# jklebes/MetropolisEngine

Measured on AMD Instinct MI355X. Metric: MC steps/sec (chains x sweeps) at 2^20 chains, 16 params, higher is better.
Workload: dtype f64

## Files before the change

### metropolisengine_amd/csrc/me_api.hip

```cpp
#include <algorithm>
#include <cmath>
#include <cstdlib>
#include <cstring>
#include <dlfcn.h>
#include <mutex>
#include <memory>
#include <string>
#include <atomic>
#include <chrono>
#include <vector>

#include "me_engine.h"

namespace me {

static std::vector<const KernelSet *> &registry() {
  static std::vector<const KernelSet *> sets;
  return sets;
}
static std::mutex &registry_mutex() {
  static std::mutex m;
  return m;
}
void register_kernel_set(const KernelSet *set) {
  std::lock_guard<std::mutex> lock(registry_mutex());
  registry().push_back(set);
}
static bool is_user_kind(int kind) { return kind == ME_ENERGY_USER || kind == ME_ENERGY_USER_INDIRECT; }
const KernelSet *find_kernel_set(int dtype, int n_real, int n_complex, int energy_kind, const char *user_name) {
  std::lock_guard<std::mutex> lock(registry_mutex());
  for (const KernelSet *s : registry()) {
    if (s->dtype != dtype || s->n_real != n_real || s->n_complex != n_complex || !s->has_energy(energy_kind)) continue;
    if (is_user_kind(energy_kind)) {
      if (!s->user_name || !user_name || std::strcmp(s->user_name, user_name) != 0) continue;
    }
    return s;
  }
  if (n_real + 2 * n_complex > kMaxRegisterDof && !is_user_kind(energy_kind))
    for (const KernelSet *s : registry())
      if (s->dtype == dtype && s->n_real < 0 && s->has_energy(energy_kind)) return s;
  return nullptr;
}
bool has_dims(int dtype, int n_real, int n_complex) {
  if (n_real + 2 * n_complex > kMaxRegisterDof) return true;
  std::lock_guard<std::mutex> lock(registry_mutex());
  for (const KernelSet *s : registry())
    if (s->dtype == dtype && s->n_real == n_real && s->n_complex == n_complex && !s->user_name) return true;
  return false;
}

static thread_local std::string g_create_error;

static double norm_ppf(double q) {
  double x = 0.0;
  x = std::log(q / (1.0 - q)) / 1.702;
  for (int it = 0; it < 50; ++it) {
    const double cdf = 0.5 * std::erfc(-x / std::sqrt(2.0));
    const double pdf = std::exp(-0.5 * x * x) / std::sqrt(2.0 * M_PI);
    const double f = cdf - q;
    const double step = f / (pdf * (1.0 + 0.5 * x * f / pdf));
    x -= step;
    if (std::fabs(step) < 1e-16 * std::max(1.0, std::fabs(x))) break;
// ... 54 lines not shown
}

int fail(me_engine *e, int code, const std::string &msg) {
  if (e) e->err = msg;
  else g_create_error = msg;
  return code;
}

static void to_device_type(const double *src, size_t count, int dtype, std::vector<unsigned char> &out) {
  out.resize(count * (dtype == ME_F32 ? 4 : 8));
  if (dtype == ME_F32) {
    float *o = reinterpret_cast<float *>(out.data());
    for (size_t i = 0; i < count; ++i) o[i] = (float)src[i];
  } else {
    std::memcpy(out.data(), src, count * 8);
  }
}

hipError_t upload(DeviceBuffer &dst, const double *src, size_t count, int dtype) {
  std::vector<unsigned char> bytes;
  to_device_type(src, count, dtype, bytes);
  const hipError_t err = dst.resize(bytes.size());
  return err != hipSuccess ? err : hipMemcpy(dst.get(), bytes.data(), bytes.size(), hipMemcpyHostToDevice);
}

int refuse_stale_total(me_engine *e, const char *subject) {
  if (!e->stale_total) return ME_OK;
  return fail(e, ME_ERR_UNSUPPORTED, std::string(subject) + " not available with ME_FLAG_REFERENCE_ENERGY_LEDGERS: its two ledgers "
                                                            "make the energy of a chain ambiguous");
}

static int report_status(me_engine *e, unsigned int bits) {
  if (!bits) return ME_OK;
  ME_HIP(e, hipMemsetAsync(e->status.get(), 0, sizeof(unsigned int), e->stream));
  std::string msg = "numeric failure in at least one chain:";
  if (bits & ST_NONFINITE_ENERGY) msg += " non-finite energy;";
  if (bits & ST_BAD_PIVOT) msg += " non-positive Cholesky pivot (proposal covariance not positive definite);";
  if (bits & ST_BAD_WIDTH) msg += " sampling width <= 0;";
  return fail(e, ME_ERR_NUMERIC, msg);
}
int check_status(me_engine *e) {
  unsigned long long *scratch = e->host_scratch.get<unsigned long long>();
  ME_HIP(e, hipMemcpyAsync(&scratch[0], e->status.get(), sizeof(unsigned int), hipMemcpyDeviceToHost, e->stream));
  ME_HIP(e, hipStreamSynchronize(e->stream));
  return report_status(e, (unsigned int)scratch[0]);
}

}

using namespace me;

namespace {

int broadcast(me_engine *e, DeviceBuffer &dst, const std::vector<double> &row, bool tiled = false) {
  std::vector<unsigned char> bytes;
  to_device_type(row.data(), row.size(), e->dtype, bytes);
  ME_HIP(e, hipMemcpyAsync(e->row_dev.get(), bytes.data(), bytes.size(), hipMemcpyHostToDevice, e->stream));
  if (tiled) ME_HIP(e, launch_broadcast_tiled(dst.get(), e->row_dev.get(), (int)row.size(), e->n, e->dtype, e->stream));
  else ME_HIP(e, launch_broadcast_rows(dst.get(), e->row_dev.get(), (int)row.size(), e->n, e->dtype, e->stream));
  ME_HIP(e, hipStreamSynchronize(e->stream));
  return ME_OK;
}

template <typename T>
void gather_rows(const T *t, int comps, int64_t n_chains, double *dst) {
  for (int r = 0; r < comps; ++r)
    for (int64_t c = 0; c < n_chains; ++c) dst[c * comps + r] = (double)t[(size_t)r * n_chains + c];
}
template <typename T>
void scatter_rows(T *t, int comps, int64_t n_chains, const double *src) {
  for (int r = 0; r < comps; ++r)
    for (int64_t c = 0; c < n_chains; ++c) t[(size_t)r * n_chains + c] = (T)src[c * comps + r];
}
template <typename T>
void transpose_tiled(T *t, int entries, int64_t tile0, int64_t chain_begin, int64_t n_chains, double *dst, const double *src) {
  const size_t tile_values = (size_t)entries * 64;
  auto at = [&](int64_t c, int k) { return (size_t)((c >> 6) - tile0) * tile_values + (size_t)k * 64 + (size_t)(c & 63); };
  for (int64_t i = 0; i < n_chains; ++i)
    for (int k = 0; k < entries; ++k) {
      if (dst) dst[i * entries + k] = (double)t[at(chain_begin + i, k)];
      else t[at(chain_begin + i, k)] = (T)src[i * entries + k];
    }
}

int copy_tiled(me_engine *e, void *field_ptr, int entries, int64_t chain_begin, int64_t n_chains, double *dst, const double *src) {
  const int64_t tile0 = chain_begin >> 6, tile1 = (chain_begin + n_chains - 1) >> 6;
  const size_t tile_values = (size_t)entries * 64, n_values = (size_t)(tile1 - tile0 + 1) * tile_values;
  unsigned char *dev = (unsigned char *)field_ptr + (size_t)tile0 * tile_values * e->esize;
  std::vector<unsigned char> tmp(n_values * e->esize);
  const bool whole = (chain_begin & 63) == 0 && (((chain_begin + n_chains) & 63) == 0 || chain_begin + n_chains == e->n);
  if (dst || !whole) {
    ME_HIP(e, hipMemcpyAsync(tmp.data(), dev, tmp.size(), hipMemcpyDeviceToHost, e->stream));
    ME_HIP(e, hipStreamSynchronize(e->stream));
  }
  if (e->dtype == ME_F32) transpose_tiled(reinterpret_cast<float *>(tmp.data()), entries, tile0, chain_begin, n_chains, dst, src);
  else transpose_tiled(reinterpret_cast<double *>(tmp.data()), entries, tile0, chain_begin, n_chains, dst, src);
  if (src) {
    ME_HIP(e, hipMemcpyAsync(dev, tmp.data(), tmp.size(), hipMemcpyHostToDevice, e->stream));
    ME_HIP(e, hipStreamSynchronize(e->stream));
  }
  return dst ? check_status(e) : ME_OK;
}

int field_info(me_engine *e, int field, void **ptr, int *comps) {
  switch (field) {
    case ME_FIELD_PARAMS: *ptr = e->x.get(); *comps = e->d; return ME_OK;
    case ME_FIELD_ENERGY: *ptr = e->energy.get(); *comps = e->n_terms; return ME_OK;
    case ME_FIELD_WIDTH: *ptr = e->width.get(); *comps = e->width_rows; return ME_OK;
    case ME_FIELD_MEAN: *ptr = e->mean.get(); *comps = e->d; return ME_OK;
    case ME_FIELD_OBS_MEAN: *ptr = e->obs_mean.get(); *comps = e->nobs; return ME_OK;
    case ME_FIELD_COV:
      if (!e->cov)
        return fail(e, ME_ERR_UNSUPPORTED, "this engine keeps no per-chain covariance: for large parameter spaces it is "
                                           "kept on request only (me_config.flags: ME_FLAG_TRACK_COVARIANCE), and not "
                                           "at all where the field would pass 4 GiB");
      *ptr = e->cov.get(); *comps = e->p; return ME_OK;
    case ME_FIELD_ENERGY_TOTAL:
      if (!e->stale_total)
        return fail(e, ME_ERR_UNSUPPORTED, "this engine keeps one coherent energy ledger (sum ME_FIELD_ENERGY); a separate "
                                           "energy_total exists with ME_FLAG_REFERENCE_ENERGY_LEDGERS only");
      *ptr = e->energy.get<unsigned char>() + (size_t)e->n_terms * (size_t)e->n * e->esize; *comps = 1; return ME_OK;
    case ME_FIELD_FACTOR:
      if (!e->factor) return fail(e, ME_ERR_UNSUPPORTED, "this engine keeps no per-chain proposal factors (dimensions "
                                                         "without per-chain kernels, or a field beyond 4 GiB)");
      *ptr = e->factor.get(); *comps = e->p; return ME_OK;
    default: return fail(e, ME_ERR_INVALID, "unknown field id");
  }
}

int upload_shared_factor(me_engine *e, const double *packed) {
  ME_HIP(e, upload(e->shared_factor, packed, (size_t)e->p, e->dtype));
  if (e->shared_full) {
    std::vector<double> full((size_t)e->nr * e->nr, 0.0);
    for (int i = 0; i < e->nr; ++i)
      for (int j = 0; j <= i; ++j) full[(size_t)i * e->nr + j] = packed[i * (i + 1) / 2 + j];
    ME_HIP(e, upload(e->shared_full, full.data(), full.size(), e->dtype));
    if (e->shared_image) ME_HIP(e, e->ks->prepare_matrix(e->shared_full.get(), e->shared_image.get(), e->stream));
  }
  return ME_OK;
}

void fill_step_launch(me_engine *e, StepLaunch &l, int n_sweeps) {
  l.n_real = e->nr;
  l.n_complex = e->nc;
  l.x = e->x.get();
  l.energy = e->energy.get();
  l.width = e->width.get();
  l.factor = e->cov_kind == CK_PER_CHAIN ? e->factor.get() : e->shared_factor.get();
  l.factor_full = e->shared_full.get();
// ... 90 lines not shown
  if (!ks) {
    if (is_user_kind(c->energy_kind))
      return fail(nullptr, ME_ERR_UNSUPPORTED,
                  std::string("no user-energy plugin named '") + (c->user_energy_name ? c->user_energy_name : "") +
                      "' is loaded for these dimensions (build it with metropolisengine_amd.build.build_user_energy "
                      "and load it with me_load_plugin)");
    if (!has_dims(c->dtype, c->n_real, c->n_complex))
      return fail(nullptr, ME_ERR_UNSUPPORTED,
                  "no kernel set compiled for (dtype, n_real, n_complex) = (" + std::to_string(c->dtype) + ", " +
                      std::to_string(c->n_real) + ", " + std::to_string(c->n_complex) + ")");
    return fail(nullptr, ME_ERR_UNSUPPORTED, "energy kind " + std::to_string(c->energy_kind) +
                                                  " is not compiled for these dimensions");
  }
  if ((rc = check_user_reject(nullptr, c->reject_kind, ks)) != ME_OK) return rc;
  if (ks->n_real < 0) {
    if (c->cov_mode == ME_COV_POOLED && c->n_complex > 0)
      return fail(nullptr, ME_ERR_UNSUPPORTED,
                  "parameter spaces beyond " + std::to_string(kMaxRegisterDof) + " real degrees of freedom with complex "
                  "parameters run with the identity proposal shape (ME_COV_FIXED, cov_mode=\"fixed\") or per-chain shapes "
                  "(ME_COV_REFERENCE); one shared factor (ME_COV_POOLED) is there for pure real spaces");
    const bool starts_shared = !initial_shape_is_identity(c) && c->cov_mode != ME_COV_REFERENCE;
    if (starts_shared && c->n_complex > 0)
      return fail(nullptr, ME_ERR_UNSUPPORTED,
                  "parameter spaces beyond " + std::to_string(kMaxRegisterDof) + " real degrees of freedom with complex "
                  "parameters run with the identity proposal shape only: leave covariance_matrix_real / _complex unset");
    {
      const long long per_block = (long long)(c->n_real + 2 * c->n_complex) * 64 * (c->dtype == ME_F32 ? 4 : 8);
      const bool dense = c->energy_kind == ME_ENERGY_DENSE_QUAD, pooled = c->cov_mode == ME_COV_POOLED || starts_shared;
      const bool per_chain = c->cov_mode == ME_COV_REFERENCE || (c->flags & ME_FLAG_TRACK_COVARIANCE) != 0;
      if ((dense || pooled || per_chain) && per_block * (pooled ? 2 : 1) > 150 * 1024)
        return fail(nullptr, ME_ERR_UNSUPPORTED,
                    "a dense quadratic form, a shared proposal factor or per-chain shapes beyond " + std::to_string(kMaxRegisterDof) +
                        " degrees of freedom are staged in LDS: this many parameters do not fit (float64: about 290, 145 with "
                        "a shared factor or an initial covariance that ME_COV_FIXED keeps; float32 twice that)");
    }
    if (c->flags & ME_FLAG_REFERENCE_ENERGY_LEDGERS)
      return fail(nullptr, ME_ERR_UNSUPPORTED, "ME_FLAG_REFERENCE_ENERGY_LEDGERS is not available beyond " +
                                                   std::to_string(kMaxRegisterDof) + " real degrees of freedom");
    if (c->reject_kind == ME_REJECT_USER) return fail(nullptr, ME_ERR_UNSUPPORTED, "no user plugins at these dimensions");
  }
  if ((c->flags & ME_FLAG_REFERENCE_ENERGY_LEDGERS) && (c->n_real == 0 || c->n_complex == 0))
    return fail(nullptr, ME_ERR_INVALID,
                "ME_FLAG_REFERENCE_ENERGY_LEDGERS applies to mixed engines (real and complex parameters): only their "
                "step_all keeps a separate energy_total (metropolis_engine.py:241-259)");
  if (c->cov_mode == ME_COV_REFERENCE && !ks->per_chain_cov)
    return fail(nullptr, ME_ERR_UNSUPPORTED,
                "per-chain adaptive covariance is not compiled for these dimensions; use ME_COV_FIXED or ME_COV_POOLED");
  return ME_OK;
}

struct Layout {
  bool keep_per_chain;
  bool keep_cov;
  bool x_tiled;
  int width_rows;
};
int decide_layout(const me_config *c, const KernelSet *ks, Layout &l) {
  const long long esz = c->dtype == ME_F32 ? 4 : 8, limit = 1ll << 32, padded = padded_chains(c->n_chains);
  l.keep_per_chain = ks->per_chain_cov && (!ks->streams_packed || c->cov_mode == ME_COV_REFERENCE);
  if (l.keep_per_chain && !ks->streams_packed && (long long)packed_total(c->n_real, c->n_complex) * padded * esz >= limit) {
    if (c->cov_mode == ME_COV_REFERENCE)
      return fail(nullptr, ME_ERR_UNSUPPORTED,
                  "the per-chain covariance field would exceed 4 GiB on this engine; shard the chains over more "
                  "engines or use ME_COV_FIXED / ME_COV_POOLED");
    l.keep_per_chain = false;
  }
  const long long rows = std::max<long long>(c->n_real + 2 * c->n_complex, 2 * c->n_real + c->n_complex);
  if (rows * padded * esz >= limit)
    return fail(nullptr, ME_ERR_UNSUPPORTED,
                "a per-chain field would exceed 4 GiB on this engine; shard the chains over more engines");
  l.keep_cov = l.keep_per_chain ||
               ((!ks->per_chain_cov || ks->streams_packed) && ks->tracks_cov && (c->flags & ME_FLAG_TRACK_COVARIANCE));
  l.x_tiled = ks->tiled_state;
  l.width_rows = (c->n_real > 0 && c->n_complex > 0) ? 3 : 1;
  return ME_OK;
}

std::unique_ptr<me_engine> configure(const me_config *c, const KernelSet *ks, const Layout &l) {
  std::unique_ptr<me_engine> e(new me_engine);
  e->device = c->device_id;
  e->ks = ks;
  e->n_terms = ks->energy_terms(c->energy_kind);
  e->dtype = c->dtype;
  e->esize = c->dtype == ME_F32 ? 4 : 8;
  e->n = c->n_chains;
  e->nr = c->n_real;
  e->nc = c->n_complex;
  e->d = e->nr + 2 * e->nc;
  e->p = packed_total(e->nr, e->nc);
  e->nobs = n_observables(e->nr, e->nc);
  e->chain_offset = c->chain_offset;
  e->seed = c->seed;
  e->temp = c->temp;
  e->target_acceptance = c->target_acceptance;
  e->energy_kind = c->energy_kind;
  e->reject_kind = c->reject_kind;
  e->reject_bound = c->reject_bound;
  e->cov_mode = c->cov_mode;
  e->coef.assign(c->energy_coeffs, c->energy_coeffs + c->n_energy_coeffs);
  e->alpha = -norm_ppf(c->target_acceptance / 2.0);
  e->m = e->nr + e->nc;
  e->ratio = (1.0 - 1.0 / e->m) * std::sqrt(2.0 * M_PI) * std::exp(e->alpha * e->alpha / 2.0) / 2.0 * e->alpha +
             1.0 / (e->m * c->target_acceptance * (1.0 - c->target_acceptance));
  if (const char *g = std::getenv("ME_GRID_BLOCKS")) e->grid_blocks = std::atoi(g);
  e->x_tiled = l.x_tiled;
  e->stale_total = (c->flags & ME_FLAG_REFERENCE_ENERGY_LEDGERS) != 0;
  e->width_rows = l.width_rows;
  e->n_slots = (e->n + 31) / 32 + 8;
  return e;
}

int allocate(me_engine *e, const Layout &l) {
  const KernelSet *ks = e->ks;
  ME_HIP(e, hipSetDevice(e->device));
  ME_HIP(e, e->stream.create());
  const size_t n = (size_t)e->n, tiles = (size_t)padded_chains(e->n), es = e->esize;
  ME_HIP(e, e->x.resize((e->x_tiled ? tiles : n) * e->d * es));
  ME_HIP(e, e->energy.resize(n * (e->n_terms + (e->stale_total ? 1 : 0)) * es));
  ME_HIP(e, e->width.resize(n * e->width_rows * es));
  ME_HIP(e, e->mean.resize(n * e->d * es));
  ME_HIP(e, e->obs_mean.resize(n * e->nobs * es));
  if (l.keep_cov) ME_HIP(e, e->cov.resize(tiles * e->p * es));
  if (l.keep_per_chain) ME_HIP(e, e->factor.resize(tiles * e->p * es));
  ME_HIP(e, e->shared_factor.resize((size_t)e->p * es));
  if (e->nc == 0) ME_HIP(e, e->shared_full.resize((size_t)e->nr * e->nr * es));
  if (e->shared_full && ks->prepare_matrix) ME_HIP(e, e->shared_image.resize(ks->matrix_image_bytes));
  ME_HIP(e, e->row_dev.resize((size_t)std::max(std::max(e->d, e->p), e->nobs) * es));
  ME_HIP(e, e->accept_slots.resize((size_t)e->n_slots * sizeof(unsigned long long)));
  ME_HIP(e, e->accept_total.resize(sizeof(unsigned long long)));
  ME_HIP(e, e->status.resize(sizeof(unsigned int)));
  const size_t moments_bytes = sizeof(double) * (size_t)moments_size(e->nr, e->nc);
  ME_HIP(e, e->pool.dev.resize(moments_bytes));
  ME_HIP(e, e->host_scratch.allocate(64));
  e->host_scratch.get<unsigned long long>()[0] = e->host_scratch.get<unsigned long long>()[1] = 0;
  ME_HIP(e, e->pool.host.allocate(moments_bytes));
  if (pool_reduce_supported(e->nr, e->nc, e->dtype))
    ME_HIP(e, e->pool.partials.resize(sizeof(double) * (size_t)pool_reduce_blocks(e->n, e->nr, e->nc) *
                                      (size_t)(1 + e->d + e->nr + e->nc + e->d * (e->d + 1) / 2)));
  ME_HIP(e, hipMemsetAsync(e->accept_slots.get(), 0, e->accept_slots.bytes(), e->stream));
  ME_HIP(e, hipMemsetAsync(e->status.get(), 0, sizeof(unsigned int), e->stream));
  return ME_OK;
}

int upload_coefficients(me_engine *e) {
  const std::vector<double> &coef = e->coef;
  const bool runtime_dims = e->ks->n_real < 0;
  std::vector<double> form;
  if (runtime_dims && e->energy_kind == ME_ENERGY_DIAG_QUAD) {
    if ((int)coef.size() != e->nr + e->nc) return fail(e, ME_ERR_INVALID, "wrong number of energy coefficients for this energy kind");
    form.assign(coef.begin(), coef.end());
    form.insert(form.end(), coef.begin() + e->nr, coef.end());
  } else if (runtime_dims && e->energy_kind == ME_ENERGY_DENSE_QUAD) {
    if ((int)coef.size() != e->d * e->d) return fail(e, ME_ERR_INVALID, "wrong number of energy coefficients for this energy kind");
    form.reserve((size_t)e->d * (e->d + 1) / 2);
    for (int i = 0; i < e->d; ++i)
      for (int j = 0; j <= i; ++j)
        form.push_back(i == j ? coef[(size_t)i * e->d + i] : coef[(size_t)i * e->d + j] + coef[(size_t)j * e->d + i]);
  } else if (e->energy_kind == ME_ENERGY_DENSE_QUAD || (is_user_kind(e->energy_kind) && !coef.empty())) {
    form = coef;
  } else {
    return ME_OK;
  }
  ME_HIP(e, upload(e->coef_dev, form.data(), form.size(), e->dtype));
  if (!runtime_dims && e->energy_kind == ME_ENERGY_DENSE_QUAD && e->ks->prepare_matrix) {
    ME_HIP(e, e->energy_image.resize(e->ks->matrix_image_bytes));
    ME_HIP(e, e->ks->prepare_matrix(e->coef_dev.get(), e->energy_image.get(), e->stream));
  }
  return ME_OK;
}

int initial_state(me_engine *e, const me_config *c) {
  std::vector<double> init(c->initial_params, c->initial_params + e->d);
  std::vector<double> obs(e->nobs);
  for (int i = 0; i < e->nr; ++i) {
    obs[i] = std::fabs(init[i]);
    obs[e->nr + e->nc + i] = init[i] * init[i];
  }
  for (int j = 0; j < e->nc; ++j) obs[e->nr + j] = std::hypot(init[e->nr + j], init[e->nr + e->nc + j]);
  const int pr = packed_real(e->nr);
  std::vector<double> c0(e->p, 0.0);
  bool identity = true;
  for (int i = 0; i < e->nr; ++i)
    for (int j = 0; j <= i; ++j) {
      const double v = c->covariance_real ? c->covariance_real[i * e->nr + j] : (i == j ? 1.0 : 0.0);
      c0[i * (i + 1) / 2 + j] = v;
      identity = identity && v == (i == j ? 1.0 : 0.0);
    }
  for (int i = 0; i < e->nc; ++i) {
    for (int j = 0; j < i; ++j) {
      const double re = c->covariance_complex ? c->covariance_complex[2 * (i * e->nc + j)] : 0.0;
      const double im = c->covariance_complex ? c->covariance_complex[2 * (i * e->nc + j) + 1] : 0.0;
      c0[pr + i * i + 2 * j] = re;
      c0[pr + i * i + 2 * j + 1] = im;
      identity = identity && re == 0.0 && im == 0.0;
    }
    const double dg = c->covariance_complex ? c->covariance_complex[2 * (i * e->nc + i)] : 1.0;
    c0[pr + i * i + 2 * i] = dg;
    identity = identity && dg == 1.0;
  }
  std::vector<double> f0 = c0;
  for (int i = 0; i < e->nc; ++i)
    for (int j = 0; j < i; ++j) f0[pr + i * i + 2 * j + 1] = -f0[pr + i * i + 2 * j + 1];
  if (!host_factor(f0, e->nr, e->nc))
    return fail(e, ME_ERR_INVALID, "initial covariance matrix is not positive definite (metropolis_engine.py:270)");
  int rc = ME_OK;
  std::vector<double> width_row((size_t)e->width_rows, c->sampling_width);
  if ((rc = broadcast(e, e->x, init, e->x_tiled)) || (rc = broadcast(e, e->mean, init)) || (rc = broadcast(e, e->obs_mean, obs)) ||
      (rc = broadcast(e, e->width, width_row)) || (e->cov && (rc = broadcast(e, e->cov, c0, true))) ||
      (e->factor && (rc = broadcast(e, e->factor, f0, true))) || (rc = upload_shared_factor(e, f0.data())))
    return rc;
  e->cov_kind = identity ? CK_IDENTITY : (e->ks->n_real < 0 && e->factor) ? CK_PER_CHAIN : CK_SHARED;
  return ME_OK;
}

int initial_energy(me_engine *e) {
  const int rc = me_recompute_energy(e);
  if (rc != ME_OK) return rc;
  const hipError_t herr = hipStreamSynchronize(e->stream);
  if (herr != hipSuccess) return fail(e, ME_ERR_HIP, std::string("initial energy evaluation: ") + hipGetErrorString(herr));
  return ME_OK;
}

}

int me_create(const me_config *c, me_engine **out) {
  if (!c || !out) return fail(nullptr, ME_ERR_INVALID, "null config or output pointer");
  *out = nullptr;
  const KernelSet *ks = nullptr;
  Layout layout;
  int rc;
  if ((rc = validate_config(c, &ks)) || (rc = decide_layout(c, ks, layout))) return rc;
  int n_dev = 0;
  if (hipGetDeviceCount(&n_dev) != hipSuccess || n_dev <= 0)
    return fail(nullptr, ME_ERR_HIP, "no HIP device available (this library has no CPU fallback)");
  if (c->device_id < 0 || c->device_id >= n_dev) return fail(nullptr, ME_ERR_INVALID, "device_id out of range");

  std::unique_ptr<me_engine> e = configure(c, ks, layout);
  if ((rc = allocate(e.get(), layout)) || (rc = upload_coefficients(e.get())) || (rc = initial_state(e.get(), c)) ||
      (rc = initial_energy(e.get())))
    return fail(nullptr, rc, e->err);
  *out = e.release();
  return ME_OK;
}

int me_set_reject_condition(me_engine *e, int32_t reject_kind, double reject_bound) {
  if (!e) return ME_ERR_INVALID;
  int rc;
  if ((rc = check_reject_kind(e, reject_kind, e->energy_kind, e->nr)) || (rc = check_user_reject(e, reject_kind, e->ks))) return rc;
  e->reject_kind = reject_kind;
  e->reject_bound = reject_bound;
  return ME_OK;
}

int me_set_energy(me_engine *e, int32_t energy_kind, const double *coeffs, int32_t n_coeffs, const char *user_name) {
  if (!e) return ME_ERR_INVALID;
  if (n_coeffs < 0 || (n_coeffs > 0 && !coeffs)) return fail(e, ME_ERR_INVALID, "energy coefficients missing");
  if (e->ks->n_real < 0) return fail(e, ME_ERR_UNSUPPORTED, "me_set_energy: not available on the runtime-dimension kernel set");
  if (energy_kind == ME_ENERGY_DENSE_QUAD)
    return fail(e, ME_ERR_UNSUPPORTED, "me_set_energy: the dense quadratic form keeps device images of its matrix; create a new engine");
  const KernelSet *ks = find_kernel_set(e->dtype, e->nr, e->nc, energy_kind, user_name);
  if (!ks || ks->n_real < 0)
    return fail(e, ME_ERR_UNSUPPORTED, is_user_kind(energy_kind)
                    ? std::string("no user-energy plugin named '") + (user_name ? user_name : "") + "' is loaded for these dimensions"
                    : "energy kind " + std::to_string(energy_kind) + " is not compiled for these dimensions");
  if (ks->tiled_state != e->ks->tiled_state || ks->per_chain_cov != e->ks->per_chain_cov || ks->streams_packed != e->ks->streams_packed ||
      ks->tracks_cov != e->ks->tracks_cov)
    return fail(e, ME_ERR_UNSUPPORTED, "me_set_energy: the plugin was built with other per-chain covariance options than this engine's kernel set");
  if (e->reject_kind == ME_REJECT_USER && !ks->has_user_reject)
    return fail(e, ME_ERR_UNSUPPORTED, "me_set_energy: the engine's wall is the plugin's me_user_reject, which the new energy does not define");
  const int n_terms = ks->energy_terms(energy_kind);
  ME_HIP(e, hipSetDevice(e->device));
  ME_HIP(e, hipStreamSynchronize(e->stream));
  DeviceBuffer ledger, coef_dev;
  if (n_terms != e->n_terms)
    ME_HIP(e, ledger.resize((size_t)e->n * (size_t)(n_terms + (e->stale_total ? 1 : 0)) * e->esize));
  if (is_user_kind(energy_kind) && n_coeffs > 0) ME_HIP(e, upload(coef_dev, coeffs, (size_t)n_coeffs, e->dtype));
  if (n_terms != e->n_terms) {
    e->energy = std::move(ledger);
    e->n_terms = n_terms;
    if (e->trace.chains > 0) e->trace.restart();
  }
  e->coef.assign(coeffs, coeffs + n_coeffs);
  e->coef_dev = std::move(coef_dev);
  e->ks = ks;
  e->energy_kind = energy_kind;
  const int rc = me_recompute_energy(e);
  if (rc != ME_OK) return rc;
  ME_HIP(e, hipStreamSynchronize(e->stream));
  return check_status(e);
}

int me_load_plugin(const char *path) {
  if (!path) return fail(nullptr, ME_ERR_INVALID, "null plugin path");
  void *handle = dlopen(path, RTLD_NOW | RTLD_GLOBAL);
  if (!handle) return fail(nullptr, ME_ERR_INVALID, std::string("dlopen failed: ") + dlerror());
  return ME_OK;
}

int me_destroy(me_engine *e) {
  if (!e) return ME_ERR_INVALID;
  (void)hipSetDevice(e->device);
  if (e->stream) (void)hipStreamSynchronize(e->stream);
  if (e->pool.copy_stream) (void)hipStreamSynchronize(e->pool.copy_stream);
  delete e;
  return ME_OK;
}

int me_recompute_energy(me_engine *e) {
  if (!e) return ME_ERR_INVALID;
  ME_HIP(e, hipSetDevice(e->device));
  EnergyLaunch l;
  l.n_real = e->nr;
  l.n_complex = e->nc;
  l.total_row = e->stale_total ? e->n_terms : -1;
  l.x = e->x.get();
  l.energy = e->energy.get();
  l.coef_device = e->coef_dev.get();
  l.coef_host = e->coef.data();
// ... 88 lines not shown
      for (size_t j = 0; j < nz; ++j) zn[(s * nz + j) * n + c] = normals[(s * n + c) * nz + j];
      for (size_t j = 0; j < nu; ++j) un[(s * nu + j) * n + c] = uniforms[(s * n + c) * nu + j];
    }
  DeviceBuffer zd, ud;
  ME_HIP(e, zd.resize(zn.size() * sizeof(double)));
  if (ud.resize(un.size() * sizeof(double)) != hipSuccess) return fail(e, ME_ERR_HIP, "hipMalloc of the injected uniforms failed");
  if (hipMemcpy(zd.get(), zn.data(), zd.bytes(), hipMemcpyHostToDevice) != hipSuccess ||
      hipMemcpy(ud.get(), un.data(), ud.bytes(), hipMemcpyHostToDevice) != hipSuccess)
    return fail(e, ME_ERR_HIP, "upload of the injected streams failed");
  int rc = launch_step_kind(e, kind, n_sweeps, zd.get(), ud.get());
  if (rc == ME_OK && hipStreamSynchronize(e->stream) != hipSuccess) rc = fail(e, ME_ERR_HIP, "injected step failed");
  return rc;
}

namespace {
void fill_measure_launch(me_engine *e, MeasureLaunch &l, unsigned long long count) {
  l.n_real = e->nr;
  l.n_complex = e->nc;
  l.x = e->x.get();
  l.width = e->width.get();
  l.mean = e->mean.get();
  l.cov = e->cov.get();
  l.obs_mean = e->obs_mean.get();
  l.factor = e->factor.get();
  l.status = e->status.get<unsigned int>();
  l.n = e->n;
  l.measure_count = count;
  l.update_cov = (count > 50 && e->cov) ? 1 : 0;
  l.split_widths = (e->width_rows == 3 && !e->widths_synced) ? 1 : 0;
  l.write_factor = (l.update_cov && e->cov_mode == ME_COV_REFERENCE) ? 1 : 0;
  l.grid_blocks = e->grid_blocks;
}

int commit_measure(me_engine *e, const MeasureLaunch &l) {
  e->measure_count = l.measure_count;
  if (l.write_factor) e->cov_kind = CK_PER_CHAIN;
  if (e->trace.chains > 0) {
    const long long cols = e->d + e->n_terms + e->width_rows;
    if (e->trace.rows == e->trace.capacity) {
      const long long cap = e->trace.capacity ? 2 * e->trace.capacity : 1024;
      DeviceBuffer bigger;
      ME_HIP(e, bigger.resize(sizeof(double) * (size_t)(cap * cols * e->trace.chains)));
      if (e->trace.dev) {
        ME_HIP(e, hipMemcpyAsync(bigger.get(), e->trace.dev.get(), sizeof(double) * (size_t)(e->trace.rows * cols * e->trace.chains),
                                 hipMemcpyDeviceToDevice, e->stream));
        ME_HIP(e, hipStreamSynchronize(e->stream));
      }
      e->trace.dev = std::move(bigger);
      e->trace.capacity = cap;
    }
    const int rows_valid = (e->width_rows == 3 && e->widths_synced) ? 1 : e->width_rows;
    double *row = e->trace.dev.get<double>() + e->trace.rows * cols * e->trace.chains;
    ME_HIP(e, launch_trace(e->x.get(), e->energy.get(), e->width.get(), e->n, e->d, e->n_terms, rows_valid, e->dtype, e->trace.chains,
                           e->trace.stride, row, e->stream, e->x_tiled));
    if (rows_valid != e->width_rows) {
      double *widths = row + (size_t)(e->d + e->n_terms) * e->trace.chains;
      for (int r = 1; r < 3; ++r)
        ME_HIP(e, hipMemcpyAsync(widths + (size_t)r * e->trace.chains, widths, sizeof(double) * (size_t)e->trace.chains,
                                 hipMemcpyDeviceToDevice, e->stream));
    }
    e->trace.rows += 1;
  }
  return ME_OK;
}
}

int me_measure(me_engine *e) {
  if (!e) return ME_ERR_INVALID;
  ME_HIP(e, hipSetDevice(e->device));
  MeasureLaunch l;
  fill_measure_launch(e, l, e->measure_count + 1);
  ME_HIP(e, e->ks->measure(l, e->stream));
  return commit_measure(e, l);
}

int me_cycle(me_engine *e, int32_t n_sweeps) {
  if (!e) return ME_ERR_INVALID;
  if (n_sweeps <= 0) return fail(e, ME_ERR_INVALID, "n_sweeps must be positive");
  ME_HIP(e, hipSetDevice(e->device));
  if (e->ks->cycle) {
    StepLaunch sl;
    fill_step_launch(e, sl, n_sweeps);
    MeasureLaunch ml;
    fill_measure_launch(e, ml, e->measure_count + 1);
    ml.split_widths = 0;
    const hipError_t err = e->ks->cycle(sl, ml, e->stream);
    if (err == hipSuccess) {
      count_steps(e, n_sweeps);
      e->fused_cycles += 1;
      return commit_measure(e, ml);
    }
    if (err != hipErrorNotSupported) ME_HIP(e, err);
    (void)hipGetLastError();
  }
  const int rc = me_step(e, n_sweeps);
  return rc != ME_OK ? rc : me_measure(e);
}

int me_cycle_stats(me_engine *e, uint64_t *fused_cycles) {
  if (!e || !fused_cycles) return ME_ERR_INVALID;
  *fused_cycles = e->fused_cycles;
  return ME_OK;
}

int me_trace_enable(me_engine *e, int64_t n_traced, int64_t stride) {
  if (!e) return ME_ERR_INVALID;
  if (n_traced < 0 || stride < 1 || (n_traced > 0 && (n_traced - 1) * stride >= e->n))
    return fail(e, ME_ERR_INVALID, "traced chains out of range");
  ME_HIP(e, hipSetDevice(e->device));
  ME_HIP(e, hipStreamSynchronize(e->stream));
  e->trace.restart();
  e->trace.chains = n_traced;
  e->trace.stride = stride;
  return ME_OK;
}

int me_trace_shape(me_engine *e, int64_t *rows, int64_t *cols, int64_t *n_traced) {
  if (!e) return ME_ERR_INVALID;
  if (rows) *rows = e->trace.rows;
  if (cols) *cols = e->d + e->n_terms + e->width_rows;
  if (n_traced) *n_traced = e->trace.chains;
  return ME_OK;
}

int me_trace_get(me_engine *e, double *dst, int64_t n_doubles) {
  if (!e || !dst) return ME_ERR_INVALID;
  const long long want = e->trace.rows * (e->d + e->n_terms + e->width_rows) * e->trace.chains;
  if (n_doubles != want) return fail(e, ME_ERR_INVALID, "wrong trace buffer length");
  if (want == 0) return ME_OK;
  ME_HIP(e, hipSetDevice(e->device));
  ME_HIP(e, hipStreamSynchronize(e->stream));
  ME_HIP(e, hipMemcpy(dst, e->trace.dev.get(), sizeof(double) * (size_t)want, hipMemcpyDeviceToHost));
  return ME_OK;
}

int me_field_components(me_engine *e, int32_t field, int32_t *n_components) {
  if (!e || !n_components) return ME_ERR_INVALID;
  void *ptr;
  int comps;
  int rc = field_info(e, field, &ptr, &comps);
  if (rc == ME_OK) *n_components = comps;
  return rc;
}

int me_energy_terms(me_engine *e, int32_t *n_terms) {
  if (!e || !n_terms) return ME_ERR_INVALID;
  *n_terms = e->n_terms;
  return ME_OK;
}

int me_get(me_engine *e, int32_t field, int64_t chain_begin, int64_t n_chains, double *dst) {
  if (!e || !dst) return ME_ERR_INVALID;
  if (chain_begin < 0 || n_chains < 0 || chain_begin + n_chains > e->n) return fail(e, ME_ERR_INVALID, "chain range out of bounds");
  ME_HIP(e, hipSetDevice(e->device));
  void *ptr;
  int comps;
  int rc = field_info(e, field, &ptr, &comps);
  if (rc != ME_OK) return rc;
  if (n_chains == 0) return ME_OK;
  if (field == ME_FIELD_COV || field == ME_FIELD_FACTOR || (field == ME_FIELD_PARAMS && e->x_tiled))
    return copy_tiled(e, ptr, comps, chain_begin, n_chains, dst, nullptr);
  std::vector<unsigned char> tmp((size_t)comps * n_chains * e->esize);
  for (int r = 0; r < comps; ++r)
    ME_HIP(e, hipMemcpyAsync(tmp.data() + (size_t)r * n_chains * e->esize,
                             (const unsigned char *)ptr + ((size_t)r * e->n + chain_begin) * e->esize,
                             (size_t)n_chains * e->esize, hipMemcpyDeviceToHost, e->stream));
  ME_HIP(e, hipStreamSynchronize(e->stream));
  if (e->dtype == ME_F32) gather_rows(reinterpret_cast<const float *>(tmp.data()), comps, n_chains, dst);
  else gather_rows(reinterpret_cast<const double *>(tmp.data()), comps, n_chains, dst);
  if (field == ME_FIELD_WIDTH && e->width_rows == 3 && e->widths_synced)
    for (int64_t c = 0; c < n_chains; ++c) dst[c * 3 + 1] = dst[c * 3 + 2] = dst[c * 3];
  return check_status(e);
}

int me_set(me_engine *e, int32_t field, int64_t chain_begin, int64_t n_chains, const double *src) {
  if (!e || !src) return ME_ERR_INVALID;
  if (chain_begin < 0 || n_chains < 0 || chain_begin + n_chains > e->n) return fail(e, ME_ERR_INVALID, "chain range out of bounds");
  ME_HIP(e, hipSetDevice(e->device));
  void *ptr;
  int comps;
  int rc = field_info(e, field, &ptr, &comps);
  if (rc != ME_OK) return rc;
  if (field == ME_FIELD_WIDTH && e->width_rows == 3 && (chain_begin != 0 || n_chains != e->n))
    return fail(e, ME_ERR_INVALID, "widths of a mixed engine must be set for all chains at once");
  if (n_chains == 0) return ME_OK;
  if (field == ME_FIELD_COV || field == ME_FIELD_FACTOR || (field == ME_FIELD_PARAMS && e->x_tiled)) {
    rc = copy_tiled(e, ptr, comps, chain_begin, n_chains, nullptr, src);
    if (rc != ME_OK) return rc;
    if (field == ME_FIELD_FACTOR) e->cov_kind = CK_PER_CHAIN;
    return ME_OK;
  }
  std::vector<unsigned char> tmp((size_t)comps * n_chains * e->esize);
  if (e->dtype == ME_F32) scatter_rows(reinterpret_cast<float *>(tmp.data()), comps, n_chains, src);
  else scatter_rows(reinterpret_cast<double *>(tmp.data()), comps, n_chains, src);
  for (int r = 0; r < comps; ++r)
    ME_HIP(e, hipMemcpyAsync((unsigned char *)ptr + ((size_t)r * e->n + chain_begin) * e->esize,
                             tmp.data() + (size_t)r * n_chains * e->esize, (size_t)n_chains * e->esize,
                             hipMemcpyHostToDevice, e->stream));
  ME_HIP(e, hipStreamSynchronize(e->stream));
  if (field == ME_FIELD_FACTOR) e->cov_kind = CK_PER_CHAIN;
  if (field == ME_FIELD_WIDTH && e->width_rows == 3) e->widths_synced = false;
  return ME_OK;
}

int me_constants(me_engine *e, double *alpha, int32_t *m, double *ratio) {
  if (!e) return ME_ERR_INVALID;
  if (alpha) *alpha = e->alpha;
  if (m) *m = e->m;
  if (ratio) *ratio = e->ratio;
  return ME_OK;
}

int me_counters(me_engine *e, uint64_t *step_index, uint64_t *measure_step_counter) {
  if (!e) return ME_ERR_INVALID;
  if (step_index) *step_index = e->step_index;
  if (measure_step_counter) *measure_step_counter = e->measure_count;
  return ME_OK;
}

int me_set_counters(me_engine *e, uint64_t step_index, uint64_t measure_step_counter) {
  if (!e) return ME_ERR_INVALID;
  if (measure_step_counter < 1) return fail(e, ME_ERR_INVALID, "measure_step_counter starts at 1");
  e->step_index = step_index;
  e->measure_count = measure_step_counter;
  return ME_OK;
}

int me_accept_stats(me_engine *e, uint64_t *accepted, uint64_t *proposed) {
  if (!e) return ME_ERR_INVALID;
  ME_HIP(e, hipSetDevice(e->device));
  unsigned long long *scratch = e->host_scratch.get<unsigned long long>();
  ME_HIP(e, launch_sum_slots(e->accept_slots.get<unsigned long long>(), e->n_slots, e->accept_total.get<unsigned long long>(), e->stream));
  ME_HIP(e, hipMemcpyAsync(&scratch[1], e->accept_total.get(), sizeof(unsigned long long), hipMemcpyDeviceToHost, e->stream));
  ME_HIP(e, hipMemcpyAsync(&scratch[0], e->status.get(), sizeof(unsigned int), hipMemcpyDeviceToHost, e->stream));
  ME_HIP(e, hipStreamSynchronize(e->stream));
  if (accepted) *accepted = scratch[1];
  if (proposed) *proposed = e->proposed;
  return report_status(e, (unsigned int)scratch[0]);
}

int me_set_accept_stats(me_engine *e, uint64_t accepted, uint64_t proposed) {
  if (!e) return ME_ERR_INVALID;
  if (accepted > proposed) return fail(e, ME_ERR_INVALID, "accepted exceeds proposed");
  ME_HIP(e, hipSetDevice(e->device));
  const unsigned long long total = accepted;
  ME_HIP(e, hipMemsetAsync(e->accept_slots.get(), 0, e->accept_slots.bytes(), e->stream));
  ME_HIP(e, hipMemcpyAsync(e->accept_slots.get(), &total, sizeof(total), hipMemcpyHostToDevice, e->stream));
  ME_HIP(e, hipStreamSynchronize(e->stream));
  e->proposed = proposed;
  return ME_OK;
}

int me_pooled_moments_size(me_engine *e, int64_t *n_doubles) {
  if (!e || !n_doubles) return ME_ERR_INVALID;
  *n_doubles = moments_size(e->nr, e->nc);
  return ME_OK;
}

namespace {
hipError_t wait_polling(hipEvent_t ev) {
  const auto t0 = std::chrono::steady_clock::now();
  for (;;) {
    const hipError_t rc = hipEventQuery(ev);
    if (rc != hipErrorNotReady) return rc;
    if (std::chrono::steady_clock::now() - t0 > std::chrono::milliseconds(2)) return hipEventSynchronize(ev);
  }
}
hipError_t wait_polling(hipStream_t stream) {
  const auto t0 = std::chrono::steady_clock::now();
  for (;;) {
    const hipError_t rc = hipStreamQuery(stream);
    if (rc != hipErrorNotReady) return rc;
    if (std::chrono::steady_clock::now() - t0 > std::chrono::milliseconds(2)) return hipStreamSynchronize(stream);
  }
}

int check_pooled(me_engine *e, int64_t n_doubles) {
  if (n_doubles != moments_size(e->nr, e->nc)) return fail(e, ME_ERR_INVALID, "wrong pooled-moment buffer length");
  if (e->pool.pending) return fail(e, ME_ERR_STATE, "a pooled-moment reduction is in flight (me_pooled_moments_end first)");
  if (!e->pool.partials) return fail(e, ME_ERR_UNSUPPORTED, "pooled moments: dimension too large for the reduction kernel");
  ME_HIP(e, hipSetDevice(e->device));
  return ME_OK;
}
int enqueue_pool_reduce(me_engine *e, const void *x, long long n_chains, long long n_slots, double proposed, double *device_out) {
  hipError_t err = launch_pool_reduce(x, n_chains, e->nr, e->nc, e->dtype, e->accept_slots.get<unsigned long long>(), n_slots, proposed,
                                      e->pool.partials.get<double>(), device_out, e->stream, e->ks->pool_stage1, e->x_tiled);
  if (err == hipErrorInvalidValue) return fail(e, ME_ERR_UNSUPPORTED, "pooled moments: dimension too large for the reduction kernel");
  ME_HIP(e, err);
  return ME_OK;
}
int enqueue_pooled_moments(me_engine *e, double *device_out, int64_t n_doubles) {
  const int rc = check_pooled(e, n_doubles);
  return rc != ME_OK ? rc : enqueue_pool_reduce(e, e->x.get(), e->n, e->n_slots, (double)e->proposed, device_out);
}
int fetch_pooled_moments(me_engine *e, double *host_out, int64_t n_doubles) {
  const size_t bytes = sizeof(double) * (size_t)n_doubles;
  ME_HIP(e, hipMemcpyAsync(e->pool.host.get<double>(), e->pool.dev.get(), bytes, hipMemcpyDeviceToHost, e->stream));
  ME_HIP(e, wait_polling(e->stream));
  std::memcpy(host_out, e->pool.host.get<double>(), bytes);
  return ME_OK;
}
}

int me_pooled_moments_device(me_engine *e, void *device_out, int64_t n_doubles) {
  if (!e || !device_out) return ME_ERR_INVALID;
  int rc = enqueue_pooled_moments(e, (double *)device_out, n_doubles);
  if (rc != ME_OK) return rc;
  ME_HIP(e, wait_polling(e->stream));
  return ME_OK;
}

int me_pooled_moments(me_engine *e, double *host_out, int64_t n_doubles) {
  if (!e || !host_out) return ME_ERR_INVALID;
  const int rc = enqueue_pooled_moments(e, e->pool.dev.get<double>(), n_doubles);
  return rc != ME_OK ? rc : fetch_pooled_moments(e, host_out, n_doubles);
}

int me_pooled_moments_range(me_engine *e, int64_t chain_begin, int64_t n_chains, double *host_out, int64_t n_doubles) {
  if (!e || !host_out) return ME_ERR_INVALID;
  if (chain_begin < 0 || n_chains <= 0 || chain_begin + n_chains > e->n || chain_begin % 64 != 0 || n_chains % 64 != 0)
    return fail(e, ME_ERR_INVALID, "the chain range must be whole 64-chain tiles inside the engine");
  int rc = check_pooled(e, n_doubles);
  if (rc != ME_OK) return rc;
  const unsigned char *x = e->x.get<unsigned char>();
  if (e->x_tiled) {
    x += (size_t)chain_begin * e->d * e->esize;
  } else {
    const size_t row = (size_t)n_chains * e->esize;
    if (row * e->d > e->pool.range_x.bytes()) {
      ME_HIP(e, hipStreamSynchronize(e->stream));
      ME_HIP(e, e->pool.range_x.reserve(row * e->d));
    }
    ME_HIP(e, hipMemcpy2DAsync(e->pool.range_x.get(), row, x + (size_t)chain_begin * e->esize, (size_t)e->n * e->esize, row, (size_t)e->d,
                               hipMemcpyDeviceToDevice, e->stream));
    x = e->pool.range_x.get<unsigned char>();
  }
  if ((rc = enqueue_pool_reduce(e, x, n_chains, 0, 0.0, e->pool.dev.get<double>())) != ME_OK) return rc;
  return fetch_pooled_moments(e, host_out, n_doubles);
}

namespace {
int begin_pooled(me_engine *e, bool allreduce) {
  if (e->pool.pending) return fail(e, ME_ERR_STATE, "a pooled-moment reduction is already in flight: call me_pooled_moments_end first");
  if (allreduce && !e->comm)
    return fail(e, ME_ERR_STATE, "this engine has no communicator: call me_comm_init_rank first (single-GPU engines use me_pooled_moments)");
  ME_HIP(e, hipSetDevice(e->device));
  if (!e->pool.copy_stream) {
    ME_HIP(e, e->pool.copy_stream.create());
    ME_HIP(e, e->pool.reduced.create(hipEventDisableTiming));
    ME_HIP(e, e->pool.copied.create(hipEventDisableTiming));
  }
  const int64_t n_doubles = moments_size(e->nr, e->nc);
  int rc = enqueue_pooled_moments(e, e->pool.dev.get<double>(), n_doubles);
  if (rc != ME_OK) return rc;
  ME_HIP(e, hipEventRecord(e->pool.reduced, e->stream));
  ME_HIP(e, hipStreamWaitEvent(e->pool.copy_stream, e->pool.reduced, 0));
  if (allreduce) {
    const ncclResult_t nrc = e->rccl->all_reduce(e->pool.dev.get<double>(), e->pool.dev.get<double>(), (size_t)n_doubles, ncclDouble, ncclSum, e->comm, e->pool.copy_stream);
    if (nrc != ncclSuccess) return fail(e, ME_ERR_HIP, std::string("ncclAllReduce: ") + e->rccl->error_string(nrc));
  }
  ME_HIP(e, hipMemcpyAsync(e->pool.host.get<double>(), e->pool.dev.get<double>(), sizeof(double) * (size_t)n_doubles, hipMemcpyDeviceToHost, e->pool.copy_stream));
  ME_HIP(e, hipEventRecord(e->pool.copied, e->pool.copy_stream));
  e->pool.pending = true;
  return ME_OK;
}
}

int me_pooled_moments_begin(me_engine *e) {
  if (!e) return ME_ERR_INVALID;
  return begin_pooled(e, false);
}

int me_pooled_moments_allreduce_begin(me_engine *e) {
  if (!e) return ME_ERR_INVALID;
  return begin_pooled(e, true);
}

int me_pooled_moments_allreduce(me_engine *e, double *host_out, int64_t n_doubles) {
// ... 148 lines not shown
```

### metropolisengine_amd/csrc/me_device.h

```cpp
#pragma once

#include <type_traits>
#include <utility>

#include <hip/hip_runtime.h>
#include <stdint.h>

#include "me_internal.h"
#include "me_math64.h"

namespace me {

struct U4 {
  uint32_t x, y, z, w;
};

__device__ __forceinline__ uint32_t xor3(uint32_t a, uint32_t b, uint32_t c) {
  return __builtin_amdgcn_bitop3_b32(a, b, c, 0x96);
}
__device__ __forceinline__ U4 philox4x32_10(U4 c, uint32_t k0, uint32_t k1) {
#pragma unroll
  for (int r = 0; r < 10; ++r) {
    const uint64_t p0 = (uint64_t)0xD2511F53u * c.x;
    const uint64_t p1 = (uint64_t)0xCD9E8D57u * c.z;
// ... 148 lines not shown
  static constexpr unsigned int kEntryBytes = 64u * (unsigned int)sizeof(R);
  template <int AUX>
  __device__ __forceinline__ R load_aux(int k, unsigned int tile_off) const {
    if constexpr (sizeof(R) == 4) {
      return __builtin_bit_cast(R, __builtin_amdgcn_raw_buffer_load_b32(rsrc, tile_off, (unsigned int)k * kEntryBytes, AUX));
    } else {
      const auto v = __builtin_amdgcn_raw_buffer_load_b64(rsrc, tile_off, (unsigned int)k * kEntryBytes, AUX);
      return __builtin_bit_cast(R, v);
    }
  }
  template <int AUX>
  __device__ __forceinline__ void store_aux(int k, unsigned int tile_off, R value) const {
    if constexpr (sizeof(R) == 4) {
      __builtin_amdgcn_raw_buffer_store_b32(__builtin_bit_cast(unsigned int, value), rsrc, tile_off, (unsigned int)k * kEntryBytes, AUX);
    } else {
      using v2 = decltype(__builtin_amdgcn_raw_buffer_load_b64(rsrc, 0u, 0u, 0));
      __builtin_amdgcn_raw_buffer_store_b64(__builtin_bit_cast(v2, value), rsrc, tile_off, (unsigned int)k * kEntryBytes, AUX);
    }
  }
  __device__ __forceinline__ R load(int k, unsigned int tile_off) const { return load_aux<0>(k, tile_off); }
  __device__ __forceinline__ R load_nt(int k, unsigned int tile_off) const { return load_aux<ME_NT_AUX>(k, tile_off); }
  __device__ __forceinline__ void store(int k, unsigned int tile_off, R value) const { store_aux<0>(k, tile_off, value); }
  __device__ __forceinline__ void store_nt(int k, unsigned int tile_off, R value) const { store_aux<ME_NT_AUX>(k, tile_off, value); }
};

template <bool NT, class F>
__device__ __forceinline__ auto packed_load(const F &f, int row, unsigned int chain_off) {
  if constexpr (NT) return f.load_nt(row, chain_off);
  else return f.load(row, chain_off);
}
template <bool NT, class F, typename R>
__device__ __forceinline__ void packed_store(const F &f, int row, unsigned int chain_off, R value) {
  if constexpr (NT) f.store_nt(row, chain_off, value);
  else f.store(row, chain_off, value);
}

template <typename R, bool NTS>
struct StateField : Field<R> {
  using Field<R>::Field;
  __device__ __forceinline__ R load(int row, unsigned int chain_off) const {
    if constexpr (NTS) return Field<R>::load_nt(row, chain_off);
    else return Field<R>::load(row, chain_off);
  }
  __device__ __forceinline__ void store(int row, unsigned int chain_off, R value) const {
    if constexpr (NTS) Field<R>::store_nt(row, chain_off, value);
    else Field<R>::store(row, chain_off, value);
  }
};

#ifndef ME_TILED_STATE_DOF
#define ME_TILED_STATE_DOF 16
#endif
constexpr int kTiledStateDof = ME_TILED_STATE_DOF;
template <typename R, int D, bool NTS = false>
struct XField {
  static constexpr bool kTiled = D >= kTiledStateDof;
  std::conditional_t<kTiled, TiledField<R>, StateField<R, NTS>> f;
  __device__ __forceinline__ XField(const R *base, long long n) : f(base, n, D) {}
  static __device__ __forceinline__ unsigned int offset(long long c) {
    if constexpr (kTiled) return tiled_offset<R>(c, D);
    else return (unsigned int)c * (unsigned int)sizeof(R);
  }
  __device__ __forceinline__ R load(int row, unsigned int off) const {
    if constexpr (kTiled && NTS) return f.load_nt(row, off);
    else return f.load(row, off);
  }
  __device__ __forceinline__ void store(int row, unsigned int off, R value) const {
    if constexpr (kTiled && NTS) f.store_nt(row, off, value);
    else f.store(row, off, value);
  }
};
template <typename R, int D>
__device__ __forceinline__ long long state_index(long long c, int row, long long n) {
  if constexpr (D >= kTiledStateDof) return ((c >> 6) * (long long)D + row) * 64 + (c & 63);
  else return (long long)row * n + c;
}

constexpr int kMaxPackedInRegisters = 160;
#ifndef ME_STREAM_F64_ENTRIES
#define ME_STREAM_F64_ENTRIES 96
#endif
constexpr int kStreamF64Entries = ME_STREAM_F64_ENTRIES;

template <typename R, int NR, int NC>
struct EnergyIso {
  static constexpr int D = NR + 2 * NC;
  R a;
  __device__ __forceinline__ R operator()(const R (&x)[D]) const {
    R s0 = 0, s1 = 0;
#pragma unroll
    for (int d = 0; d + 1 < D; d += 2) {
      s0 += x[d] * x[d];
      s1 += x[d + 1] * x[d + 1];
    }
    if constexpr (D % 2 == 1) s0 += x[D - 1] * x[D - 1];
    return a * (s0 + s1);
  }
};

template <typename R, int NR, int NC>
struct EnergyDiag {
  static constexpr int D = NR + 2 * NC;
  R w[D];
  __device__ __forceinline__ R operator()(const R (&x)[D]) const {
    R s0 = 0, s1 = 0;
#pragma unroll
    for (int d = 0; d + 1 < D; d += 2) {
      s0 += w[d] * x[d] * x[d];
      s1 += w[d + 1] * x[d + 1] * x[d + 1];
    }
    if constexpr (D % 2 == 1) s0 += w[D - 1] * x[D - 1] * x[D - 1];
    return s0 + s1;
  }
};

template <typename R, int NR, int NC>
struct EnergyDense {
  static constexpr int D = NR + 2 * NC;
  static constexpr int PT = D * (D + 1) / 2;
  const R *a;
  static __device__ __forceinline__ R *folded() {
    __shared__ R t[PT];
    return t;
  }
  __device__ __forceinline__ void prepare() const {
    R *t = folded();
    constexpr int kBatch = 8;
    for (int k0 = threadIdx.x; k0 < PT; k0 += kBatch * (int)blockDim.x) {
      R lo[kBatch], hi[kBatch];
// ... 256 lines not shown
  constexpr bool MOVE_REAL = NR > 0 && GROUP != GROUP_COMPLEX;
  constexpr bool MOVE_COMPLEX = NC > 0 && GROUP != GROUP_REAL;
#pragma unroll
  for (int d = 0; d < D; ++d) xp[d] = x[d];
  if constexpr (CK == CK_IDENTITY) {
    if constexpr (MOVE_REAL) {
#pragma unroll
      for (int i = 0; i < NR; ++i) xp[i] = x[i] + w_r * g[i];
    }
    if constexpr (MOVE_COMPLEX) {
#pragma unroll
      for (int j = 0; j < NC; ++j) {
        xp[NR + j] = x[NR + j] + w_c * (g[NR + j] * R(0.70710678118654752440));
        xp[NR + NC + j] = x[NR + NC + j] + w_c * (g[NR + NC + j] * R(0.70710678118654752440));
      }
    }
  } else {
    if constexpr (MOVE_REAL) {
#pragma unroll
      for (int i = 0; i < NR; ++i) {
        R acc = 0;
#pragma unroll
        for (int j = 0; j <= i; ++j) acc += fac(tri(i, j)) * g[j];
        xp[i] = x[i] + w_r * acc;
      }
    }
    if constexpr (MOVE_COMPLEX) {
#pragma unroll
      for (int i = 0; i < NC; ++i) {
        R are = 0, aim = 0;
#pragma unroll
        for (int j = 0; j < i; ++j) {
          const R lre = fac(cre(PR, i, j));
          const R lim = fac(cim(PR, i, j));
          const R wre = g[NR + j] * R(0.70710678118654752440), wim = g[NR + NC + j] * R(0.70710678118654752440);
          are += lre * wre - lim * wim;
          aim += lre * wim + lim * wre;
        }
        const R ld = fac(cdiag(PR, i));
        are += ld * (g[NR + i] * R(0.70710678118654752440));
        aim += ld * (g[NR + NC + i] * R(0.70710678118654752440));
        xp[NR + i] = x[NR + i] + w_c * are;
        xp[NR + NC + i] = x[NR + NC + i] + w_c * aim;
      }
    }
  }

}

template <typename R, int NR, int NC, class Energy, int CK, int GROUP, bool LADDER, class Ledger>
__device__ __forceinline__ void decide_step(const StepArgs<R> &a, long long c, const Energy &en, bool stale_total, R u,
                                            const R (&g)[2 * ((NR + 2 * NC + 1) / 2)], R (&x)[NR + 2 * NC], const R (&xp)[NR + 2 * NC],
                                            Ledger &ledger, R &total_q5, R &w, R &w_r, R &w_c, unsigned int &wave_accepted,
                                            bool &bad_energy) {
  [[maybe_unused]] constexpr int D = NR + 2 * NC;
  constexpr bool MOVE_REAL = NR > 0 && GROUP != GROUP_COMPLEX;
  constexpr bool MOVE_COMPLEX = NC > 0 && GROUP != GROUP_REAL;
  using N_ = Num<R>;
  bool rejected = false;
  if (a.reject_kind == ME_REJECT_ABS_REAL0_GE) rejected = !(N_::abs_(xp[0]) < a.reject_bound);
  else if (a.reject_kind == ME_REJECT_USER) rejected = energy_reject(en, xp, 0);
  R terms_new[Ledger::T];
  const R e_new = ledger.propose(en, xp, terms_new);
  const R diff = e_new - (stale_total ? total_q5 : ledger.partial());
  bool accept = diff <= R(0);
  if constexpr (LADDER) accept = accept || uphill_at<true>(a, c, u, diff);
  else if (a.temp > R(0)) accept = accept || N_::uphill(u, diff, a.inv_temp, a.inv_temp_log2e);
  accept = accept && !rejected;
  bad_energy |= (!rejected && !N_::finite(e_new));
  if constexpr (CK == CK_IDENTITY) {
    const R wa_r = accept ? w_r : R(0), wa_c = accept ? w_c : R(0);
    if constexpr (MOVE_REAL) {
#pragma unroll
      for (int i = 0; i < NR; ++i) x[i] = x[i] + wa_r * g[i];
    }
    if constexpr (MOVE_COMPLEX) {
#pragma unroll
      for (int j = 0; j < NC; ++j) {
        x[NR + j] = x[NR + j] + wa_c * (g[NR + j] * R(0.70710678118654752440));
        x[NR + NC + j] = x[NR + NC + j] + wa_c * (g[NR + NC + j] * R(0.70710678118654752440));
      }
    }
  } else {
#pragma unroll
    for (int d = 0; d < D; ++d) x[d] = accept ? xp[d] : x[d];
  }
  if (stale_total) total_q5 = accept ? e_new : total_q5;
  else ledger.commit(accept, terms_new);
  w = N_::adapt(w, accept, a.ratio, a.p, a.damping, a.up, a.down);
  if constexpr (GROUP == GROUP_ALL) w_r = w_c = w;
  else if constexpr (GROUP == GROUP_REAL) w_r = w;
  else w_c = w;
  wave_accepted += (unsigned int)__popcll(__ballot(accept));
}

template <typename R, int NR, int NC, class Energy, int CK, bool INJECT, int GROUP, bool LADDER, class Ledger, class Fac>
__device__ __forceinline__ void run_sweeps(const StepArgs<R> &a, const Energy &en, long long c, unsigned long long gid,
                                           bool stale_total, R (&x)[NR + 2 * NC], Ledger &ledger, R &total_q5, R &w, R &w_r,
                                           R &w_c, Fac &&fac, unsigned int &wave_accepted, bool &bad_energy) {
  constexpr int D = NR + 2 * NC;
  constexpr int NW = 2 * ((D + 1) / 2);
  for (int s = 0; s < a.n_sweeps; ++s) {
    R g[NW], u, xp[D];
    draw_step<R, NR, NC, INJECT>(a, c, gid, s, g, u);
    propose_registers<R, NR, NC, CK, GROUP>(x, g, w_r, w_c, fac, xp);
    decide_step<R, NR, NC, Energy, CK, GROUP, LADDER>(a, c, en, stale_total, u, g, x, xp, ledger, total_q5, w, w_r, w_c, wave_accepted, bad_energy);
  }
}

#ifndef ME_STEP_WAVES_PER_EU
#define ME_STEP_WAVES_PER_EU 0
#endif
#if ME_STEP_WAVES_PER_EU > 0
#define ME_STEP_BOUNDS __launch_bounds__(kFusedStepThreads, ME_STEP_WAVES_PER_EU)
#else
#define ME_STEP_BOUNDS __launch_bounds__(kFusedStepThreads)
#endif

#ifndef ME_STEP_PRIO_SHIFT
#define ME_STEP_PRIO_SHIFT 8
#endif
__device__ __forceinline__ void stagger_priority() {
#if ME_STEP_PRIO_SHIFT >= 0
  switch ((blockIdx.x >> ME_STEP_PRIO_SHIFT) & 3u) {
    case 0: __builtin_amdgcn_s_setprio(3); break;
    case 1: __builtin_amdgcn_s_setprio(2); break;
    case 2: __builtin_amdgcn_s_setprio(1); break;
    default: break;
  }
#endif
}

template <typename R, int NR, int NC, class Energy, int CK, bool INJECT = false, int GROUP = GROUP_ALL, bool NTS = false,
          bool LADDER = false>
__global__ void ME_STEP_BOUNDS k_step(StepArgs<R> a, Energy en) {
  constexpr int D = NR + 2 * NC;
  constexpr bool MIXED = NR > 0 && NC > 0;
  static_assert(GROUP == GROUP_ALL || MIXED, "group-wise kernels exist for mixed engines only");
  using N_ = Num<R>;

  stagger_priority();
  if constexpr (!INJECT) N_::prepare();
  energy_prepare(en, 0);
  unsigned int wave_accepted = 0;
  bool bad_energy = false, bad_width = false;
  const long long stride = (long long)gridDim.x * blockDim.x;
  using Ledger = EnergyLedger<R, Energy, GROUP>;
  const XField<R, D, NTS> fx(a.x, a.n);
  const StateField<R, NTS> fe(a.energy, a.n, Ledger::T + (MIXED ? 1 : 0)), fw(a.width, a.n, MIXED ? 3 : 1);
  const bool stale_total = MIXED && GROUP == GROUP_ALL && a.stale_total != 0;
  constexpr bool PER_CHAIN = CK == CK_PER_CHAIN || CK == CK_PER_CHAIN_NT;
  constexpr int PF = PER_CHAIN ? NR * (NR + 1) / 2 + NC * NC : 0;
  constexpr bool STREAM_FACTOR = PER_CHAIN && (PF > kMaxPackedInRegisters ||
                                               (!INJECT && sizeof(R) == 8 && NC == 0 && PF > kStreamF64Entries));
  const TiledField<R> ffac(a.factor, a.n, STREAM_FACTOR ? 0 : PF);
  for (long long c = (long long)blockIdx.x * blockDim.x + threadIdx.x; c < a.n; c += stride) {
    const unsigned int coff = (unsigned int)c * (unsigned int)sizeof(R);
    const unsigned int xoff = fx.offset(c);
    R x[D];
#pragma unroll
    for (int d = 0; d < D; ++d) x[d] = fx.load(d, xoff);
    Ledger ledger;
    R total_q5 = R(0);
    if (stale_total) total_q5 = fe.load(Ledger::T, coff);
    else ledger.load(fe, coff);
    R w = fw.load(MIXED ? GROUP : 0, coff);
    R w_r = w, w_c = w;
    if constexpr (MIXED && GROUP == GROUP_ALL) {
      if (a.split_widths) {
        w_r = fw.load(GROUP_REAL, coff);
        w_c = fw.load(GROUP_COMPLEX, coff);
      }
    }
    const unsigned long long gid = a.chain_offset + (unsigned long long)c;
    [[maybe_unused]] const unsigned int toff = tiled_offset<R>(c, PF);
    auto fac = [&](int k) -> R {
      if constexpr (CK == CK_PER_CHAIN_NT) return ffac.load_nt(k, toff);
      else if constexpr (CK == CK_PER_CHAIN) return ffac.load(k, toff);
      else return a.factor[k];
    };

    if constexpr (STREAM_FACTOR) {
      constexpr int NW = 2 * ((D + 1) / 2);
      for (int s = 0; s < a.n_sweeps; ++s) {
        static_assert(!INJECT, "the streamed-factor form has no replay hook");
        constexpr int NBLK = (NW + 1 + 3) / 4;
        const unsigned long long step = a.step_index + (unsigned long long)s;
        R g[NW];
        R u_accept;
        {
          uint32_t words[4 * NBLK];
#pragma unroll
          for (int b = 0; b < NBLK; ++b) {
            U4 ctr;
            ctr.x = (uint32_t)gid;
            ctr.y = (uint32_t)(gid >> 32);
            ctr.z = (uint32_t)step;
            ctr.w = ((uint32_t)(step >> 32) << 16) | (uint32_t)b;
            const U4 o = philox4x32_10(ctr, a.seed_lo, a.seed_hi);
            words[4 * b + 0] = o.x;
            words[4 * b + 1] = o.y;
            words[4 * b + 2] = o.z;
            words[4 * b + 3] = o.w;
          }
#pragma unroll
          for (int q = 0; q < NW / 2; ++q) N_::normal_pair(words[2 * q], words[2 * q + 1], g[2 * q], g[2 * q + 1]);
          u_accept = N_::unit(words[NW]);
        }
        R xp[D];
#pragma unroll
        for (int d = 0; d < D; ++d) xp[d] = x[d];
        asm volatile("" ::: "memory");
        constexpr int CH = (int)(ME_STREAM_CHUNK_BYTES / sizeof(R));
        const R *tile_base = a.factor + (c >> 6) * (long long)PF * 64;
// ... 24 lines not shown
            __builtin_amdgcn_sched_barrier(0);
          }
          return f[(k / CH) & 1][k % CH];
        };
        static_for<NR>([&](auto row_index) {
          constexpr int i = decltype(row_index)::value;
          R acc = 0;
          static_for<i + 1>([&](auto col_index) {
            constexpr int j = decltype(col_index)::value, k = tri(i, j);
            const R l = use(std::integral_constant<int, k>{});
            acc = j == 0 ? l * g[0] : acc + l * g[j];
          });
          if constexpr (GROUP != GROUP_COMPLEX) xp[i] = x[i] + w_r * acc;
        });
        static_for<NC>([&](auto row_index) {
          constexpr int i = decltype(row_index)::value;
          R are = 0, aim = 0;
          static_for<i>([&](auto col_index) {
            constexpr int j = decltype(col_index)::value;
            const R lre = use(std::integral_constant<int, cre(NR * (NR + 1) / 2, i, j)>{});
            const R lim = use(std::integral_constant<int, cim(NR * (NR + 1) / 2, i, j)>{});
            const R wre = g[NR + j] * R(0.70710678118654752440), wim = g[NR + NC + j] * R(0.70710678118654752440);
            are += lre * wre - lim * wim;
            aim += lre * wim + lim * wre;
          });
          const R ld = use(std::integral_constant<int, cdiag(NR * (NR + 1) / 2, i)>{});
          are += ld * (g[NR + i] * R(0.70710678118654752440));
          aim += ld * (g[NR + NC + i] * R(0.70710678118654752440));
          if constexpr (GROUP != GROUP_REAL) {
            xp[NR + i] = x[NR + i] + w_c * are;
            xp[NR + NC + i] = x[NR + NC + i] + w_c * aim;
          }
        });
        bool rejected = false;
        if (a.reject_kind == ME_REJECT_ABS_REAL0_GE) rejected = !(N_::abs_(xp[0]) < a.reject_bound);
        else if (a.reject_kind == ME_REJECT_USER) rejected = energy_reject(en, xp, 0);
        R terms_new[Ledger::T];
        const R e_new = ledger.propose(en, xp, terms_new);
        const R diff = e_new - (stale_total ? total_q5 : ledger.partial());
        bool accept = diff <= R(0);
        if constexpr (LADDER) accept = accept || uphill_at<true>(a, c, u_accept, diff);
        else if (a.temp > R(0)) accept = accept || N_::uphill(u_accept, diff, a.inv_temp, a.inv_temp_log2e);
        accept = accept && !rejected;
        bad_energy |= (!rejected && !N_::finite(e_new));
#pragma unroll
        for (int d = 0; d < D; ++d) x[d] = accept ? xp[d] : x[d];
        if (stale_total) total_q5 = accept ? e_new : total_q5;
        else ledger.commit(accept, terms_new);
        w = N_::adapt(w, accept, a.ratio, a.p, a.damping, a.up, a.down);
        if constexpr (GROUP == GROUP_ALL) w_r = w_c = w;
        else if constexpr (GROUP == GROUP_REAL) w_r = w;
        else w_c = w;
        wave_accepted += (unsigned int)__popcll(__ballot(accept));
      }
    } else {
      run_sweeps<R, NR, NC, Energy, CK, INJECT, GROUP, LADDER>(a, en, c, gid, stale_total, x, ledger, total_q5, w, w_r, w_c, fac, wave_accepted, bad_energy);
    }
    bad_width |= !(w > R(0));
#pragma unroll
    for (int d = 0; d < D; ++d) fx.store(d, xoff, x[d]);
    if (stale_total) fe.store(Ledger::T, coff, total_q5);
    else ledger.store(fe, coff);
    fw.store(MIXED ? GROUP : 0, coff, w);
  }
  if ((threadIdx.x & 63) == 0 && wave_accepted) {
    unsigned long long *slot = a.accept_slots + (size_t)blockIdx.x * (blockDim.x >> 6) + (threadIdx.x >> 6);
    *slot += (unsigned long long)wave_accepted;
  }
  const unsigned int bits = (bad_energy ? ST_NONFINITE_ENERGY : 0u) | (bad_width ? ST_BAD_WIDTH : 0u);
  if (bits) atomicOr(a.status, bits);
}

template <typename R, int NR, int NC, class Energy>
__global__ void __launch_bounds__(kStepThreads) k_init_energy(const R *xs, R *energy, long long n, unsigned int *status,
                                                                Energy en, int total_row) {
  constexpr int D = NR + 2 * NC;
  energy_prepare(en, 0);
  const long long stride = (long long)gridDim.x * kStepThreads;
  for (long long c = (long long)blockIdx.x * kStepThreads + threadIdx.x; c < n; c += stride) {
    R x[D];
#pragma unroll
    for (int d = 0; d < D; ++d) x[d] = xs[state_index<R, D>(c, d, n)];
    constexpr int T = term_count<Energy>::value;
    bool finite = true;
    R total = R(0);
#pragma unroll
    for (int t = 0; t < T; ++t) {
      R e;
      if constexpr (T == 1) e = en(x);
      else e = en.term(t, x);
      energy[(long long)t * n + c] = e;
      total = t == 0 ? e : total + e;
      finite = finite && Num<R>::finite(e);
    }
    if (total_row >= 0) energy[(long long)total_row * n + c] = total;
    if (!finite) atomicOr(status, (unsigned int)ST_NONFINITE_ENERGY);
  }
}

template <typename R>
struct MeasureArgs {
  const R *x, *width;
  R *mean, *cov, *obs_mean, *factor;
  unsigned int *status;
  long long n;
  R keep;
  R inv_i;
  R cov_keep;
  int update_cov, write_factor, split_widths;
};

template <typename R, int NR, int NC>
__device__ __forceinline__ void cholesky_packed(R (&m)[NR * (NR + 1) / 2 + NC * NC], bool &bad_pivot) {
  constexpr int PR = NR * (NR + 1) / 2;
  using N_ = Num<R>;
#pragma unroll
    for (int j = 0; j < NR; ++j) {
      R s = m[tri(j, j)];
#pragma unroll
      for (int k = 0; k < j; ++k) s = fma_(-m[tri(j, k)], m[tri(j, k)], s);
      if (!(s > R(0))) { bad_pivot = true; s = R(1e-30); }
      const R dg = N_::sqrt_(s);
      const R inv = R(1) / dg;
      m[tri(j, j)] = dg;
#pragma unroll
      for (int i = j + 1; i < NR; ++i) {
        R t = m[tri(i, j)];
#pragma unroll
        for (int k = 0; k < j; ++k) t = fma_(-m[tri(i, k)], m[tri(j, k)], t);
        m[tri(i, j)] = t * inv;
      }
    }
#pragma unroll
    for (int j = 0; j < NC; ++j) {
      R s = m[cdiag(PR, j)];
// ... 149 lines not shown
        }
      } else {
      R m[P];
#pragma unroll
      for (int k = 0; k < P; ++k) m[k] = src.cov(k);
#pragma unroll
      for (int i = 0; i < NR; ++i)
#pragma unroll
        for (int j = 0; j <= i; ++j) {
          const int k = tri(i, j);
          R v = fma_(delta[i] * delta[j], a.inv_i, m[k] * a.cov_keep);
          if (i == j) v = fma_(w2_real, a.inv_i, v);
          packed_store<NT>(fcov, k, toff, v);
          m[k] = v;
        }
#pragma unroll
      for (int i = 0; i < NC; ++i) {
        const R ai = delta[NR + i], bi = delta[NR + NC + i];
#pragma unroll
        for (int j = 0; j < i; ++j) {
          const R aj = delta[NR + j], bj = delta[NR + NC + j];
          const int kr = cre(PR, i, j), ki = cim(PR, i, j);
          const R vr = fma_(fma_(ai, aj, bi * bj), a.inv_i, m[kr] * a.cov_keep);
          const R vi = fma_(fma_(bi, aj, -(ai * bj)), a.inv_i, m[ki] * a.cov_keep);
          packed_store<NT>(fcov, kr, toff, vr);
          packed_store<NT>(fcov, ki, toff, vi);
          m[kr] = vr;
          m[ki] = -vi;
        }
        const int kd = cdiag(PR, i);
        const R vd = fma_(w2_cplx, a.inv_i, fma_(fma_(ai, ai, bi * bi), a.inv_i, m[kd] * a.cov_keep));
        packed_store<NT>(fcov, kd, toff, vd);
        m[kd] = vd;
      }
      if constexpr (FUSED) {
        if (a.write_factor) {
          cholesky_packed<R, NR, NC>(m, bad_pivot);
#pragma unroll
          for (int k = 0; k < P; ++k) packed_store<NT>(ffac, k, toff, m[k]);
        }
      }
      }
    }
  }
}

template <typename R, int NR, int NC, bool PER_CHAIN_COV, bool FUSED, bool NT, bool NTM>
__global__ void __launch_bounds__(kStepThreads, ME_MEASURE_WAVES) k_measure(MeasureArgs<R> a) {
  constexpr int D = NR + 2 * NC;
  constexpr int P = NR * (NR + 1) / 2 + NC * NC;
  constexpr int NOBS = 2 * NR + NC;
  bool bad_pivot = false;
  const long long stride = (long long)gridDim.x * kStepThreads;
  const XField<R, D> fx(a.x, a.n);
  const Field<R> fw(a.width, a.n, (NR > 0 && NC > 0) ? 3 : 1), fmean(a.mean, a.n, D), fobs(a.obs_mean, a.n, NOBS);
  constexpr bool STREAM = PER_CHAIN_COV && P > kMaxPackedInRegisters;
  const TiledField<R> fcov(a.cov, a.n, (PER_CHAIN_COV && !STREAM) ? P : 0);
  const TiledField<R> ffac(a.factor, a.n, (PER_CHAIN_COV && FUSED) ? P : 0);
  __shared__ R s_delta[STREAM ? D : 1][kStepThreads];
  for (long long c = (long long)blockIdx.x * kStepThreads + threadIdx.x; c < a.n; c += stride) {
    const unsigned int coff = (unsigned int)c * (unsigned int)sizeof(R);
    const unsigned int xoff = fx.offset(c);
    R x[D];
#pragma unroll
    for (int d = 0; d < D; ++d) x[d] = fx.load(d, xoff);
    const MeasureFromMemory<R, NT, NTM> src{fmean, fobs, fcov, coff, tiled_offset<R>(c, P)};
    measure_chain<R, NR, NC, PER_CHAIN_COV, FUSED, NT, NTM>(a, c, x, src, fmean, fobs, fcov, ffac, s_delta, [&](R &w_real, R &w_cplx) {
      constexpr bool MIXED = NR > 0 && NC > 0;
      w_real = fw.load((MIXED && a.split_widths) ? 1 : 0, coff);
      w_cplx = fw.load((MIXED && a.split_widths) ? 2 : 0, coff);
    }, bad_pivot);
  }
  if (bad_pivot) atomicOr(a.status, (unsigned int)ST_BAD_PIVOT);
}

#ifndef ME_CYCLE_PREFETCH
#define ME_CYCLE_PREFETCH 0
#endif
constexpr int cycle_prefetch_level(int, int, int, int) { return ME_CYCLE_PREFETCH; }

template <typename R, int NR, int NC, class Energy, int CK, bool NT, bool NTM, bool LADDER = false>
__global__ void ME_STEP_BOUNDS k_cycle(StepArgs<R> a, MeasureArgs<R> ma, Energy en) {
  constexpr int D = NR + 2 * NC;
  constexpr int P = NR * (NR + 1) / 2 + NC * NC;
  constexpr int NOBS = 2 * NR + NC;
  constexpr bool MIXED = NR > 0 && NC > 0;
  static_assert(P <= kMaxPackedInRegisters, "k_cycle keeps the packed matrix in registers");
  static_assert(CK == CK_IDENTITY || CK == CK_SHARED || CK == CK_PER_CHAIN, "NT selects the non-temporal factor read");
  constexpr int CKX = CK == CK_PER_CHAIN ? (NT ? CK_PER_CHAIN_NT : CK_PER_CHAIN) : CK;
  using N_ = Num<R>;
  N_::prepare();
  energy_prepare(en, 0);
  unsigned int wave_accepted = 0;
  bool bad_energy = false, bad_width = false, bad_pivot = false;
  const long long stride = (long long)gridDim.x * blockDim.x;
  using Ledger = EnergyLedger<R, Energy, GROUP_ALL>;
  const XField<R, D> fx(a.x, a.n);
  const Field<R> fe(a.energy, a.n, Ledger::T + (MIXED ? 1 : 0)), fw(a.width, a.n, MIXED ? 3 : 1);
  const Field<R> fmean(ma.mean, a.n, D), fobs(ma.obs_mean, a.n, NOBS);
  const TiledField<R> fcov(ma.cov, a.n, P), ffac(ma.factor, a.n, P);
  const bool stale_total = MIXED && a.stale_total != 0;
  for (long long c = (long long)blockIdx.x * blockDim.x + threadIdx.x; c < a.n; c += stride) {
    const unsigned int coff = (unsigned int)c * (unsigned int)sizeof(R);
    const unsigned int xoff = fx.offset(c);
    R x[D];
#pragma unroll
    for (int d = 0; d < D; ++d) x[d] = fx.load(d, xoff);
    Ledger ledger;
    R total_q5 = R(0);
    if (stale_total) total_q5 = fe.load(Ledger::T, coff);
    else ledger.load(fe, coff);
    R w = fw.load(0, coff);
    R w_r = w, w_c = w;
    if constexpr (MIXED) {
      if (a.split_widths) {
        w_r = fw.load(GROUP_REAL, coff);
        w_c = fw.load(GROUP_COMPLEX, coff);
      }
    }
    const unsigned long long gid = a.chain_offset + (unsigned long long)c;
    [[maybe_unused]] const unsigned int toff = tiled_offset<R>(c, P);
    auto fac = [&](int k) -> R {
      if constexpr (CK == CK_PER_CHAIN) return packed_load<NT>(ffac, k, toff);
      else return a.factor[k];
    };
    constexpr int kPrefetch = cycle_prefetch_level(D, NOBS, P, (int)sizeof(R));
    MeasurePreloaded<R, D, NOBS, P, kPrefetch, NT> pre{{}, {}, {}, fcov, toff};
    if constexpr (kPrefetch >= 1) {
#pragma unroll
      for (int d = 0; d < D; ++d) pre.mu[d] = packed_load<NTM>(fmean, d, coff);
#pragma unroll
      for (int k = 0; k < NOBS; ++k) pre.ob[k] = packed_load<NTM>(fobs, k, coff);
    }
    if constexpr (kPrefetch >= 2) {
      if (ma.update_cov) {
#pragma unroll
        for (int k = 0; k < P; ++k) pre.cv[k] = packed_load<NT>(fcov, k, toff);
      }
    }
    run_sweeps<R, NR, NC, Energy, CKX, false, GROUP_ALL, LADDER>(a, en, c, gid, stale_total, x, ledger, total_q5, w, w_r, w_c, fac,
                                                         wave_accepted, bad_energy);
    bad_width |= !(w > R(0));
#pragma unroll
    for (int d = 0; d < D; ++d) fx.store(d, xoff, x[d]);
    if (stale_total) fe.store(Ledger::T, coff, total_q5);
    else ledger.store(fe, coff);
    fw.store(0, coff, w);
    if constexpr (kPrefetch >= 1) {
      measure_chain<R, NR, NC, true, true, NT, NTM>(ma, c, x, pre, fmean, fobs, fcov, ffac, nullptr,
                                                    [&](R &w_real, R &w_cplx) { w_real = w_cplx = w; }, bad_pivot);
    } else {
      const MeasureFromMemory<R, NT, NTM> src{fmean, fobs, fcov, coff, toff};
      measure_chain<R, NR, NC, true, true, NT, NTM>(ma, c, x, src, fmean, fobs, fcov, ffac, nullptr,
                                                    [&](R &w_real, R &w_cplx) { w_real = w_cplx = w; }, bad_pivot);
    }
  }
  if ((threadIdx.x & 63) == 0 && wave_accepted) {
    unsigned long long *slot = a.accept_slots + (size_t)blockIdx.x * (blockDim.x >> 6) + (threadIdx.x >> 6);
    *slot += (unsigned long long)wave_accepted;
  }
  const unsigned int bits = (bad_energy ? ST_NONFINITE_ENERGY : 0u) | (bad_width ? ST_BAD_WIDTH : 0u) | (bad_pivot ? ST_BAD_PIVOT : 0u);
  if (bits) atomicOr(a.status, bits);
}

template <typename R, int NR, int NC, bool NT>
__global__ void __launch_bounds__(kStepThreads) k_factor(const R *cov, R *factor, unsigned int *status, long long n) {
  constexpr int PR = NR * (NR + 1) / 2;
  constexpr int P = PR + NC * NC;
  bool bad_pivot = false;
  const long long stride = (long long)gridDim.x * kStepThreads;
  const TiledField<R> fcov(cov, n, P), ffac(factor, n, P);
  for (long long c = (long long)blockIdx.x * kStepThreads + threadIdx.x; c < n; c += stride) {
    const unsigned int toff = tiled_offset<R>(c, P);
    R m[P];
#pragma unroll
    for (int k = 0; k < P; ++k) m[k] = packed_load<NT>(fcov, k, toff);
#pragma unroll
    for (int i = 0; i < NC; ++i)
#pragma unroll
      for (int j = 0; j < i; ++j) m[cim(PR, i, j)] = -m[cim(PR, i, j)];
    cholesky_packed<R, NR, NC>(m, bad_pivot);
#pragma unroll
    for (int k = 0; k < P; ++k) packed_store<NT>(ffac, k, toff, m[k]);
  }
  if (bad_pivot) atomicOr(status, (unsigned int)ST_BAD_PIVOT);
}

template <typename R, int NR, bool NT>
__global__ void __launch_bounds__(kStepThreads) k_factor_stream(const R *cov, R *factor, unsigned int *status, long long n) {
  constexpr int P = NR * (NR + 1) / 2;
  constexpr int ROWS = sizeof(R) == 4 ? 4 : 2;
  using N_ = Num<R>;
  __shared__ R rows[ROWS][NR][kStepThreads];
  bool bad_pivot = false;
// ... 178 lines not shown
```

### metropolisengine_amd/csrc/me_engine.h

```cpp
#pragma once

#include <string>
#include <utility>
#include <vector>

#include "me_comm.h"
#include "me_internal.h"

#pragma GCC visibility push(hidden)

namespace me {


class DeviceBuffer {
 public:
  DeviceBuffer() = default;
  DeviceBuffer(DeviceBuffer &&o) noexcept : ptr_(std::exchange(o.ptr_, nullptr)), bytes_(std::exchange(o.bytes_, 0)) {}
  DeviceBuffer &operator=(DeviceBuffer &&o) noexcept {
    if (this != &o) {
      reset();
      ptr_ = std::exchange(o.ptr_, nullptr);
      bytes_ = std::exchange(o.bytes_, 0);
    }
    return *this;
// ... 66 lines not shown

 private:
  hipStream_t stream_ = nullptr;
  bool owned_ = false;
};

class Event {
 public:
  Event() = default;
  Event(const Event &) = delete;
  Event &operator=(const Event &) = delete;
  ~Event() { reset(); }
  void reset() {
    if (event_) (void)hipEventDestroy(event_);
    event_ = nullptr;
  }
  hipError_t create(unsigned flags = hipEventDefault) {
    reset();
    return hipEventCreateWithFlags(&event_, flags);
  }
  operator hipEvent_t() const { return event_; }

 private:
  hipEvent_t event_ = nullptr;
};

}

struct me_engine {
  int device = 0;
  me::Stream stream;
  const me::KernelSet *ks = nullptr;
  int dtype = ME_F32;
  size_t esize = 4;
  long long n = 0;
  int nr = 0, nc = 0, d = 0, p = 0, nobs = 0;
  unsigned long long chain_offset = 0, seed = 0;
  double temp = 0, target_acceptance = 0.3, alpha = 0, ratio = 0, reject_bound = 0;
  int m = 0, energy_kind = 0, reject_kind = 0, cov_mode = 0;
  bool stale_total = false;
  me::Event time_start, time_stop;
  std::vector<double> shared_host;
  int cov_kind = me::CK_IDENTITY;
  int grid_blocks = 0;
  int n_terms = 1;
  std::vector<double> coef;
  unsigned long long step_index = 0, measure_count = 1;
  unsigned long long fused_cycles = 0;
  me::DeviceBuffer x, energy, width, mean, cov, obs_mean;
  me::DeviceBuffer factor, shared_factor, shared_full, shared_image, energy_image, coef_dev, row_dev;
  me::DeviceBuffer accept_slots, accept_total;
  long long n_slots = 0;
  unsigned long long proposed = 0;
  bool x_tiled = false;
  int width_rows = 1;
  bool widths_synced = true;
  me::DeviceBuffer status;
  me::PinnedBuffer host_scratch;
  struct Pool {
    me::DeviceBuffer dev, partials;
    me::PinnedBuffer host;
    me::DeviceBuffer range_x;
    me::Stream copy_stream;
    me::Event reduced, copied;
    bool pending = false;
  } pool;
  const me::RcclApi *rccl = nullptr;
  ncclComm_t comm = nullptr;
  int comm_rank = 0, comm_world = 1;
  struct Trace {
    me::DeviceBuffer dev;
    long long chains = 0, stride = 1, rows = 0, capacity = 0;
    void restart() {
      dev.reset();
      rows = capacity = 0;
    }
  } trace;
  struct Ladder {
    int n_rungs = 0;
    std::vector<double> temps;
    me::DeviceBuffer table;
    me::DeviceBuffer pair_counts;
    unsigned long long round = 0;
  } ladder;
  struct Population {
    me::DeviceBuffer fam, fam_out;
    me::DeviceBuffer x, energy;
    me::DeviceBuffer anc;
    me::DeviceBuffer scratch;
    me::DeviceBuffer records;
    unsigned long long stages = 0, capacity = 0;
    std::vector<double> temps;
  } population;
  struct Samples {
    me::DeviceBuffer data;
    long long capacity = 0, rows = 0;
  } samples;
  std::string err;

  ~me_engine() {
    (void)hipSetDevice(device);
    if (comm && rccl) (void)rccl->comm_destroy(comm);
  }
};

namespace me {

// ... 21 lines not shown
```

### metropolisengine_amd/csrc/me_generic.hip

```cpp
#include "me_internal.h"
#include "me_per_device.h"

namespace me {
namespace {

template <typename R>
__global__ void __launch_bounds__(kBlockThreads) k_broadcast_rows(R *dst, const R *row_values, int rows, long long n) {
  const long long stride = (long long)gridDim.x * kBlockThreads;
  for (long long c = (long long)blockIdx.x * kBlockThreads + threadIdx.x; c < n; c += stride)
    for (int r = 0; r < rows; ++r) dst[(long long)r * n + c] = row_values[r];
}

template <typename R>
__global__ void __launch_bounds__(kBlockThreads) k_broadcast_tiled(R *dst, const R *entry_values, int entries, long long n_padded) {
  const long long total = n_padded * entries, stride = (long long)gridDim.x * kBlockThreads;
  for (long long i = (long long)blockIdx.x * kBlockThreads + threadIdx.x; i < total; i += stride)
    dst[i] = entry_values[(i >> 6) % entries];
}

__device__ __forceinline__ void pair_of(int p, int &i, int &j) {
  i = (int)((sqrtf(8.0f * (float)p + 1.0f) - 1.0f) * 0.5f);
  while (i * (i + 1) / 2 > p) --i;
  while ((i + 1) * (i + 2) / 2 <= p) ++i;
  j = p - i * (i + 1) / 2;
}

constexpr int kMaxEntries = 12;

template <typename R, int TILE>
__global__ void __launch_bounds__(kBlockThreads) k_pool_reduce(const R *x, long long n, int nr, int nc, int entry_base, int tiled, double *partials) {
  extern __shared__ __attribute__((aligned(16))) unsigned char smem_raw[];
  R *tile = reinterpret_cast<R *>(smem_raw);
  constexpr int kTilePitch = TILE + 1;
  const int d = nr + 2 * nc;
  const int n_aug = d + nr + nc;
  const int n_pair = d * (d + 1) / 2;
  const int n_entries = 1 + n_aug + n_pair;
  const int tid = threadIdx.x;
  auto at = [&](int r, long long c) -> long long { return tiled ? ((c >> 6) * (long long)d + r) * 64 + (c & 63) : (long long)r * n + c; };

  int row_i[kMaxEntries], row_j[kMaxEntries];
  bool active[kMaxEntries];
  double acc[kMaxEntries];
#pragma unroll
  for (int k = 0; k < kMaxEntries; ++k) {
    const int e = entry_base + tid + k * kBlockThreads;
    acc[k] = 0.0;
    row_i[k] = row_j[k] = -1;
    active[k] = e < n_entries;
    if (!active[k] || e == 0) continue;
    if (e <= n_aug) {
      row_i[k] = e - 1;
    } else {
      pair_of(e - 1 - n_aug, row_i[k], row_j[k]);
    }
  }

  const long long n_tiles = (n + TILE - 1) / TILE;
  for (long long t = blockIdx.x; t < n_tiles; t += gridDim.x) {
    const long long base = t * TILE;
    const int valid = (int)((n - base) < TILE ? (n - base) : TILE);
    for (int r = tid / TILE; r < n_aug; r += kBlockThreads / TILE) {
      const int col = tid % TILE;
      R v = 0;
      if (col < valid) {
        const long long c = base + col;
        if (r < d) v = x[at(r, c)];
        else if (r < d + nr) {
          const R xv = x[at(r - d, c)];
          v = xv < 0 ? -xv : xv;
        } else {
          const int j = r - d - nr;
          const R re = x[at(nr + j, c)], im = x[at(nr + nc + j, c)];
          v = (R)sqrt((double)re * re + (double)im * im);
        }
      }
      tile[r * kTilePitch + col] = v;
    }
    __syncthreads();
#pragma unroll
    for (int k = 0; k < kMaxEntries; ++k) {
      if (!active[k]) continue;
      if (row_i[k] < 0) {
        acc[k] += (double)valid;
      } else if (row_j[k] < 0) {
        const R *ri = tile + row_i[k] * kTilePitch;
        R s = 0;
        for (int col = 0; col < TILE; ++col) s += ri[col];
        acc[k] += (double)s;
      } else {
        const R *ri = tile + row_i[k] * kTilePitch;
        const R *rj = tile + row_j[k] * kTilePitch;
// ... 52 lines not shown
    for (int b = slice; b < n_blocks; b += kFinishSlices) s += partials[(long long)b * n_entries + e];
  }
  part[slice][lane] = s;
  __syncthreads();
  if (slice != 0) return;
  s = 0.0;
#pragma unroll
  for (int w = 0; w < kFinishSlices; ++w) s += part[w][lane];
  if (e == 0) {
    out[0] = s;
  } else if (e <= n_aug) {
    const int r = e - 1;
    out[r < d ? 1 + r : 1 + d + n_pair + (r - d)] = s;
  } else if (e < n_entries) {
    const int p = e - 1 - n_aug;
    int i, j;
    pair_of(p, i, j);
    out[1 + d + p] = s;
    if (i == j && i < nr) out[1 + d + n_pair + nr + nc + i] = s;
  }
}

}

hipError_t launch_broadcast_rows(void *dst, const void *row_values, int rows, long long n, int dtype,
                                 hipStream_t stream) {
  long long blocks = (n + kBlockThreads - 1) / kBlockThreads;
  if (blocks > 4096) blocks = 4096;
  if (blocks < 1) blocks = 1;
  if (dtype == ME_F32)
    hipLaunchKernelGGL(k_broadcast_rows<float>, dim3((unsigned)blocks), dim3(kBlockThreads), 0, stream, (float *)dst,
                       (const float *)row_values, rows, n);
  else
    hipLaunchKernelGGL(k_broadcast_rows<double>, dim3((unsigned)blocks), dim3(kBlockThreads), 0, stream, (double *)dst,
                       (const double *)row_values, rows, n);
  return hipGetLastError();
}

hipError_t launch_broadcast_tiled(void *dst, const void *entry_values, int entries, long long n, int dtype,
                                  hipStream_t stream) {
  const long long n_padded = (n + 63) / 64 * 64;
  long long blocks = (n_padded * entries + kBlockThreads - 1) / kBlockThreads;
  if (blocks > 8192) blocks = 8192;
  if (blocks < 1) blocks = 1;
  if (dtype == ME_F32)
    hipLaunchKernelGGL(k_broadcast_tiled<float>, dim3((unsigned)blocks), dim3(kBlockThreads), 0, stream, (float *)dst,
                       (const float *)entry_values, entries, n_padded);
  else
    hipLaunchKernelGGL(k_broadcast_tiled<double>, dim3((unsigned)blocks), dim3(kBlockThreads), 0, stream, (double *)dst,
                       (const double *)entry_values, entries, n_padded);
  return hipGetLastError();
}

constexpr int kSumThreads = 1024;
__global__ void __launch_bounds__(kSumThreads) k_sum_slots(const unsigned long long *slots, long long n_slots,
                                                           unsigned long long *total) {
  __shared__ unsigned long long part[kSumThreads / 64];
  unsigned long long s = 0;
  long long i = threadIdx.x;
  for (; i + 7 * kSumThreads < n_slots; i += 8 * kSumThreads) {
    unsigned long long v[8];
#pragma unroll
    for (int u = 0; u < 8; ++u) v[u] = slots[i + u * kSumThreads];
#pragma unroll
    for (int u = 0; u < 8; ++u) s += v[u];
  }
  for (; i < n_slots; i += kSumThreads) s += slots[i];
#pragma unroll
  for (int w = 32; w > 0; w >>= 1) s += __shfl_xor(s, w, 64);
  if ((threadIdx.x & 63) == 0) part[threadIdx.x >> 6] = s;
  __syncthreads();
  if (threadIdx.x == 0) {
    unsigned long long t = 0;
#pragma unroll
    for (int w = 0; w < kSumThreads / 64; ++w) t += part[w];
    total[0] = t;
  }
}

template <typename R>
__global__ void __launch_bounds__(kBlockThreads) k_trace(const R *x, const R *energy, const R *width, long long n, int d,
                                                         int n_terms, int width_rows, long long n_traced, long long stride,
                                                         int tiled, double *out) {
  const long long t = (long long)blockIdx.x * kBlockThreads + threadIdx.x;
  if (t >= n_traced) return;
  const long long c = t * stride;
  for (int k = 0; k < d; ++k)
    out[(long long)k * n_traced + t] = (double)x[tiled ? ((c >> 6) * (long long)d + k) * 64 + (c & 63) : (long long)k * n + c];
  for (int k = 0; k < n_terms; ++k) out[(long long)(d + k) * n_traced + t] = (double)energy[(long long)k * n + c];
  for (int r = 0; r < width_rows; ++r)
    out[(long long)(d + n_terms + r) * n_traced + t] = (double)width[(long long)r * n + c];
}

hipError_t launch_trace(const void *x, const void *energy, const void *width, long long n, int d, int n_terms,
                        int width_rows, int dtype, long long n_traced, long long stride, double *out, hipStream_t stream,
                        bool tiled_state) {
  const dim3 grid((unsigned)((n_traced + kBlockThreads - 1) / kBlockThreads)), block(kBlockThreads);
  if (dtype == ME_F32)
    hipLaunchKernelGGL(k_trace<float>, grid, block, 0, stream, (const float *)x, (const float *)energy, (const float *)width,
                       n, d, n_terms, width_rows, n_traced, stride, tiled_state ? 1 : 0, out);
  else
    hipLaunchKernelGGL(k_trace<double>, grid, block, 0, stream, (const double *)x, (const double *)energy,
                       (const double *)width, n, d, n_terms, width_rows, n_traced, stride, tiled_state ? 1 : 0, out);
  return hipGetLastError();
}

hipError_t launch_sum_slots(const unsigned long long *slots, long long n_slots, unsigned long long *total,
                            hipStream_t stream) {
  hipLaunchKernelGGL(k_sum_slots, dim3(1), dim3(kSumThreads), 0, stream, slots, n_slots, total);
  return hipGetLastError();
}

constexpr size_t kPoolLdsLimit = 160 * 1024;
int pool_tile_chains(int nr, int nc, int dtype) {
  const int n_aug = nr + 2 * nc + nr + nc;
  const size_t elem = dtype == ME_F32 ? sizeof(float) : sizeof(double);
  for (int tile : {64, 32, 16})
    if ((size_t)n_aug * (size_t)(tile + 1) * elem <= kPoolLdsLimit) return tile;
  return 0;
}

bool pool_reduce_supported(int nr, int nc, int dtype) { return pool_tile_chains(nr, nc, dtype) != 0; }

int pool_reduce_blocks(long long n, int nr, int nc) {
  const int d = nr + 2 * nc;
  const long long n_entries = 1 + d + nr + nc + (long long)d * (d + 1) / 2;
  long long cap = (32ll << 20) / (8 * n_entries);
  if (cap > 1024) cap = 1024;
  if (cap < 64) cap = 64;
  if (d + nr + nc <= 32) cap = 256;
  const long long tiles = (n + 63) / 64;
  return (int)(tiles < cap ? (tiles < 1 ? 1 : tiles) : cap);
}

namespace {
template <typename R, int TILE>
hipError_t launch_pool_stage1(const void *x, long long n, int nr, int nc, int n_entries, int blocks, double *partials, hipStream_t stream, bool tiled) {
  const size_t lds = (size_t)(nr + 2 * nc + nr + nc) * (size_t)(TILE + 1) * sizeof(R);
  if (lds > 64 * 1024) {
    static PerDevice<hipError_t> attr;
    int device = 0;
    if (hipError_t rc = hipGetDevice(&device); rc != hipSuccess) return rc;
    const hipError_t rc = attr.get(device, [] {
      return hipFuncSetAttribute((const void *)k_pool_reduce<R, TILE>, hipFuncAttributeMaxDynamicSharedMemorySize, (int)kPoolLdsLimit);
    });
    if (rc != hipSuccess) return rc;
  }
  for (int base = 0; base < n_entries; base += kMaxEntries * kBlockThreads)
    hipLaunchKernelGGL((k_pool_reduce<R, TILE>), dim3((unsigned)blocks), dim3(kBlockThreads), lds, stream, (const R *)x, n, nr, nc, base,
                       tiled ? 1 : 0, partials);
  return hipGetLastError();
}
template <typename R>
hipError_t launch_pool_stage1_tile(int tile, const void *x, long long n, int nr, int nc, int n_entries, int blocks, double *partials, hipStream_t stream, bool tiled) {
  switch (tile) {
    case 64: return launch_pool_stage1<R, 64>(x, n, nr, nc, n_entries, blocks, partials, stream, tiled);
    case 32: return launch_pool_stage1<R, 32>(x, n, nr, nc, n_entries, blocks, partials, stream, tiled);
    case 16: return launch_pool_stage1<R, 16>(x, n, nr, nc, n_entries, blocks, partials, stream, tiled);
    default: return hipErrorInvalidValue;
  }
}
}

hipError_t launch_pool_reduce(const void *x, long long n, int nr, int nc, int dtype, const unsigned long long *slots,
                              long long n_slots, double proposed, double *partials, double *out_device,
                              hipStream_t stream,
                              hipError_t (*stage1)(const void *, long long, double *, int, hipStream_t), bool tiled_state) {
  const int d = nr + 2 * nc;
  const int n_aug = d + nr + nc;
  const int n_entries = 1 + n_aug + d * (d + 1) / 2;
  const int tile = pool_tile_chains(nr, nc, dtype);
  if (!stage1 && tile == 0) return hipErrorInvalidValue;
  const int blocks = pool_reduce_blocks(n, nr, nc);
  hipError_t err;
  if (stage1) err = stage1(x, n, partials, blocks, stream);
  else if (dtype == ME_F32) err = launch_pool_stage1_tile<float>(tile, x, n, nr, nc, n_entries, blocks, partials, stream, tiled_state);
  else err = launch_pool_stage1_tile<double>(tile, x, n, nr, nc, n_entries, blocks, partials, stream, tiled_state);
  if (err != hipSuccess) return err;
  hipLaunchKernelGGL(k_pool_finish, dim3((unsigned)((n_entries + 63) / 64 + 1)), dim3(kFinishThreads), 0, stream,
                     (const double *)partials, blocks, nr, nc, slots, n_slots, proposed, out_device);
  return hipGetLastError();
}

}
```

### metropolisengine_amd/csrc/me_internal.h

```cpp
#pragma once

#include <hip/hip_runtime.h>
#include <stdint.h>

#include "../../include/metropolis_engine.h"

namespace me {

enum CovKind { CK_IDENTITY = 0, CK_SHARED = 1, CK_PER_CHAIN = 2, CK_PER_CHAIN_NT = 3 };

enum StepGroup { GROUP_ALL = 0, GROUP_REAL = 1, GROUP_COMPLEX = 2 };

enum StatusBits : uint32_t {
  ST_NONFINITE_ENERGY = 1u,
  ST_BAD_PIVOT = 2u,
  ST_BAD_WIDTH = 4u
};

long long cache_budget_bytes();
void set_cache_budget_bytes(long long bytes);

constexpr int kBlockThreads = 256;
#ifndef ME_STEP_THREADS
#define ME_STEP_THREADS 64
#endif
constexpr int kStepThreads = ME_STEP_THREADS;
constexpr int kFusedStepThreads = 256;
constexpr int kFusedSweepsThreshold = 4;

struct StepLaunch {
  int n_real, n_complex;
  void *x, *energy, *width;
  const void *factor;
  const void *factor_full;
  const void *factor_image;
  const void *energy_image;
  const void *coef_device;
  const double *coef_host;
  int n_coef;
  const void *inj_normals;
  const void *inj_uniforms;
  unsigned long long *accept_slots;
  unsigned int *status;
  long long n;
  unsigned long long chain_offset, step_index, seed;
  int n_sweeps, energy_kind, cov_kind, reject_kind, grid_blocks;
  int group;
  int split_widths;
  int stale_total;
  const void *cov;
  double reject_bound, temp, ratio, target_acceptance, damping;
  const void *ladder;
  int tiles_per_rung;
};

struct MeasureLaunch {
  int n_real, n_complex;
  void *x, *width, *mean, *cov, *obs_mean, *factor;
  unsigned int *status;
  long long n;
  unsigned long long measure_count;
  int update_cov;
  int split_widths;
  int write_factor;
  int grid_blocks;
};

struct EnergyLaunch {
  int n_real, n_complex;
  int total_row;
  void *x, *energy;
  const void *coef_device;
  const double *coef_host;
  int n_coef;
  unsigned int *status;
  long long n;
  int energy_kind, grid_blocks;
};

constexpr int kMaxRegisterDof = 96;

struct KernelSet {
  const char *user_name;
  int dtype, n_real, n_complex;
  bool per_chain_cov;
  bool tracks_cov;
  bool (*has_energy)(int energy_kind);
  int (*energy_terms)(int energy_kind);
  hipError_t (*step)(const StepLaunch &, hipStream_t);
  hipError_t (*magphase)(const StepLaunch &, hipStream_t);
  hipError_t (*measure)(const MeasureLaunch &, hipStream_t);
  hipError_t (*init_energy)(const EnergyLaunch &, hipStream_t);
  size_t matrix_image_bytes;
  hipError_t (*prepare_matrix)(const void *matrix, void *image, hipStream_t);
  hipError_t (*pool_stage1)(const void *x, long long n, double *partials, int n_rows, hipStream_t);
  bool has_user_reject;
  bool streams_packed;
  hipError_t (*cycle)(const StepLaunch &, const MeasureLaunch &, hipStream_t);
  bool tiled_state;
};

void register_kernel_set(const KernelSet *set);
const KernelSet *find_kernel_set(int dtype, int n_real, int n_complex, int energy_kind, const char *user_name);
bool has_dims(int dtype, int n_real, int n_complex);

hipError_t launch_broadcast_rows(void *dst, const void *row_values, int rows, long long n, int dtype,
                                 hipStream_t stream);
hipError_t launch_broadcast_tiled(void *dst, const void *entry_values, int entries, long long n, int dtype,
                                  hipStream_t stream);
hipError_t launch_pool_reduce(const void *x, long long n, int n_real, int n_complex, int dtype,
                              const unsigned long long *slots, long long n_slots, double proposed, double *partials,
                              double *out_device, hipStream_t stream,
                              hipError_t (*stage1)(const void *, long long, double *, int, hipStream_t) = nullptr,
                              bool tiled_state = false);
int pool_reduce_blocks(long long n, int n_real, int n_complex);
bool pool_reduce_supported(int n_real, int n_complex, int dtype);
hipError_t launch_trace(const void *x, const void *energy, const void *width, long long n, int d, int n_terms,
                        int width_rows, int dtype, long long n_traced, long long stride, double *out, hipStream_t stream,
                        bool tiled_state = false);
hipError_t launch_sum_slots(const unsigned long long *slots, long long n_slots, unsigned long long *total,
                            hipStream_t stream);

inline int grid_for(long long n, int requested, int threads = kStepThreads) {
  long long blocks = (n + threads - 1) / threads;
  if (requested > 0 && blocks > requested) blocks = requested;
  if (blocks < 1) blocks = 1;
  return (int)blocks;
}

__host__ __device__ inline int packed_real(int nr) { return nr * (nr + 1) / 2; }
__host__ __device__ inline int packed_total(int nr, int nc) { return nr * (nr + 1) / 2 + nc * nc; }
__host__ __device__ inline int n_observables(int nr, int nc) { return 2 * nr + nc; }
__host__ __device__ inline long long moments_size(int nr, int nc) {
  const int d = nr + 2 * nc;
  return 1 + d + (long long)d * (d + 1) / 2 + n_observables(nr, nc) + 2;
}

}
```

### metropolisengine_amd/csrc/me_kernels.hip

```cpp
#include <type_traits>

#include "me_device.h"
#include "me_dense_mfma.h"
#include "me_dense_bf16x3.h"
#include "me_dense_f64.h"
#include "me_factor_tile.h"
#include "me_per_device.h"
#include "me_pool_gram.h"
#include "me_magphase.h"

#ifdef ME_USER_SOURCE
#include ME_USER_SOURCE
#endif

#ifndef ME_NR
#error "compile with -DME_NR=<n_real> -DME_NC=<n_complex>"
#endif
#ifndef ME_DENSE
#define ME_DENSE 0
#endif
#ifndef ME_PER_CHAIN
#define ME_PER_CHAIN 1
#endif
#ifndef ME_TRACK_COV
// ... 73 lines not shown
  if (kind == ME_ENERGY_USER) return 1;
#endif
  return kind == ME_ENERGY_USER_INDIRECT ? 1 : 0;
#endif
  switch (kind) {
    case ME_ENERGY_ISO_QUAD:
    case ME_ENERGY_DIAG_QUAD: return 1;
    case ME_ENERGY_DENSE_QUAD: return ME_DENSE != 0 ? 1 : 0;
    case ME_ENERGY_LANDAU_TOY: return kLandau ? 1 : 0;
    case ME_ENERGY_LANDAU_TERMS: return kLandau ? 2 : 0;
    case ME_ENERGY_CYLINDER: return kCylinder ? 1 : 0;
    default: return 0;
  }
}
bool has_energy(int kind) { return energy_terms(kind) > 0; }

template <typename R>
StepArgs<R> typed(const StepLaunch &l) {
  StepArgs<R> a;
  a.x = (R *)l.x;
  a.energy = (R *)l.energy;
  a.width = (R *)l.width;
  a.factor = (const R *)l.factor;
  a.inj_normals = (const R *)l.inj_normals;
  a.inj_uniforms = (const R *)l.inj_uniforms;
  a.accept_slots = l.accept_slots;
  a.status = l.status;
  a.n = l.n;
  a.chain_offset = l.chain_offset;
  a.step_index = l.step_index;
  a.seed_lo = (uint32_t)l.seed;
  a.seed_hi = (uint32_t)(l.seed >> 32);
  a.n_sweeps = l.n_sweeps;
  a.reject_kind = l.reject_kind;
  a.split_widths = l.split_widths;
  a.stale_total = l.stale_total;
  a.reject_bound = (R)l.reject_bound;
  a.temp = (R)l.temp;
  a.inv_temp = l.temp > 0 ? (R)(1.0 / l.temp) : (R)0;
  a.inv_temp_log2e = l.temp > 0 ? (R)(1.4426950408889634 / l.temp) : (R)0;
  a.ratio = (R)l.ratio;
  a.p = (R)l.target_acceptance;
  a.damping = (R)l.damping;
  a.up = (R)(l.ratio * (1.0 - l.target_acceptance) / l.damping);
  a.down = (R)(-l.ratio * l.target_acceptance / l.damping);
  a.ladder = (const R *)l.ladder;
  a.tiles_per_rung = l.tiles_per_rung;
  return a;
}

template <typename R, class Energy, bool INJECT, int GROUP, bool LADDER>
hipError_t launch_step_cov(const StepLaunch &l, const StepArgs<R> &a, const Energy &en, dim3 grid, dim3 block,
                           hipStream_t stream) {
  switch (l.cov_kind) {
    case CK_IDENTITY: {
      constexpr long long state_bytes = (long long)sizeof(R) * (D + 2);
      if constexpr (!INJECT && GROUP == GROUP_ALL && !LADDER) {
        if (state_bytes * l.n > 2 * cache_budget_bytes()) {
          hipLaunchKernelGGL((k_step<R, NR, NC, Energy, CK_IDENTITY, INJECT, GROUP, true>), grid, block, 0, stream, a, en);
          break;
        }
      }
      hipLaunchKernelGGL((k_step<R, NR, NC, Energy, CK_IDENTITY, INJECT, GROUP, false, LADDER>), grid, block, 0, stream, a, en);
      break;
    }
    case CK_SHARED: hipLaunchKernelGGL((k_step<R, NR, NC, Energy, CK_SHARED, INJECT, GROUP, false, LADDER>), grid, block, 0, stream, a, en); break;
#if ME_PER_CHAIN == 2
    case CK_PER_CHAIN: {
      if constexpr (INJECT) return hipErrorInvalidValue;
      else hipLaunchKernelGGL((k_step<R, NR, NC, Energy, CK_PER_CHAIN_NT, INJECT, GROUP, false, LADDER>), grid, block, 0, stream, a, en);
      break;
    }
#elif ME_PER_CHAIN
    case CK_PER_CHAIN: {
      constexpr long long per_chain_bytes = (long long)sizeof(R) * (D + 2 + NR * (NR + 1) / 2 + NC * NC);
      if constexpr (!INJECT) {
        if (per_chain_bytes * l.n > cache_budget_bytes()) {
          hipLaunchKernelGGL((k_step<R, NR, NC, Energy, CK_PER_CHAIN_NT, INJECT, GROUP, false, LADDER>), grid, block, 0, stream, a, en);
          break;
        }
      }
      hipLaunchKernelGGL((k_step<R, NR, NC, Energy, CK_PER_CHAIN, INJECT, GROUP, false, LADDER>), grid, block, 0, stream, a, en);
      break;
    }
#endif
    default: return hipErrorInvalidValue;
  }
  return hipGetLastError();
}

template <typename R, class Energy, bool INJECT, bool LADDER = false>
hipError_t launch_step_group(const StepLaunch &l, const StepArgs<R> &a, const Energy &en, dim3 grid, dim3 block,
                             hipStream_t stream) {
  if (l.group == GROUP_ALL) return launch_step_cov<R, Energy, INJECT, GROUP_ALL, LADDER>(l, a, en, grid, block, stream);
  if constexpr (NR > 0 && NC > 0) {
    if (l.group == GROUP_REAL) return launch_step_cov<R, Energy, INJECT, GROUP_REAL, LADDER>(l, a, en, grid, block, stream);
    if (l.group == GROUP_COMPLEX) return launch_step_cov<R, Energy, INJECT, GROUP_COMPLEX, LADDER>(l, a, en, grid, block, stream);
  }
  return hipErrorInvalidValue;
}

template <typename R, class Energy>
hipError_t step_with(const StepLaunch &l, const Energy &en, hipStream_t stream) {
  const StepArgs<R> a = typed<R>(l);
  const bool per_chain = l.cov_kind == CK_PER_CHAIN;
  const int threads = (l.n_sweeps >= kFusedSweepsThreshold || (ME_PER_CHAIN == 2 && per_chain)) ? kFusedStepThreads : kStepThreads;
  const dim3 grid(grid_for(l.n, l.grid_blocks, threads)), block(threads);
  if (l.ladder) {
    if (l.inj_normals) return hipErrorNotSupported;
#if ME_DENSE && !defined(ME_USER_SOURCE)
    if constexpr (NR == 64 && NC == 0 && std::is_same<Energy, EnergyDense<R, 64, 0>>::value) return hipErrorNotSupported;
    else
#endif
      return launch_step_group<R, Energy, false, true>(l, a, en, grid, block, stream);
  }
  if (l.inj_normals) {
    if constexpr (std::is_same<R, double>::value) return launch_step_group<R, Energy, true>(l, a, en, grid, block, stream);
    else return hipErrorNotSupported;
  }
#if ME_DENSE && !defined(ME_USER_SOURCE)
  if constexpr (std::is_same<R, float>::value && NR == 64 && NC == 0 &&
                std::is_same<Energy, EnergyDense<float, 64, 0>>::value) {
    if (per_chain) return launch_step_group<R, Energy, false>(l, a, en, grid, block, stream);
    if (dense64_exact_fp32_mfma()) {
      if (l.cov_kind == CK_IDENTITY)
        return launch_step_dense64_mfma<CK_IDENTITY>(a, en.a, nullptr, l.grid_blocks, stream);
      if (l.cov_kind == CK_SHARED && l.factor_full)
        return launch_step_dense64_mfma<CK_SHARED>(a, en.a, (const float *)l.factor_full, l.grid_blocks, stream);
      return hipErrorInvalidValue;
    }
    if (!l.energy_image) return hipErrorInvalidValue;
    if (l.cov_kind == CK_IDENTITY)
      return launch_step_dense64_bf16x3<CK_IDENTITY>(a, (const unsigned int *)l.energy_image, nullptr, l.grid_blocks, stream);
    if (l.cov_kind == CK_SHARED && l.factor_image)
      return launch_step_dense64_bf16x3<CK_SHARED>(a, (const unsigned int *)l.energy_image,
// ... 234 lines not shown
  return hipGetLastError();
}

#ifdef ME_USER_SOURCE
#define ME_SET_NAME ME_USER_NAME
#else
#define ME_SET_NAME nullptr
#endif
constexpr auto pool_stage1_f32() -> hipError_t (*)(const void *, long long, double *, int, hipStream_t) {
  if constexpr (NR == 64 && NC == 0) return launch_pool_gram64;
  else if constexpr (D + NR + NC <= 32) return launch_pool_gram32<NR, NC>;
  else return nullptr;
}
constexpr auto pool_stage1_f64() -> hipError_t (*)(const void *, long long, double *, int, hipStream_t) {
  if constexpr (NR == 64 && NC == 0) return launch_pool_gram64_f64;
  else if constexpr (D + NR + NC <= 32) return launch_pool_gram32_f64<NR, NC>;
  else return nullptr;
}
#if ME_DENSE && !defined(ME_USER_SOURCE)
hipError_t prepare_matrix_f32(const void *factor_full, void *image, hipStream_t stream) {
  if constexpr (NR == 64 && NC == 0) {
    hipLaunchKernelGGL(k_dense64_bf16_fragments<0>, dim3(1), dim3(256), 0, stream, (const float *)factor_full,
                       (unsigned int *)image);
    return hipGetLastError();
  }
  return hipSuccess;
}
[[maybe_unused]] constexpr size_t kMatrixImageBytes = (NR == 64 && NC == 0) ? sizeof(unsigned int) * kBf16FragWords : 0;
#define ME_PREPARE_MATRIX_F32 kMatrixImageBytes, (kMatrixImageBytes ? prepare_matrix_f32 : nullptr), pool_stage1_f32()
hipError_t prepare_matrix_f64(const void *matrix, void *image, hipStream_t stream) {
  if constexpr (NR == 64 && NC == 0) {
    hipLaunchKernelGGL(k_dense64_f64_fragments<0>, dim3(1), dim3(256), 0, stream, (const double *)matrix, (double *)image);
    return hipGetLastError();
  }
  return hipSuccess;
}
[[maybe_unused]] constexpr size_t kMatrixImageBytesF64 = (NR == 64 && NC == 0) ? sizeof(double) * kDense64F64ImageDoubles : 0;
#define ME_PREPARE_MATRIX_F64 kMatrixImageBytesF64, (kMatrixImageBytesF64 ? prepare_matrix_f64 : nullptr), pool_stage1_f64()
#else
#define ME_PREPARE_MATRIX_F32 0, nullptr, pool_stage1_f32()
#define ME_PREPARE_MATRIX_F64 0, nullptr, pool_stage1_f64()
#endif
#ifdef ME_USER_HAS_REJECT
constexpr bool kHasUserReject = true;
#else
constexpr bool kHasUserReject = false;
#endif
#ifndef ME_ONLY_DTYPE
#define ME_ONLY_DTYPE 0
#endif
#if ME_ONLY_DTYPE != 64
const KernelSet kSetF32 = {ME_SET_NAME, ME_F32, NR, NC, ME_PER_CHAIN != 0, (ME_PER_CHAIN != 0 || ME_TRACK_COV != 0), has_energy, energy_terms, step<float>,
                           (NC > 0 && ME_PER_CHAIN == 1) ? magphase<float> : nullptr, measure<float>, init_energy<float>,
                           ME_PREPARE_MATRIX_F32, kHasUserReject, ME_PER_CHAIN == 2, cycle<float>, D >= kTiledStateDof};
#endif
#if ME_ONLY_DTYPE != 32
const KernelSet kSetF64 = {ME_SET_NAME, ME_F64, NR, NC, ME_PER_CHAIN != 0, (ME_PER_CHAIN != 0 || ME_TRACK_COV != 0), has_energy, energy_terms, step<double>,
                           (NC > 0 && ME_PER_CHAIN == 1) ? magphase<double> : nullptr, measure<double>, init_energy<double>,
                           ME_PREPARE_MATRIX_F64, kHasUserReject, ME_PER_CHAIN == 2, cycle<double>, D >= kTiledStateDof};
#endif

struct Registrar {
  Registrar() {
#if ME_ONLY_DTYPE != 64
    register_kernel_set(&kSetF32);
#endif
#if ME_ONLY_DTYPE != 32
    register_kernel_set(&kSetF64);
#endif
  }
} registrar;

}
}
```

### metropolisengine_amd/csrc/me_pool_gram.h

```cpp
#pragma once

#include "me_dense_mfma.h"
#include "me_dense_f64.h"
#include "me_per_device.h"

namespace me {

constexpr int kGramWaves = 2;
constexpr int kGramPitch = 65;

template <int UNUSED = 0>
__global__ void __launch_bounds__(64 * kGramWaves) k_pool_gram64(const float *__restrict__ x, long long n,
                                                                 double *__restrict__ partials, int n_rows) {
  constexpr int D = 64;
  constexpr int n_aug = 2 * D;
  constexpr int n_entries = 1 + n_aug + D * (D + 1) / 2;
  __shared__ float slab[kGramWaves][D * kGramPitch];
  const int lane = threadIdx.x & 63, wave = threadIdx.x >> 6;
  const int row_id = blockIdx.x * kGramWaves + wave;
  if (row_id >= n_rows) return;
  float *tile = slab[wave];
  const int r31 = lane & 31, h = lane >> 5;

  double g[3][16];
// ... 253 lines not shown
      if (v - 1024 < n_aug) out[1 + (v - 1024)] = s;
    } else {
      const int r = v >> 6, l = v & 63;
      const int i = acc_row(r) + 4 * (l >> 5), j = l & 31;
      if (i < D && j <= i) out[1 + n_aug + i * (i + 1) / 2 + j] = s;
    }
  }
}

template <int NR, int NC>
inline hipError_t launch_pool_gram32(const void *x, long long n, double *partials, int n_rows, hipStream_t stream) {
  constexpr size_t lds = (size_t)kSmallWavesF32 * kSmallSlabBytesF32;
  static PerDevice<int> raised;
  int device = 0;
  hipError_t err = hipGetDevice(&device);
  if (err != hipSuccess) return err;
  if (raised.get(device, [&]() -> int {
        return hipFuncSetAttribute((const void *)k_pool_gram32<NR, NC>, hipFuncAttributeMaxDynamicSharedMemorySize, (int)lds) == hipSuccess ? 1 : -1;
      }) < 0)
    return hipErrorInvalidValue;
  hipLaunchKernelGGL((k_pool_gram32<NR, NC>), dim3((unsigned)n_rows), dim3(64 * kSmallWavesF32), lds, stream, (const float *)x, n, partials, n_rows);
  return hipGetLastError();
}

template <int NR, int NC>
__global__ void __launch_bounds__(64 * kSmallWavesF64) k_pool_gram32_f64(const double *__restrict__ x, long long n,
                                                                         double *__restrict__ partials, int n_rows) {
  constexpr int D = NR + 2 * NC;
  constexpr int n_aug = D + NR + NC;
  static_assert(n_aug <= 32, "two 16-row MFMA blocks");
  static_assert(897 * 8 <= kSmallSlabBytesF64, "slab holds the sums");
  constexpr int n_entries = 1 + n_aug + D * (D + 1) / 2;
  extern __shared__ __attribute__((aligned(16))) unsigned char small_lds[];
  const int lane = threadIdx.x & 63, wave = threadIdx.x >> 6;
  double *tile = reinterpret_cast<double *>(small_lds + (size_t)wave * kSmallSlabBytesF64);
  const int j = lane & 15, h = lane >> 4;
#pragma unroll
  for (int r = n_aug; r < 32; ++r) tile[r * kSmallPitchF64 + lane] = 0.0;

  f64x4 acc[3];
#pragma unroll
  for (int b = 0; b < 3; ++b) acc[b] = f64x4{0.0, 0.0, 0.0, 0.0};
  double sum_row[2] = {0.0, 0.0}, count = 0.0;

  const long long n_tiles = (n + 63) / 64;
  const long long first = (long long)blockIdx.x * kSmallWavesF64 + wave, step = (long long)n_rows * kSmallWavesF64;
  double next[D];
  auto request = [&](long long t) {
    const long long c = t * 64 + lane;
    const bool live = t < n_tiles && c < n;
    const long long cc = live ? c : 0;
#pragma unroll
    for (int d = 0; d < D; ++d) {
      const double v = x[state_index<double, D>(cc, d, n)];
      next[d] = live ? v : 0.0;
    }
  };
  request(first);
  for (long long t = first; t < n_tiles; t += step) {
#pragma unroll
    for (int d = 0; d < D; ++d) tile[d * kSmallPitchF64 + lane] = next[d];
#pragma unroll
    for (int i = 0; i < NR; ++i) tile[(D + i) * kSmallPitchF64 + lane] = __builtin_fabs(next[i]);
#pragma unroll
    for (int k = 0; k < NC; ++k)
      tile[(D + NR + k) * kSmallPitchF64 + lane] = sqrt(next[NR + k] * next[NR + k] + next[NR + NC + k] * next[NR + NC + k]);
    request(t + step);
    count += (double)(n - t * 64 < 64 ? n - t * 64 : 64);
    __builtin_amdgcn_wave_barrier();
#pragma unroll 4
    for (int s = 0; s < 16; ++s) {
      double f[2];
#pragma unroll
      for (int b = 0; b < 2; ++b) {
        f[b] = tile[(16 * b + j) * kSmallPitchF64 + 4 * s + h];
        sum_row[b] += f[b];
      }
      acc[0] = __builtin_amdgcn_mfma_f64_16x16x4f64(f[0], f[0], acc[0], 0, 0, 0);
      acc[1] = __builtin_amdgcn_mfma_f64_16x16x4f64(f[1], f[0], acc[1], 0, 0, 0);
      acc[2] = __builtin_amdgcn_mfma_f64_16x16x4f64(f[1], f[1], acc[2], 0, 0, 0);
    }
    __builtin_amdgcn_wave_barrier();
  }
#pragma unroll
  for (int b = 0; b < 2; ++b) {
    sum_row[b] += __shfl_xor(sum_row[b], 16);
    sum_row[b] += __shfl_xor(sum_row[b], 32);
  }
  double *red = reinterpret_cast<double *>(small_lds + (size_t)wave * kSmallSlabBytesF64);
#pragma unroll
  for (int b = 0; b < 3; ++b)
#pragma unroll
    for (int r = 0; r < 4; ++r) red[64 * (4 * b + r) + lane] = acc[b][r];
  red[768 + lane] = sum_row[0];
  red[832 + lane] = sum_row[1];
  if (lane == 0) red[896] = count;
  __syncthreads();
  double *out = partials + (long long)blockIdx.x * n_entries;
  for (int v = threadIdx.x; v < 897; v += 64 * kSmallWavesF64) {
    double s = 0.0;
#pragma unroll
    for (int w = 0; w < kSmallWavesF64; ++w) s += reinterpret_cast<const double *>(small_lds + (size_t)w * kSmallSlabBytesF64)[v];
    if (v == 896) {
      out[0] = s;
    } else if (v >= 768) {
      const int b = (v - 768) >> 6, l = (v - 768) & 63;
      if (l < 16 && 16 * b + l < n_aug) out[1 + 16 * b + l] = s;
// ... 26 lines not shown
```

### metropolisengine_amd/csrc/me_population.hip

```cpp
#include <algorithm>
#include <cmath>
#include <vector>

#include "me_device.h"
#include "me_engine.h"

namespace me {
namespace {

constexpr int kPopThreads = 256;
constexpr int kPopWaves = kPopThreads / 64;
constexpr int kPopItems = 8;
constexpr int kPopChunk = kPopThreads * kPopItems;
constexpr int kFinalThreads = 256;
constexpr long long kSerialSlots = 8;

struct PopParams {
  double M, W, u;
  long long hi;
  long long n_finite;
};

template <typename R>
__device__ __forceinline__ double chain_log_weight(const Field<R> &fe, long long c, long long n, int n_terms, double neg_dbeta,
// ... 204 lines not shown
      if (c < n) ancestors[c] = (unsigned int)c;
    }
    return;
  }
  const Field<R> fe(energy, n, n_terms);
  const double m = partials[4 * (size_t)blockIdx.x], f = factors[blockIdx.x], o = offsets[blockIdx.x];
  const double N = (double)n;
  double l[kPopItems];
  bool ok[kPopItems];
#pragma unroll
  for (int r = 0; r < kPopItems; ++r) l[r] = chain_log_weight(fe, base + r * kPopThreads + threadIdx.x, n, n_terms, neg_dbeta, ok[r]);
  double carry = 0.0, prev;
#pragma unroll
  for (int r = 0; r < kPopItems; ++r) {
    const double v = ok[r] ? exp(l[r] - m) : 0.0;
    const double q = round_running_sum(v, carry, prev, wave_tot, wave_last);
    const long long c = base + r * kPopThreads + threadIdx.x;
    long long lo = 0, up = 0;
    if (q > prev) {
      lo = slot_bound(o + f * prev, N, p.W, p.u, p.hi);
      up = slot_bound(o + f * q, N, p.W, p.u, p.hi);
    }
    const bool long_run = up - lo > kSerialSlots;
    if (!long_run)
      for (long long j = lo; j < up; ++j) ancestors[j] = (unsigned int)c;
    unsigned long long runs = __ballot(long_run);
    while (runs) {
      const int src = __ffsll((long long)runs) - 1;
      runs &= runs - 1;
      const long long run_lo = __shfl(lo, src), run_up = __shfl(up, src);
      const unsigned int run_c = (unsigned int)__shfl(c, src);
      for (long long j = run_lo + (threadIdx.x & 63); j < run_up; j += 64) ancestors[j] = run_c;
    }
  }
}

template <class F>
__device__ __forceinline__ void copy_rows(const F &src, const F &dst, unsigned int src_off, unsigned int dst_off, int rows) {
  constexpr int B = 8;
  for (int r0 = 0; r0 < rows; r0 += B) {
    decltype(src.load(0, 0u)) v[B];
#pragma unroll
    for (int k = 0; k < B; ++k)
      if (r0 + k < rows) v[k] = src.load(r0 + k, src_off);
#pragma unroll
    for (int k = 0; k < B; ++k)
      if (r0 + k < rows) dst.store(r0 + k, dst_off, v[k]);
  }
}

template <typename R>
__global__ void __launch_bounds__(kPopThreads) k_pop_gather(const R *x, const R *energy, const long long *fam, R *x_out,
                                                           R *energy_out, long long *fam_out, long long n, int d, int n_terms,
                                                           int tiled, const unsigned int *ancestors, const PopParams *params) {
  const long long j = (long long)blockIdx.x * kPopThreads + threadIdx.x;
  if (j >= n) return;
  const long long hi = params->hi;
  const long long a = (long long)ancestors[j < hi ? j : hi - 1];
  const unsigned int a_off = (unsigned int)a * (unsigned int)sizeof(R), j_off = (unsigned int)j * (unsigned int)sizeof(R);
  if (tiled) copy_rows(TiledField<R>(x, n, d), TiledField<R>(x_out, n, d), tiled_offset<R>(a, d), tiled_offset<R>(j, d), d);
  else copy_rows(Field<R>(x, n, d), Field<R>(x_out, n, d), a_off, j_off, d);
  copy_rows(Field<R>(energy, n, n_terms), Field<R>(energy_out, n, n_terms), a_off, j_off, n_terms);
  fam_out[j] = fam[a];
}

__global__ void __launch_bounds__(kPopThreads) k_pop_init_families(long long *fam, long long n, unsigned long long chain_offset) {
  const long long j = (long long)blockIdx.x * kPopThreads + threadIdx.x;
  if (j < n) fam[j] = (long long)(chain_offset + (unsigned long long)j);
}

template <typename R>
hipError_t launch(me_engine *e, double neg_dbeta) {
  me_engine::Population &pop = e->population;
  const long long n = e->n;
  hipStream_t stream = e->stream;
  const int n_blocks = (int)((n + kPopChunk - 1) / kPopChunk);
  const unsigned slot_blocks = (unsigned)((n + kPopThreads - 1) / kPopThreads);
  double *partials = pop.scratch.get<double>(), *factors = partials + 4 * (size_t)n_blocks, *offsets = factors + n_blocks;
  PopParams *params = (PopParams *)(offsets + n_blocks + 1);
  double *record = pop.records.get<double>() + 3 * (size_t)pop.stages;
  hipLaunchKernelGGL(k_pop_weights<R>, dim3(n_blocks), dim3(kPopThreads), 0, stream, e->energy.get<const R>(), n, e->n_terms,
                     neg_dbeta, partials);
  hipLaunchKernelGGL(k_pop_finalize, dim3(1), dim3(kFinalThreads), 0, stream, (const double *)partials, n_blocks, n,
                     e->chain_offset, pop.stages, (uint32_t)e->seed, (uint32_t)(e->seed >> 32), factors, offsets, params, record);
  hipLaunchKernelGGL(k_pop_scan_ancestors<R>, dim3(n_blocks), dim3(kPopThreads), 0, stream, e->energy.get<const R>(), n,
                     e->n_terms, neg_dbeta, (const double *)partials, (const double *)factors, (const double *)offsets,
                     (const PopParams *)params, pop.anc.get<unsigned int>());
  hipLaunchKernelGGL(k_pop_gather<R>, dim3(slot_blocks), dim3(kPopThreads), 0, stream, e->x.get<const R>(), e->energy.get<const R>(),
                     pop.fam.get<const long long>(), pop.x.get<R>(), pop.energy.get<R>(), pop.fam_out.get<long long>(), n, e->d,
                     e->n_terms, e->x_tiled ? 1 : 0, pop.anc.get<const unsigned int>(), (const PopParams *)params);
  return hipGetLastError();
}

size_t population_scratch_doubles(long long n) {
  const long long n_blocks = (n + kPopChunk - 1) / kPopChunk;
  return (size_t)(4 * n_blocks + n_blocks + n_blocks + 1) + (sizeof(PopParams) + sizeof(double) - 1) / sizeof(double);
}

int ensure_families(me_engine *e) {
  me_engine::Population &pop = e->population;
  if (pop.fam) return ME_OK;
  ME_HIP(e, pop.fam.resize((size_t)e->n * sizeof(long long)));
  hipLaunchKernelGGL(k_pop_init_families, dim3((unsigned)((e->n + kPopThreads - 1) / kPopThreads)), dim3(kPopThreads), 0, e->stream,
                     pop.fam.get<long long>(), e->n, e->chain_offset);
  ME_HIP(e, hipGetLastError());
  return ME_OK;
}
int ensure_population_scratch(me_engine *e) {
  me_engine::Population &pop = e->population;
  const size_t energy_bytes = (size_t)e->n * (size_t)e->n_terms * e->esize;
  if (pop.energy.bytes() < energy_bytes) {
    if (pop.energy) ME_HIP(e, hipStreamSynchronize(e->stream));
    ME_HIP(e, pop.energy.reserve(energy_bytes));
  }
  if (!pop.x) {
    ME_HIP(e, pop.x.resize(e->x.bytes()));
    ME_HIP(e, hipMemcpyAsync(pop.x.get(), e->x.get(), pop.x.bytes(), hipMemcpyDeviceToDevice, e->stream));
  }
  ME_HIP(e, pop.fam_out.resize((size_t)e->n * sizeof(long long)));
  ME_HIP(e, pop.anc.resize((size_t)e->n * sizeof(unsigned int)));
  ME_HIP(e, pop.scratch.resize(population_scratch_doubles(e->n) * sizeof(double)));
  return ME_OK;
}
int ensure_records(me_engine *e, unsigned long long stages) {
  me_engine::Population &pop = e->population;
  if (stages <= pop.capacity) return ME_OK;
  unsigned long long cap = std::max<unsigned long long>(256, pop.capacity);
  while (cap < stages) cap *= 2;
  DeviceBuffer grown;
  ME_HIP(e, grown.resize((size_t)cap * 3 * sizeof(double)));
  if (pop.records) {
    ME_HIP(e, hipMemcpyAsync(grown.get(), pop.records.get(), (size_t)pop.stages * 3 * sizeof(double), hipMemcpyDeviceToDevice, e->stream));
    ME_HIP(e, hipStreamSynchronize(e->stream));
  }
  pop.records = std::move(grown);
  pop.capacity = cap;
  return ME_OK;
}
int check_family_range(me_engine *e, int64_t chain_begin, int64_t n) {
  if (chain_begin < 0 || n < 0 || chain_begin + n > e->n) return fail(e, ME_ERR_INVALID, "family range outside the engine's chains");
  return ME_OK;
}

// ... 109 lines not shown
```

### metropolisengine_amd/csrc/me_replica.hip

```cpp
#include <algorithm>
#include <cmath>
#include <string>
#include <vector>

#include "me_device.h"
#include "me_engine.h"

namespace me {
namespace {

constexpr int kSwapThreads = 256;
constexpr int kSwapBlocks = 2048;

template <typename R>
struct SwapArgs {
  R *x, *energy;
  const R *ladder;
  unsigned long long *pair_counts;
  long long n, rung_chains;
  unsigned long long chain_offset, round;
  uint32_t seed_lo, seed_hi;
  int d, n_terms, first_rung, tiled;
};

template <class F>
__device__ __forceinline__ void swap_rows(const F &f, unsigned int off_a, unsigned int off_b, int rows) {
  constexpr int B = 8;
  for (int r0 = 0; r0 < rows; r0 += B) {
    decltype(f.load(0, 0u)) va[B], vb[B];
#pragma unroll
    for (int u = 0; u < B; ++u)
      if (r0 + u < rows) {
        va[u] = f.load(r0 + u, off_a);
        vb[u] = f.load(r0 + u, off_b);
      }
#pragma unroll
    for (int u = 0; u < B; ++u)
      if (r0 + u < rows) {
        f.store(r0 + u, off_a, vb[u]);
        f.store(r0 + u, off_b, va[u]);
      }
  }
}

template <typename R>
__device__ __forceinline__ bool swap_pair(const SwapArgs<R> &s, const Field<R> &fe, int k, long long j, R dbeta, R dbeta_log2e) {
  using N_ = Num<R>;
  const long long a = (long long)k * s.rung_chains + j, b = a + s.rung_chains;
  const unsigned int ea_off = (unsigned int)a * (unsigned int)sizeof(R), eb_off = (unsigned int)b * (unsigned int)sizeof(R);
  const R ea = chain_energy(fe, ea_off, s.n_terms), eb = chain_energy(fe, eb_off, s.n_terms);
  const unsigned long long gid = s.chain_offset + (unsigned long long)a;
  U4 ctr;
  ctr.x = (uint32_t)gid;
  ctr.y = (uint32_t)(gid >> 32);
  ctr.z = (uint32_t)s.round;
  ctr.w = ((uint32_t)(s.round >> 32) << 16) | 0xffffu;
  const R u = N_::unit(philox4x32_10(ctr, s.seed_lo, s.seed_hi).x);
  const R delta = dbeta * (ea - eb);
  const bool accept = N_::finite(ea) && N_::finite(eb) && (delta >= R(0) || N_::uphill(u, eb - ea, dbeta, dbeta_log2e));
  if (accept) {
    if (s.tiled) swap_rows(TiledField<R>(s.x, s.n, s.d), tiled_offset<R>(a, s.d), tiled_offset<R>(b, s.d), s.d);
    else swap_rows(Field<R>(s.x, s.n, s.d), ea_off, eb_off, s.d);
    swap_rows(fe, ea_off, eb_off, s.n_terms);
  }
  return accept;
}

template <typename R>
__global__ void __launch_bounds__(kSwapThreads) k_replica_swap(SwapArgs<R> s) {
  const int k = s.first_rung + 2 * (int)blockIdx.y;
  const Field<R> fe(s.energy, s.n, s.n_terms);
  const R dbeta = s.ladder[2 * k] - s.ladder[2 * k + 2], dbeta_log2e = s.ladder[2 * k + 1] - s.ladder[2 * k + 3];
  unsigned int attempted = 0, accepted = 0;
  for (long long j = (long long)blockIdx.x * kSwapThreads + threadIdx.x; j < s.rung_chains; j += (long long)gridDim.x * kSwapThreads) {
    const bool acc = swap_pair(s, fe, k, j, dbeta, dbeta_log2e);
    attempted += (unsigned int)__popcll(__ballot(true));
    accepted += (unsigned int)__popcll(__ballot(acc));
  }
  __shared__ unsigned int wave_counts[kSwapThreads / 64][2];
  if ((threadIdx.x & 63) == 0) {
    wave_counts[threadIdx.x >> 6][0] = attempted;
    wave_counts[threadIdx.x >> 6][1] = accepted;
  }
  __syncthreads();
  if (threadIdx.x < 2) {
    unsigned long long total = 0;
#pragma unroll
    for (int w = 0; w < kSwapThreads / 64; ++w) total += wave_counts[w][threadIdx.x];
    if (total) atomicAdd(&s.pair_counts[2 * k + threadIdx.x], total);
  }
}

template <typename R>
hipError_t launch(void *x, void *energy, long long n, int d, int n_terms, bool tiled_state, const void *ladder, int n_rungs,
                  unsigned long long round, unsigned long long chain_offset, unsigned long long seed,
                  unsigned long long *pair_counts, hipStream_t stream) {
  SwapArgs<R> s;
  s.x = (R *)x;
  s.energy = (R *)energy;
  s.ladder = (const R *)ladder;
  s.pair_counts = pair_counts;
  s.n = n;
  s.rung_chains = n / n_rungs;
  s.first_rung = (int)(round & 1ull);
  const int n_pairs = (n_rungs - s.first_rung) / 2;
  s.chain_offset = chain_offset;
  s.round = round;
  s.seed_lo = (uint32_t)seed;
  s.seed_hi = (uint32_t)(seed >> 32);
  s.d = d;
  s.n_terms = n_terms;
  s.tiled = tiled_state ? 1 : 0;
  if (n_pairs == 0) return hipSuccess;
  const long long per_pair = std::min<long long>((s.rung_chains + kSwapThreads - 1) / kSwapThreads, std::max(kSwapBlocks / n_pairs, 1));
  hipLaunchKernelGGL(k_replica_swap<R>, dim3((unsigned)per_pair, (unsigned)n_pairs), dim3(kSwapThreads), 0, stream, s);
  return hipGetLastError();
}

int check_ladder_capable(me_engine *e) {
  if (e->ks->n_real < 0)
    return fail(e, ME_ERR_UNSUPPORTED, "temperature ladders are not available on the runtime-dimension kernel set (beyond " +
                                           std::to_string(kMaxRegisterDof) + " real degrees of freedom)");
  if (e->energy_kind == ME_ENERGY_DENSE_QUAD && e->nr == 64 && e->nc == 0)
    return fail(e, ME_ERR_UNSUPPORTED, "temperature ladders are not available on the matrix-core kernels of the dense 64-parameter form");
  return refuse_stale_total(e, "temperature ladders are");
}
int free_ladder(me_engine *e) {
  ME_HIP(e, hipStreamSynchronize(e->stream));
  e->ladder = me_engine::Ladder();
  e->samples.rows = 0;
  return ME_OK;
}
}
}

using namespace me;

extern "C" {

int me_set_temperature_ladder(me_engine *e, const double *temps, int32_t n_rungs) {
  if (!e) return ME_ERR_INVALID;
  if (n_rungs < 0 || (n_rungs > 0 && !temps)) return fail(e, ME_ERR_INVALID, "n_rungs must be >= 0 and temps given");
  ME_HIP(e, hipSetDevice(e->device));
  if (n_rungs == 0) return free_ladder(e);
  int rc = check_ladder_capable(e);
  if (rc != ME_OK) return rc;
  for (int k = 0; k < n_rungs; ++k) {
    if (!(std::isfinite(temps[k]) && temps[k] > 0))
      return fail(e, ME_ERR_INVALID, "ladder temperatures must be finite and > 0");
    if (k > 0 && !(temps[k] > temps[k - 1]))
      return fail(e, ME_ERR_INVALID, "ladder temperatures must be strictly increasing");
  }
  if (e->n % (64ll * n_rungs) != 0)
    return fail(e, ME_ERR_INVALID, "n_chains must be a multiple of 64 * n_rungs: every rung is a run of whole 64-chain tiles");
  std::vector<double> table(2 * (size_t)n_rungs);
  for (int k = 0; k < n_rungs; ++k) {
    table[2 * k] = 1.0 / temps[k];
    table[2 * k + 1] = 1.4426950408889634 / temps[k];
  }
  if ((rc = free_ladder(e)) != ME_OK) return rc;
  ME_HIP(e, upload(e->ladder.table, table.data(), table.size(), e->dtype));
  ME_HIP(e, e->ladder.pair_counts.resize(2 * (size_t)std::max(n_rungs - 1, 1) * sizeof(unsigned long long)));
  ME_HIP(e, hipMemset(e->ladder.pair_counts.get(), 0, e->ladder.pair_counts.bytes()));
  e->ladder.temps.assign(temps, temps + n_rungs);
  e->ladder.n_rungs = n_rungs;
  return ME_OK;
}

int me_temperature_ladder(me_engine *e, double *temps, int32_t capacity, int32_t *n_rungs) {
  if (!e || !n_rungs) return ME_ERR_INVALID;
  *n_rungs = e->ladder.n_rungs;
  if (e->ladder.n_rungs == 0 || !temps) return ME_OK;
  if (capacity < e->ladder.n_rungs) return fail(e, ME_ERR_INVALID, "temps must hold n_rungs doubles");
  std::copy(e->ladder.temps.begin(), e->ladder.temps.end(), temps);
  return ME_OK;
}

int me_replica_exchange(me_engine *e, int32_t n_rounds) {
  if (!e) return ME_ERR_INVALID;
  if (n_rounds < 0) return fail(e, ME_ERR_INVALID, "n_rounds must be >= 0");
  if (e->ladder.n_rungs == 0) return fail(e, ME_ERR_STATE, "no temperature ladder: call me_set_temperature_ladder first");
  ME_HIP(e, hipSetDevice(e->device));
  const auto swap = e->dtype == ME_F32 ? launch<float> : launch<double>;
  for (int i = 0; i < n_rounds; ++i) {
    ME_HIP(e, swap(e->x.get(), e->energy.get(), e->n, e->d, e->n_terms, e->x_tiled, e->ladder.table.get(), e->ladder.n_rungs, e->ladder.round,
                   e->chain_offset, e->seed, e->ladder.pair_counts.get<unsigned long long>(), e->stream));
    e->ladder.round += 1;
  }
  return ME_OK;
}

int me_replica_stats(me_engine *e, uint64_t *round, uint64_t *attempted, uint64_t *accepted, int32_t n_pairs) {
  if (!e) return ME_ERR_INVALID;
  if (e->ladder.n_rungs == 0) return fail(e, ME_ERR_STATE, "no temperature ladder");
  if (n_pairs != e->ladder.n_rungs - 1) return fail(e, ME_ERR_INVALID, "n_pairs must be n_rungs - 1");
  if (round) *round = e->ladder.round;
  if (n_pairs == 0) return ME_OK;
  ME_HIP(e, hipSetDevice(e->device));
  std::vector<unsigned long long> counts(2 * (size_t)n_pairs);
  ME_HIP(e, hipMemcpyAsync(counts.data(), e->ladder.pair_counts.get(), counts.size() * sizeof(unsigned long long), hipMemcpyDeviceToHost,
                           e->stream));
  ME_HIP(e, hipStreamSynchronize(e->stream));
  for (int k = 0; k < n_pairs; ++k) {
    if (attempted) attempted[k] = counts[2 * k];
    if (accepted) accepted[k] = counts[2 * k + 1];
  }
  return ME_OK;
}

int me_set_replica_stats(me_engine *e, uint64_t round, const uint64_t *attempted, const uint64_t *accepted, int32_t n_pairs) {
  if (!e) return ME_ERR_INVALID;
  if (e->ladder.n_rungs == 0) return fail(e, ME_ERR_STATE, "no temperature ladder");
  if (n_pairs != e->ladder.n_rungs - 1) return fail(e, ME_ERR_INVALID, "n_pairs must be n_rungs - 1");
  if (n_pairs > 0 && (!attempted || !accepted)) return fail(e, ME_ERR_INVALID, "attempted / accepted missing");
  std::vector<unsigned long long> counts(2 * (size_t)n_pairs);
  for (int k = 0; k < n_pairs; ++k) {
    if (accepted[k] > attempted[k]) return fail(e, ME_ERR_INVALID, "accepted swaps exceed attempted ones");
    counts[2 * k] = attempted[k];
    counts[2 * k + 1] = accepted[k];
  }
  ME_HIP(e, hipSetDevice(e->device));
  if (n_pairs > 0) {
    ME_HIP(e, hipMemcpyAsync(e->ladder.pair_counts.get(), counts.data(), counts.size() * sizeof(unsigned long long), hipMemcpyHostToDevice,
                             e->stream));
    ME_HIP(e, hipStreamSynchronize(e->stream));
  }
  e->ladder.round = round;
  return ME_OK;
}

}
```

Measured before the change: 18.98 billion.

## Store f64 16-parameter state chain-major with LDS-staged 128-byte line loads

Adds a chain-major state layout for f64 engines with 16 real parameters, enabled by default. Each chain's parameters then occupy one contiguous 128-byte line. A per-wave LDS staging path loads these lines with 128-bit buffer loads and transposes them into registers through a swizzled slab. On store, only the lines of chains whose proposal was accepted are written back. The aim is fully coalesced wide transfers and no write traffic for rejected chains, at the cost of LDS use, wave barriers and new host, replica and population paths for the layout.

```diff
diff --git a/metropolisengine_amd/csrc/me_api.hip b/metropolisengine_amd/csrc/me_api.hip
--- a/metropolisengine_amd/csrc/me_api.hip
+++ b/metropolisengine_amd/csrc/me_api.hip
@@ -8,6 +8,7 @@
 #include <string>
 #include <atomic>
 #include <chrono>
+#include <type_traits>
 #include <vector>
 
 #include "me_engine.h"
@@ -168,11 +169,12 @@
 
 namespace {
 
-int broadcast(me_engine *e, DeviceBuffer &dst, const std::vector<double> &row, bool tiled = false) {
+int broadcast(me_engine *e, DeviceBuffer &dst, const std::vector<double> &row, int layout = STATE_COMPONENT) {
   std::vector<unsigned char> bytes;
   to_device_type(row.data(), row.size(), e->dtype, bytes);
   ME_HIP(e, hipMemcpyAsync(e->row_dev.get(), bytes.data(), bytes.size(), hipMemcpyHostToDevice, e->stream));
-  if (tiled) ME_HIP(e, launch_broadcast_tiled(dst.get(), e->row_dev.get(), (int)row.size(), e->n, e->dtype, e->stream));
+  if (layout == STATE_CHAIN) ME_HIP(e, launch_broadcast_chains(dst.get(), e->row_dev.get(), (int)row.size(), e->n, e->dtype, e->stream));
+  else if (layout == STATE_TILED) ME_HIP(e, launch_broadcast_tiled(dst.get(), e->row_dev.get(), (int)row.size(), e->n, e->dtype, e->stream));
   else ME_HIP(e, launch_broadcast_rows(dst.get(), e->row_dev.get(), (int)row.size(), e->n, e->dtype, e->stream));
   ME_HIP(e, hipStreamSynchronize(e->stream));
   return ME_OK;
@@ -211,6 +213,30 @@
   }
   if (e->dtype == ME_F32) transpose_tiled(reinterpret_cast<float *>(tmp.data()), entries, tile0, chain_begin, n_chains, dst, src);
   else transpose_tiled(reinterpret_cast<double *>(tmp.data()), entries, tile0, chain_begin, n_chains, dst, src);
+  if (src) {
+    ME_HIP(e, hipMemcpyAsync(dev, tmp.data(), tmp.size(), hipMemcpyHostToDevice, e->stream));
+    ME_HIP(e, hipStreamSynchronize(e->stream));
+  }
+  return dst ? check_status(e) : ME_OK;
+}
+
+int copy_chains(me_engine *e, void *field_ptr, int rows, int64_t chain_begin, int64_t n_chains, double *dst, const double *src) {
+  const size_t n_values = (size_t)n_chains * rows;
+  unsigned char *dev = (unsigned char *)field_ptr + (size_t)chain_begin * rows * e->esize;
+  std::vector<unsigned char> tmp(n_values * e->esize);
+  auto convert = [&](auto *t) {
+    using T = std::remove_pointer_t<decltype(t)>;
+    for (size_t i = 0; i < n_values; ++i) {
+      if (dst) dst[i] = (double)t[i];
+      else t[i] = (T)src[i];
+    }
+  };
+  if (dst) {
+    ME_HIP(e, hipMemcpyAsync(tmp.data(), dev, tmp.size(), hipMemcpyDeviceToHost, e->stream));
+    ME_HIP(e, hipStreamSynchronize(e->stream));
+  }
+  if (e->dtype == ME_F32) convert(reinterpret_cast<float *>(tmp.data()));
+  else convert(reinterpret_cast<double *>(tmp.data()));
   if (src) {
     ME_HIP(e, hipMemcpyAsync(dev, tmp.data(), tmp.size(), hipMemcpyHostToDevice, e->stream));
     ME_HIP(e, hipStreamSynchronize(e->stream));
@@ -407,7 +433,7 @@
 struct Layout {
   bool keep_per_chain;
   bool keep_cov;
-  bool x_tiled;
+  int x_layout;
   int width_rows;
 };
 int decide_layout(const me_config *c, const KernelSet *ks, Layout &l) {
@@ -426,7 +452,7 @@
                 "a per-chain field would exceed 4 GiB on this engine; shard the chains over more engines");
   l.keep_cov = l.keep_per_chain ||
                ((!ks->per_chain_cov || ks->streams_packed) && ks->tracks_cov && (c->flags & ME_FLAG_TRACK_COVARIANCE));
-  l.x_tiled = ks->tiled_state;
+  l.x_layout = ks->state_layout;
   l.width_rows = (c->n_real > 0 && c->n_complex > 0) ? 3 : 1;
   return ME_OK;
 }
@@ -458,7 +484,7 @@
   e->ratio = (1.0 - 1.0 / e->m) * std::sqrt(2.0 * M_PI) * std::exp(e->alpha * e->alpha / 2.0) / 2.0 * e->alpha +
              1.0 / (e->m * c->target_acceptance * (1.0 - c->target_acceptance));
   if (const char *g = std::getenv("ME_GRID_BLOCKS")) e->grid_blocks = std::atoi(g);
-  e->x_tiled = l.x_tiled;
+  e->x_layout = l.x_layout;
   e->stale_total = (c->flags & ME_FLAG_REFERENCE_ENERGY_LEDGERS) != 0;
   e->width_rows = l.width_rows;
   e->n_slots = (e->n + 31) / 32 + 8;
@@ -470,7 +496,7 @@
   ME_HIP(e, hipSetDevice(e->device));
   ME_HIP(e, e->stream.create());
   const size_t n = (size_t)e->n, tiles = (size_t)padded_chains(e->n), es = e->esize;
-  ME_HIP(e, e->x.resize((e->x_tiled ? tiles : n) * e->d * es));
+  ME_HIP(e, e->x.resize((e->x_layout == STATE_TILED ? tiles : n) * e->d * es));
   ME_HIP(e, e->energy.resize(n * (e->n_terms + (e->stale_total ? 1 : 0)) * es));
   ME_HIP(e, e->width.resize(n * e->width_rows * es));
   ME_HIP(e, e->mean.resize(n * e->d * es));
@@ -560,7 +586,7 @@
     return fail(e, ME_ERR_INVALID, "initial covariance matrix is not positive definite (metropolis_engine.py:270)");
   int rc = ME_OK;
   std::vector<double> width_row((size_t)e->width_rows, c->sampling_width);
-  if ((rc = broadcast(e, e->x, init, e->x_tiled)) || (rc = broadcast(e, e->mean, init)) || (rc = broadcast(e, e->obs_mean, obs)) ||
+  if ((rc = broadcast(e, e->x, init, e->x_layout)) || (rc = broadcast(e, e->mean, init)) || (rc = broadcast(e, e->obs_mean, obs)) ||
       (rc = broadcast(e, e->width, width_row)) || (e->cov && (rc = broadcast(e, e->cov, c0, true))) ||
       (e->factor && (rc = broadcast(e, e->factor, f0, true))) || (rc = upload_shared_factor(e, f0.data())))
     return rc;
@@ -618,7 +644,7 @@
     return fail(e, ME_ERR_UNSUPPORTED, is_user_kind(energy_kind)
                     ? std::string("no user-energy plugin named '") + (user_name ? user_name : "") + "' is loaded for these dimensions"
                     : "energy kind " + std::to_string(energy_kind) + " is not compiled for these dimensions");
-  if (ks->tiled_state != e->ks->tiled_state || ks->per_chain_cov != e->ks->per_chain_cov || ks->streams_packed != e->ks->streams_packed ||
+  if (ks->state_layout != e->ks->state_layout || ks->per_chain_cov != e->ks->per_chain_cov || ks->streams_packed != e->ks->streams_packed ||
       ks->tracks_cov != e->ks->tracks_cov)
     return fail(e, ME_ERR_UNSUPPORTED, "me_set_energy: the plugin was built with other per-chain covariance options than this engine's kernel set");
   if (e->reject_kind == ME_REJECT_USER && !ks->has_user_reject)
@@ -813,7 +839,7 @@
     const int rows_valid = (e->width_rows == 3 && e->widths_synced) ? 1 : e->width_rows;
     double *row = e->trace.dev.get<double>() + e->trace.rows * cols * e->trace.chains;
     ME_HIP(e, launch_trace(e->x.get(), e->energy.get(), e->width.get(), e->n, e->d, e->n_terms, rows_valid, e->dtype, e->trace.chains,
-                           e->trace.stride, row, e->stream, e->x_tiled));
+                           e->trace.stride, row, e->stream, e->x_layout));
     if (rows_valid != e->width_rows) {
       double *widths = row + (size_t)(e->d + e->n_terms) * e->trace.chains;
       for (int r = 1; r < 3; ++r)
@@ -919,7 +945,8 @@
   int rc = field_info(e, field, &ptr, &comps);
   if (rc != ME_OK) return rc;
   if (n_chains == 0) return ME_OK;
-  if (field == ME_FIELD_COV || field == ME_FIELD_FACTOR || (field == ME_FIELD_PARAMS && e->x_tiled))
+  if (field == ME_FIELD_PARAMS && e->x_layout == STATE_CHAIN) return copy_chains(e, ptr, comps, chain_begin, n_chains, dst, nullptr);
+  if (field == ME_FIELD_COV || field == ME_FIELD_FACTOR || (field == ME_FIELD_PARAMS && e->x_layout == STATE_TILED))
     return copy_tiled(e, ptr, comps, chain_begin, n_chains, dst, nullptr);
   std::vector<unsigned char> tmp((size_t)comps * n_chains * e->esize);
   for (int r = 0; r < comps; ++r)
@@ -945,7 +972,8 @@
   if (field == ME_FIELD_WIDTH && e->width_rows == 3 && (chain_begin != 0 || n_chains != e->n))
     return fail(e, ME_ERR_INVALID, "widths of a mixed engine must be set for all chains at once");
   if (n_chains == 0) return ME_OK;
-  if (field == ME_FIELD_COV || field == ME_FIELD_FACTOR || (field == ME_FIELD_PARAMS && e->x_tiled)) {
+  if (field == ME_FIELD_PARAMS && e->x_layout == STATE_CHAIN) return copy_chains(e, ptr, comps, chain_begin, n_chains, nullptr, src);
+  if (field == ME_FIELD_COV || field == ME_FIELD_FACTOR || (field == ME_FIELD_PARAMS && e->x_layout == STATE_TILED)) {
     rc = copy_tiled(e, ptr, comps, chain_begin, n_chains, nullptr, src);
     if (rc != ME_OK) return rc;
     if (field == ME_FIELD_FACTOR) e->cov_kind = CK_PER_CHAIN;
@@ -1045,7 +1073,7 @@
 }
 int enqueue_pool_reduce(me_engine *e, const void *x, long long n_chains, long long n_slots, double proposed, double *device_out) {
   hipError_t err = launch_pool_reduce(x, n_chains, e->nr, e->nc, e->dtype, e->accept_slots.get<unsigned long long>(), n_slots, proposed,
-                                      e->pool.partials.get<double>(), device_out, e->stream, e->ks->pool_stage1, e->x_tiled);
+                                      e->pool.partials.get<double>(), device_out, e->stream, e->ks->pool_stage1, e->x_layout);
   if (err == hipErrorInvalidValue) return fail(e, ME_ERR_UNSUPPORTED, "pooled moments: dimension too large for the reduction kernel");
   ME_HIP(e, err);
   return ME_OK;
@@ -1084,7 +1112,7 @@
   int rc = check_pooled(e, n_doubles);
   if (rc != ME_OK) return rc;
   const unsigned char *x = e->x.get<unsigned char>();
-  if (e->x_tiled) {
+  if (e->x_layout != STATE_COMPONENT) {
     x += (size_t)chain_begin * e->d * e->esize;
   } else {
     const size_t row = (size_t)n_chains * e->esize;
diff --git a/metropolisengine_amd/csrc/me_device.h b/metropolisengine_amd/csrc/me_device.h
--- a/metropolisengine_amd/csrc/me_device.h
+++ b/metropolisengine_amd/csrc/me_device.h
@@ -224,29 +224,140 @@
 #define ME_TILED_STATE_DOF 16
 #endif
 constexpr int kTiledStateDof = ME_TILED_STATE_DOF;
-template <typename R, int D, bool NTS = false>
+#ifndef ME_CHAIN_MAJOR_STATE
+#define ME_CHAIN_MAJOR_STATE 1
+#endif
+constexpr int default_state_layout(int dof) { return dof >= kTiledStateDof ? STATE_TILED : STATE_COMPONENT; }
+template <typename R, int NR, int NC>
+constexpr int state_layout() {
+  if (ME_CHAIN_MAJOR_STATE != 0 && sizeof(R) == 8 && NR == 16 && NC == 0) return STATE_CHAIN;
+  return default_state_layout(NR + 2 * NC);
+}
+template <typename R>
+struct ChainField {
+  __amdgpu_buffer_rsrc_t rsrc;
+  __device__ __forceinline__ ChainField(const R *base, long long n, int d)
+      : rsrc(__builtin_amdgcn_make_buffer_rsrc(const_cast<R *>(base), 0, (unsigned int)(n * d * (long long)sizeof(R)), 0x00020000)) {}
+  template <int AUX>
+  __device__ __forceinline__ R load_aux(int row, unsigned int off) const {
+    if constexpr (sizeof(R) == 4) {
+      return __builtin_bit_cast(R, __builtin_amdgcn_raw_buffer_load_b32(rsrc, off, (unsigned int)row * 4u, AUX));
+    } else {
+      const auto v = __builtin_amdgcn_raw_buffer_load_b64(rsrc, off, (unsigned int)row * 8u, AUX);
+      return __builtin_bit_cast(R, v);
+    }
+  }
+  template <int AUX>
+  __device__ __forceinline__ void store_aux(int row, unsigned int off, R value) const {
+    if constexpr (sizeof(R) == 4) {
+      __builtin_amdgcn_raw_buffer_store_b32(__builtin_bit_cast(unsigned int, value), rsrc, off, (unsigned int)row * 4u, AUX);
+    } else {
+      using v2 = decltype(__builtin_amdgcn_raw_buffer_load_b64(rsrc, 0u, 0u, 0));
+      __builtin_amdgcn_raw_buffer_store_b64(__builtin_bit_cast(v2, value), rsrc, off, (unsigned int)row * 8u, AUX);
+    }
+  }
+  __device__ __forceinline__ R load(int row, unsigned int off) const { return load_aux<0>(row, off); }
+  __device__ __forceinline__ R load_nt(int row, unsigned int off) const { return load_aux<ME_NT_AUX>(row, off); }
+  __device__ __forceinline__ void store(int row, unsigned int off, R value) const { store_aux<0>(row, off, value); }
+  __device__ __forceinline__ void store_nt(int row, unsigned int off, R value) const { store_aux<ME_NT_AUX>(row, off, value); }
+};
+template <typename R, int D, bool NTS = false, int LAYOUT = default_state_layout(D)>
 struct XField {
-  static constexpr bool kTiled = D >= kTiledStateDof;
-  std::conditional_t<kTiled, TiledField<R>, StateField<R, NTS>> f;
+  static constexpr bool kTiled = LAYOUT == STATE_TILED;
+  static constexpr bool kChain = LAYOUT == STATE_CHAIN;
+  std::conditional_t<kChain, ChainField<R>, std::conditional_t<kTiled, TiledField<R>, StateField<R, NTS>>> f;
   __device__ __forceinline__ XField(const R *base, long long n) : f(base, n, D) {}
   static __device__ __forceinline__ unsigned int offset(long long c) {
-    if constexpr (kTiled) return tiled_offset<R>(c, D);
+    if constexpr (kChain) return (unsigned int)c * (unsigned int)(D * sizeof(R));
+    else if constexpr (kTiled) return tiled_offset<R>(c, D);
     else return (unsigned int)c * (unsigned int)sizeof(R);
   }
   __device__ __forceinline__ R load(int row, unsigned int off) const {
-    if constexpr (kTiled && NTS) return f.load_nt(row, off);
+    if constexpr ((kTiled || kChain) && NTS) return f.load_nt(row, off);
     else return f.load(row, off);
   }
   __device__ __forceinline__ void store(int row, unsigned int off, R value) const {
-    if constexpr (kTiled && NTS) f.store_nt(row, off, value);
+    if constexpr ((kTiled || kChain) && NTS) f.store_nt(row, off, value);
     else f.store(row, off, value);
   }
 };
-template <typename R, int D>
+template <typename R, int D, int LAYOUT = default_state_layout(D)>
 __device__ __forceinline__ long long state_index(long long c, int row, long long n) {
-  if constexpr (D >= kTiledStateDof) return ((c >> 6) * (long long)D + row) * 64 + (c & 63);
+  if constexpr (LAYOUT == STATE_CHAIN) return c * (long long)D + row;
+  else if constexpr (LAYOUT == STATE_TILED) return ((c >> 6) * (long long)D + row) * 64 + (c & 63);
   else return (long long)row * n + c;
 }
+
+constexpr int kLineSlabBytes = 8192, kLineWaveLds = kLineSlabBytes + 64;
+extern __shared__ __attribute__((aligned(16))) unsigned char me_line_lds[];
+typedef unsigned int me_u32x4 __attribute__((ext_vector_type(4)));
+template <typename R, int D, bool NTS>
+struct LineStage {
+  static_assert(sizeof(R) == 8 && D == 16, "one chain = one 128-byte line");
+  static constexpr int kAux = NTS ? ME_NT_AUX : 0;
+  struct Pair { R a, b; };
+  __amdgpu_buffer_rsrc_t rsrc;
+  me_u32x4 *slab;
+  unsigned char *list;
+  int lane;
+  __device__ __forceinline__ LineStage(const R *base, long long n)
+      : rsrc(__builtin_amdgcn_make_buffer_rsrc(const_cast<R *>(base), 0, (unsigned int)(n * 128), 0x00020000)),
+        slab((me_u32x4 *)(me_line_lds + (threadIdx.x >> 6) * kLineWaveLds)),
+        list(me_line_lds + (threadIdx.x >> 6) * kLineWaveLds + kLineSlabBytes),
+        lane((int)(threadIdx.x & 63u)) {}
+  static __device__ __forceinline__ int swz(int ch) { return (ch & 7) ^ ((ch >> 4) & 1); }
+  static __device__ __forceinline__ void wave_sync() {
+    __builtin_amdgcn_fence(__ATOMIC_ACQ_REL, "wavefront");
+    __builtin_amdgcn_wave_barrier();
+  }
+  __device__ __forceinline__ int lane_here() const {
+    int l = lane;
+    asm volatile("" : "+v"(l));
+    return l;
+  }
+  static __device__ __forceinline__ unsigned int tile_base(long long c) {
+    return (unsigned int)__builtin_amdgcn_readfirstlane((int)(unsigned int)(c >> 6)) * (unsigned int)kLineSlabBytes;
+  }
+  __device__ __forceinline__ void load(long long c, R (&x)[D]) const {
+    const unsigned int base = tile_base(c);
+    const int lane = lane_here();
+    me_u32x4 in[8];
+#pragma unroll
+    for (int k = 0; k < 8; ++k) in[k] = __builtin_amdgcn_raw_buffer_load_b128(rsrc, base + (unsigned int)lane * 16u + k * 1024u, 0u, kAux);
+#pragma unroll
+    for (int k = 0; k < 8; ++k) {
+      const int ch = k * 8 + (lane >> 3);
+      slab[ch * 8 + ((lane & 7) ^ swz(ch))] = in[k];
+    }
+    wave_sync();
+#pragma unroll
+    for (int j = 0; j < 8; ++j) {
+      const Pair p = __builtin_bit_cast(Pair, slab[lane * 8 + (j ^ swz(lane))]);
+      x[2 * j] = p.a;
+      x[2 * j + 1] = p.b;
+    }
+    wave_sync();
+  }
+  __device__ __forceinline__ void store(long long c, const R (&x)[D], bool changed) const {
+    const unsigned int base = tile_base(c);
+    const int lane = lane_here();
+#pragma unroll
+    for (int j = 0; j < 8; ++j) slab[lane * 8 + (j ^ swz(lane))] = __builtin_bit_cast(me_u32x4, Pair{x[2 * j], x[2 * j + 1]});
+    const unsigned long long m = __ballot(changed);
+    if (changed) list[__builtin_amdgcn_mbcnt_hi((unsigned int)(m >> 32), __builtin_amdgcn_mbcnt_lo((unsigned int)m, 0u))] = (unsigned char)lane;
+    wave_sync();
+    const int count = __popcll(m);
+    for (int i = 0; i * 8 < count; ++i) {
+      const int slot = i * 8 + (lane >> 3);
+      if (slot < count) {
+        const int ch = list[slot];
+        const me_u32x4 q = slab[ch * 8 + ((lane & 7) ^ swz(ch))];
+        __builtin_amdgcn_raw_buffer_store_b128(q, rsrc, base + (unsigned int)(ch * 128 + (lane & 7) * 16), 0u, kAux);
+      }
+    }
+    wave_sync();
+  }
+};
 
 constexpr int kMaxPackedInRegisters = 160;
 #ifndef ME_STREAM_F64_ENTRIES
@@ -609,7 +720,7 @@
 __device__ __forceinline__ void decide_step(const StepArgs<R> &a, long long c, const Energy &en, bool stale_total, R u,
                                             const R (&g)[2 * ((NR + 2 * NC + 1) / 2)], R (&x)[NR + 2 * NC], const R (&xp)[NR + 2 * NC],
                                             Ledger &ledger, R &total_q5, R &w, R &w_r, R &w_c, unsigned int &wave_accepted,
-                                            bool &bad_energy) {
+                                            bool &bad_energy, bool &changed) {
   [[maybe_unused]] constexpr int D = NR + 2 * NC;
   constexpr bool MOVE_REAL = NR > 0 && GROUP != GROUP_COMPLEX;
   constexpr bool MOVE_COMPLEX = NC > 0 && GROUP != GROUP_REAL;
@@ -649,19 +760,20 @@
   else if constexpr (GROUP == GROUP_REAL) w_r = w;
   else w_c = w;
   wave_accepted += (unsigned int)__popcll(__ballot(accept));
+  changed |= accept;
 }
 
 template <typename R, int NR, int NC, class Energy, int CK, bool INJECT, int GROUP, bool LADDER, class Ledger, class Fac>
 __device__ __forceinline__ void run_sweeps(const StepArgs<R> &a, const Energy &en, long long c, unsigned long long gid,
                                            bool stale_total, R (&x)[NR + 2 * NC], Ledger &ledger, R &total_q5, R &w, R &w_r,
-                                           R &w_c, Fac &&fac, unsigned int &wave_accepted, bool &bad_energy) {
+                                           R &w_c, Fac &&fac, unsigned int &wave_accepted, bool &bad_energy, bool &changed) {
   constexpr int D = NR + 2 * NC;
   constexpr int NW = 2 * ((D + 1) / 2);
   for (int s = 0; s < a.n_sweeps; ++s) {
     R g[NW], u, xp[D];
     draw_step<R, NR, NC, INJECT>(a, c, gid, s, g, u);
     propose_registers<R, NR, NC, CK, GROUP>(x, g, w_r, w_c, fac, xp);
-    decide_step<R, NR, NC, Energy, CK, GROUP, LADDER>(a, c, en, stale_total, u, g, x, xp, ledger, total_q5, w, w_r, w_c, wave_accepted, bad_energy);
+    decide_step<R, NR, NC, Energy, CK, GROUP, LADDER>(a, c, en, stale_total, u, g, x, xp, ledger, total_q5, w, w_r, w_c, wave_accepted, bad_energy, changed);
   }
 }
 
@@ -703,7 +815,8 @@
   bool bad_energy = false, bad_width = false;
   const long long stride = (long long)gridDim.x * blockDim.x;
   using Ledger = EnergyLedger<R, Energy, GROUP>;
-  const XField<R, D, NTS> fx(a.x, a.n);
+  constexpr bool LINE = state_layout<R, NR, NC>() == STATE_CHAIN;
+  const std::conditional_t<LINE, LineStage<R, LINE ? D : 16, NTS>, XField<R, D, NTS, state_layout<R, NR, NC>()>> fx(a.x, a.n);
   const StateField<R, NTS> fe(a.energy, a.n, Ledger::T + (MIXED ? 1 : 0)), fw(a.width, a.n, MIXED ? 3 : 1);
   const bool stale_total = MIXED && GROUP == GROUP_ALL && a.stale_total != 0;
   constexpr bool PER_CHAIN = CK == CK_PER_CHAIN || CK == CK_PER_CHAIN_NT;
@@ -711,12 +824,19 @@
   constexpr bool STREAM_FACTOR = PER_CHAIN && (PF > kMaxPackedInRegisters ||
                                                (!INJECT && sizeof(R) == 8 && NC == 0 && PF > kStreamF64Entries));
   const TiledField<R> ffac(a.factor, a.n, STREAM_FACTOR ? 0 : PF);
-  for (long long c = (long long)blockIdx.x * blockDim.x + threadIdx.x; c < a.n; c += stride) {
+  for (long long c = (long long)blockIdx.x * blockDim.x + threadIdx.x; LINE ? c - (long long)(threadIdx.x & 63u) < a.n : c < a.n; c += stride) {
     const unsigned int coff = (unsigned int)c * (unsigned int)sizeof(R);
-    const unsigned int xoff = fx.offset(c);
     R x[D];
-#pragma unroll
-    for (int d = 0; d < D; ++d) x[d] = fx.load(d, xoff);
+    [[maybe_unused]] unsigned int xoff = 0;
+    if constexpr (LINE) {
+      fx.load(c, x);
+    } else {
+      xoff = fx.offset(c);
+#pragma unroll
+      for (int d = 0; d < D; ++d) x[d] = fx.load(d, xoff);
+    }
+    bool changed = false;
+    if (!LINE || c < a.n) {
     Ledger ledger;
     R total_q5 = R(0);
     if (stale_total) total_q5 = fe.load(Ledger::T, coff);
@@ -847,16 +967,21 @@
         else if constexpr (GROUP == GROUP_REAL) w_r = w;
         else w_c = w;
         wave_accepted += (unsigned int)__popcll(__ballot(accept));
+        changed |= accept;
       }
     } else {
-      run_sweeps<R, NR, NC, Energy, CK, INJECT, GROUP, LADDER>(a, en, c, gid, stale_total, x, ledger, total_q5, w, w_r, w_c, fac, wave_accepted, bad_energy);
+      run_sweeps<R, NR, NC, Energy, CK, INJECT, GROUP, LADDER>(a, en, c, gid, stale_total, x, ledger, total_q5, w, w_r, w_c, fac, wave_accepted, bad_energy, changed);
     }
     bad_width |= !(w > R(0));
-#pragma unroll
-    for (int d = 0; d < D; ++d) fx.store(d, xoff, x[d]);
+    if constexpr (!LINE) {
+#pragma unroll
+      for (int d = 0; d < D; ++d) fx.store(d, xoff, x[d]);
+    }
     if (stale_total) fe.store(Ledger::T, coff, total_q5);
     else ledger.store(fe, coff);
     fw.store(MIXED ? GROUP : 0, coff, w);
+    }
+    if constexpr (LINE) fx.store(c, x, changed);
   }
   if ((threadIdx.x & 63) == 0 && wave_accepted) {
     unsigned long long *slot = a.accept_slots + (size_t)blockIdx.x * (blockDim.x >> 6) + (threadIdx.x >> 6);
@@ -875,7 +1000,7 @@
   for (long long c = (long long)blockIdx.x * kStepThreads + threadIdx.x; c < n; c += stride) {
     R x[D];
 #pragma unroll
-    for (int d = 0; d < D; ++d) x[d] = xs[state_index<R, D>(c, d, n)];
+    for (int d = 0; d < D; ++d) x[d] = xs[state_index<R, D, state_layout<R, NR, NC>()>(c, d, n)];
     constexpr int T = term_count<Energy>::value;
     bool finite = true;
     R total = R(0);
@@ -1131,7 +1256,7 @@
   constexpr int NOBS = 2 * NR + NC;
   bool bad_pivot = false;
   const long long stride = (long long)gridDim.x * kStepThreads;
-  const XField<R, D> fx(a.x, a.n);
+  const XField<R, D, false, state_layout<R, NR, NC>()> fx(a.x, a.n);
   const Field<R> fw(a.width, a.n, (NR > 0 && NC > 0) ? 3 : 1), fmean(a.mean, a.n, D), fobs(a.obs_mean, a.n, NOBS);
   constexpr bool STREAM = PER_CHAIN_COV && P > kMaxPackedInRegisters;
   const TiledField<R> fcov(a.cov, a.n, (PER_CHAIN_COV && !STREAM) ? P : 0);
@@ -1174,7 +1299,7 @@
   bool bad_energy = false, bad_width = false, bad_pivot = false;
   const long long stride = (long long)gridDim.x * blockDim.x;
   using Ledger = EnergyLedger<R, Energy, GROUP_ALL>;
-  const XField<R, D> fx(a.x, a.n);
+  const XField<R, D, false, state_layout<R, NR, NC>()> fx(a.x, a.n);
   const Field<R> fe(a.energy, a.n, Ledger::T + (MIXED ? 1 : 0)), fw(a.width, a.n, MIXED ? 3 : 1);
   const Field<R> fmean(ma.mean, a.n, D), fobs(ma.obs_mean, a.n, NOBS);
   const TiledField<R> fcov(ma.cov, a.n, P), ffac(ma.factor, a.n, P);
@@ -1198,6 +1323,7 @@
       }
     }
     const unsigned long long gid = a.chain_offset + (unsigned long long)c;
+    [[maybe_unused]] bool changed = false;
     [[maybe_unused]] const unsigned int toff = tiled_offset<R>(c, P);
     auto fac = [&](int k) -> R {
       if constexpr (CK == CK_PER_CHAIN) return packed_load<NT>(ffac, k, toff);
@@ -1218,7 +1344,7 @@
       }
     }
     run_sweeps<R, NR, NC, Energy, CKX, false, GROUP_ALL, LADDER>(a, en, c, gid, stale_total, x, ledger, total_q5, w, w_r, w_c, fac,
-                                                         wave_accepted, bad_energy);
+                                                         wave_accepted, bad_energy, changed);
     bad_width |= !(w > R(0));
 #pragma unroll
     for (int d = 0; d < D; ++d) fx.store(d, xoff, x[d]);
diff --git a/metropolisengine_amd/csrc/me_engine.h b/metropolisengine_amd/csrc/me_engine.h
--- a/metropolisengine_amd/csrc/me_engine.h
+++ b/metropolisengine_amd/csrc/me_engine.h
@@ -142,7 +142,7 @@
   me::DeviceBuffer accept_slots, accept_total;
   long long n_slots = 0;
   unsigned long long proposed = 0;
-  bool x_tiled = false;
+  int x_layout = me::STATE_COMPONENT;
   int width_rows = 1;
   bool widths_synced = true;
   me::DeviceBuffer status;
diff --git a/metropolisengine_amd/csrc/me_generic.hip b/metropolisengine_amd/csrc/me_generic.hip
--- a/metropolisengine_amd/csrc/me_generic.hip
+++ b/metropolisengine_amd/csrc/me_generic.hip
@@ -16,6 +16,12 @@
   const long long total = n_padded * entries, stride = (long long)gridDim.x * kBlockThreads;
   for (long long i = (long long)blockIdx.x * kBlockThreads + threadIdx.x; i < total; i += stride)
     dst[i] = entry_values[(i >> 6) % entries];
+}
+
+template <typename R>
+__global__ void __launch_bounds__(kBlockThreads) k_broadcast_chains(R *dst, const R *row_values, int rows, long long n) {
+  const long long total = n * rows, stride = (long long)gridDim.x * kBlockThreads;
+  for (long long i = (long long)blockIdx.x * kBlockThreads + threadIdx.x; i < total; i += stride) dst[i] = row_values[i % rows];
 }
 
 __device__ __forceinline__ void pair_of(int p, int &i, int &j) {
@@ -28,7 +34,7 @@
 constexpr int kMaxEntries = 12;
 
 template <typename R, int TILE>
-__global__ void __launch_bounds__(kBlockThreads) k_pool_reduce(const R *x, long long n, int nr, int nc, int entry_base, int tiled, double *partials) {
+__global__ void __launch_bounds__(kBlockThreads) k_pool_reduce(const R *x, long long n, int nr, int nc, int entry_base, int layout, double *partials) {
   extern __shared__ __attribute__((aligned(16))) unsigned char smem_raw[];
   R *tile = reinterpret_cast<R *>(smem_raw);
   constexpr int kTilePitch = TILE + 1;
@@ -37,7 +43,7 @@
   const int n_pair = d * (d + 1) / 2;
   const int n_entries = 1 + n_aug + n_pair;
   const int tid = threadIdx.x;
-  auto at = [&](int r, long long c) -> long long { return tiled ? ((c >> 6) * (long long)d + r) * 64 + (c & 63) : (long long)r * n + c; };
+  auto at = [&](int r, long long c) -> long long { return state_at(layout, c, r, d, n); };
 
   int row_i[kMaxEntries], row_j[kMaxEntries];
   bool active[kMaxEntries];
@@ -196,6 +202,19 @@
   return hipGetLastError();
 }
 
+hipError_t launch_broadcast_chains(void *dst, const void *row_values, int rows, long long n, int dtype, hipStream_t stream) {
+  long long blocks = (n * rows + kBlockThreads - 1) / kBlockThreads;
+  if (blocks > 8192) blocks = 8192;
+  if (blocks < 1) blocks = 1;
+  if (dtype == ME_F32)
+    hipLaunchKernelGGL(k_broadcast_chains<float>, dim3((unsigned)blocks), dim3(kBlockThreads), 0, stream, (float *)dst,
+                       (const float *)row_values, rows, n);
+  else
+    hipLaunchKernelGGL(k_broadcast_chains<double>, dim3((unsigned)blocks), dim3(kBlockThreads), 0, stream, (double *)dst,
+                       (const double *)row_values, rows, n);
+  return hipGetLastError();
+}
+
 constexpr int kSumThreads = 1024;
 __global__ void __launch_bounds__(kSumThreads) k_sum_slots(const unsigned long long *slots, long long n_slots,
                                                            unsigned long long *total) {
@@ -225,12 +244,12 @@
 template <typename R>
 __global__ void __launch_bounds__(kBlockThreads) k_trace(const R *x, const R *energy, const R *width, long long n, int d,
                                                          int n_terms, int width_rows, long long n_traced, long long stride,
-                                                         int tiled, double *out) {
+                                                         int layout, double *out) {
   const long long t = (long long)blockIdx.x * kBlockThreads + threadIdx.x;
   if (t >= n_traced) return;
   const long long c = t * stride;
   for (int k = 0; k < d; ++k)
-    out[(long long)k * n_traced + t] = (double)x[tiled ? ((c >> 6) * (long long)d + k) * 64 + (c & 63) : (long long)k * n + c];
+    out[(long long)k * n_traced + t] = (double)x[state_at(layout, c, k, d, n)];
   for (int k = 0; k < n_terms; ++k) out[(long long)(d + k) * n_traced + t] = (double)energy[(long long)k * n + c];
   for (int r = 0; r < width_rows; ++r)
     out[(long long)(d + n_terms + r) * n_traced + t] = (double)width[(long long)r * n + c];
@@ -238,14 +257,14 @@
 
 hipError_t launch_trace(const void *x, const void *energy, const void *width, long long n, int d, int n_terms,
                         int width_rows, int dtype, long long n_traced, long long stride, double *out, hipStream_t stream,
-                        bool tiled_state) {
+                        int state_layout) {
   const dim3 grid((unsigned)((n_traced + kBlockThreads - 1) / kBlockThreads)), block(kBlockThreads);
   if (dtype == ME_F32)
     hipLaunchKernelGGL(k_trace<float>, grid, block, 0, stream, (const float *)x, (const float *)energy, (const float *)width,
-                       n, d, n_terms, width_rows, n_traced, stride, tiled_state ? 1 : 0, out);
+                       n, d, n_terms, width_rows, n_traced, stride, state_layout, out);
   else
     hipLaunchKernelGGL(k_trace<double>, grid, block, 0, stream, (const double *)x, (const double *)energy,
-                       (const double *)width, n, d, n_terms, width_rows, n_traced, stride, tiled_state ? 1 : 0, out);
+                       (const double *)width, n, d, n_terms, width_rows, n_traced, stride, state_layout, out);
   return hipGetLastError();
 }
 
@@ -279,7 +298,7 @@
 
 namespace {
 template <typename R, int TILE>
-hipError_t launch_pool_stage1(const void *x, long long n, int nr, int nc, int n_entries, int blocks, double *partials, hipStream_t stream, bool tiled) {
+hipError_t launch_pool_stage1(const void *x, long long n, int nr, int nc, int n_entries, int blocks, double *partials, hipStream_t stream, int layout) {
   const size_t lds = (size_t)(nr + 2 * nc + nr + nc) * (size_t)(TILE + 1) * sizeof(R);
   if (lds > 64 * 1024) {
     static PerDevice<hipError_t> attr;
@@ -292,15 +311,15 @@
   }
   for (int base = 0; base < n_entries; base += kMaxEntries * kBlockThreads)
     hipLaunchKernelGGL((k_pool_reduce<R, TILE>), dim3((unsigned)blocks), dim3(kBlockThreads), lds, stream, (const R *)x, n, nr, nc, base,
-                       tiled ? 1 : 0, partials);
-  return hipGetLastError();
-}
-template <typename R>
-hipError_t launch_pool_stage1_tile(int tile, const void *x, long long n, int nr, int nc, int n_entries, int blocks, double *partials, hipStream_t stream, bool tiled) {
+                       layout, partials);
+  return hipGetLastError();
+}
+template <typename R>
+hipError_t launch_pool_stage1_tile(int tile, const void *x, long long n, int nr, int nc, int n_entries, int blocks, double *partials, hipStream_t stream, int layout) {
   switch (tile) {
-    case 64: return launch_pool_stage1<R, 64>(x, n, nr, nc, n_entries, blocks, partials, stream, tiled);
-    case 32: return launch_pool_stage1<R, 32>(x, n, nr, nc, n_entries, blocks, partials, stream, tiled);
-    case 16: return launch_pool_stage1<R, 16>(x, n, nr, nc, n_entries, blocks, partials, stream, tiled);
+    case 64: return launch_pool_stage1<R, 64>(x, n, nr, nc, n_entries, blocks, partials, stream, layout);
+    case 32: return launch_pool_stage1<R, 32>(x, n, nr, nc, n_entries, blocks, partials, stream, layout);
+    case 16: return launch_pool_stage1<R, 16>(x, n, nr, nc, n_entries, blocks, partials, stream, layout);
     default: return hipErrorInvalidValue;
   }
 }
@@ -309,7 +328,7 @@
 hipError_t launch_pool_reduce(const void *x, long long n, int nr, int nc, int dtype, const unsigned long long *slots,
                               long long n_slots, double proposed, double *partials, double *out_device,
                               hipStream_t stream,
-                              hipError_t (*stage1)(const void *, long long, double *, int, hipStream_t), bool tiled_state) {
+                              hipError_t (*stage1)(const void *, long long, double *, int, hipStream_t), int state_layout) {
   const int d = nr + 2 * nc;
   const int n_aug = d + nr + nc;
   const int n_entries = 1 + n_aug + d * (d + 1) / 2;
@@ -318,8 +337,8 @@
   const int blocks = pool_reduce_blocks(n, nr, nc);
   hipError_t err;
   if (stage1) err = stage1(x, n, partials, blocks, stream);
-  else if (dtype == ME_F32) err = launch_pool_stage1_tile<float>(tile, x, n, nr, nc, n_entries, blocks, partials, stream, tiled_state);
-  else err = launch_pool_stage1_tile<double>(tile, x, n, nr, nc, n_entries, blocks, partials, stream, tiled_state);
+  else if (dtype == ME_F32) err = launch_pool_stage1_tile<float>(tile, x, n, nr, nc, n_entries, blocks, partials, stream, state_layout);
+  else err = launch_pool_stage1_tile<double>(tile, x, n, nr, nc, n_entries, blocks, partials, stream, state_layout);
   if (err != hipSuccess) return err;
   hipLaunchKernelGGL(k_pool_finish, dim3((unsigned)((n_entries + 63) / 64 + 1)), dim3(kFinishThreads), 0, stream,
                      (const double *)partials, blocks, nr, nc, slots, n_slots, proposed, out_device);
diff --git a/metropolisengine_amd/csrc/me_internal.h b/metropolisengine_amd/csrc/me_internal.h
--- a/metropolisengine_amd/csrc/me_internal.h
+++ b/metropolisengine_amd/csrc/me_internal.h
@@ -10,6 +10,12 @@
 enum CovKind { CK_IDENTITY = 0, CK_SHARED = 1, CK_PER_CHAIN = 2, CK_PER_CHAIN_NT = 3 };
 
 enum StepGroup { GROUP_ALL = 0, GROUP_REAL = 1, GROUP_COMPLEX = 2 };
+enum StateLayout { STATE_COMPONENT = 0, STATE_TILED = 1, STATE_CHAIN = 2 };
+__host__ __device__ inline long long state_at(int layout, long long c, int row, int d, long long n) {
+  return layout == STATE_CHAIN ? c * (long long)d + row
+         : layout == STATE_TILED ? ((c >> 6) * (long long)d + row) * 64 + (c & 63)
+                                 : (long long)row * n + c;
+}
 
 enum StatusBits : uint32_t {
   ST_NONFINITE_ENERGY = 1u,
@@ -97,7 +103,7 @@
   bool has_user_reject;
   bool streams_packed;
   hipError_t (*cycle)(const StepLaunch &, const MeasureLaunch &, hipStream_t);
-  bool tiled_state;
+  int state_layout;
 };
 
 void register_kernel_set(const KernelSet *set);
@@ -108,16 +114,18 @@
                                  hipStream_t stream);
 hipError_t launch_broadcast_tiled(void *dst, const void *entry_values, int entries, long long n, int dtype,
                                   hipStream_t stream);
+hipError_t launch_broadcast_chains(void *dst, const void *row_values, int rows, long long n, int dtype,
+                                   hipStream_t stream);
 hipError_t launch_pool_reduce(const void *x, long long n, int n_real, int n_complex, int dtype,
                               const unsigned long long *slots, long long n_slots, double proposed, double *partials,
                               double *out_device, hipStream_t stream,
                               hipError_t (*stage1)(const void *, long long, double *, int, hipStream_t) = nullptr,
-                              bool tiled_state = false);
+                              int state_layout = STATE_COMPONENT);
 int pool_reduce_blocks(long long n, int n_real, int n_complex);
 bool pool_reduce_supported(int n_real, int n_complex, int dtype);
 hipError_t launch_trace(const void *x, const void *energy, const void *width, long long n, int d, int n_terms,
                         int width_rows, int dtype, long long n_traced, long long stride, double *out, hipStream_t stream,
-                        bool tiled_state = false);
+                        int state_layout = STATE_COMPONENT);
 hipError_t launch_sum_slots(const unsigned long long *slots, long long n_slots, unsigned long long *total,
                             hipStream_t stream);
 
diff --git a/metropolisengine_amd/csrc/me_kernels.hip b/metropolisengine_amd/csrc/me_kernels.hip
--- a/metropolisengine_amd/csrc/me_kernels.hip
+++ b/metropolisengine_amd/csrc/me_kernels.hip
@@ -149,23 +149,24 @@
 template <typename R, class Energy, bool INJECT, int GROUP, bool LADDER>
 hipError_t launch_step_cov(const StepLaunch &l, const StepArgs<R> &a, const Energy &en, dim3 grid, dim3 block,
                            hipStream_t stream) {
+  const size_t lds = state_layout<R, NR, NC>() == STATE_CHAIN ? (size_t)(block.x / 64) * kLineWaveLds : 0;
   switch (l.cov_kind) {
     case CK_IDENTITY: {
       constexpr long long state_bytes = (long long)sizeof(R) * (D + 2);
       if constexpr (!INJECT && GROUP == GROUP_ALL && !LADDER) {
         if (state_bytes * l.n > 2 * cache_budget_bytes()) {
-          hipLaunchKernelGGL((k_step<R, NR, NC, Energy, CK_IDENTITY, INJECT, GROUP, true>), grid, block, 0, stream, a, en);
+          hipLaunchKernelGGL((k_step<R, NR, NC, Energy, CK_IDENTITY, INJECT, GROUP, true>), grid, block, lds, stream, a, en);
           break;
         }
       }
-      hipLaunchKernelGGL((k_step<R, NR, NC, Energy, CK_IDENTITY, INJECT, GROUP, false, LADDER>), grid, block, 0, stream, a, en);
+      hipLaunchKernelGGL((k_step<R, NR, NC, Energy, CK_IDENTITY, INJECT, GROUP, false, LADDER>), grid, block, lds, stream, a, en);
       break;
     }
-    case CK_SHARED: hipLaunchKernelGGL((k_step<R, NR, NC, Energy, CK_SHARED, INJECT, GROUP, false, LADDER>), grid, block, 0, stream, a, en); break;
+    case CK_SHARED: hipLaunchKernelGGL((k_step<R, NR, NC, Energy, CK_SHARED, INJECT, GROUP, false, LADDER>), grid, block, lds, stream, a, en); break;
 #if ME_PER_CHAIN == 2
     case CK_PER_CHAIN: {
       if constexpr (INJECT) return hipErrorInvalidValue;
-      else hipLaunchKernelGGL((k_step<R, NR, NC, Energy, CK_PER_CHAIN_NT, INJECT, GROUP, false, LADDER>), grid, block, 0, stream, a, en);
+      else hipLaunchKernelGGL((k_step<R, NR, NC, Energy, CK_PER_CHAIN_NT, INJECT, GROUP, false, LADDER>), grid, block, lds, stream, a, en);
       break;
     }
 #elif ME_PER_CHAIN
@@ -173,11 +174,11 @@
       constexpr long long per_chain_bytes = (long long)sizeof(R) * (D + 2 + NR * (NR + 1) / 2 + NC * NC);
       if constexpr (!INJECT) {
         if (per_chain_bytes * l.n > cache_budget_bytes()) {
-          hipLaunchKernelGGL((k_step<R, NR, NC, Energy, CK_PER_CHAIN_NT, INJECT, GROUP, false, LADDER>), grid, block, 0, stream, a, en);
+          hipLaunchKernelGGL((k_step<R, NR, NC, Energy, CK_PER_CHAIN_NT, INJECT, GROUP, false, LADDER>), grid, block, lds, stream, a, en);
           break;
         }
       }
-      hipLaunchKernelGGL((k_step<R, NR, NC, Energy, CK_PER_CHAIN, INJECT, GROUP, false, LADDER>), grid, block, 0, stream, a, en);
+      hipLaunchKernelGGL((k_step<R, NR, NC, Energy, CK_PER_CHAIN, INJECT, GROUP, false, LADDER>), grid, block, lds, stream, a, en);
       break;
     }
 #endif
@@ -518,12 +519,12 @@
 #if ME_ONLY_DTYPE != 64
 const KernelSet kSetF32 = {ME_SET_NAME, ME_F32, NR, NC, ME_PER_CHAIN != 0, (ME_PER_CHAIN != 0 || ME_TRACK_COV != 0), has_energy, energy_terms, step<float>,
                            (NC > 0 && ME_PER_CHAIN == 1) ? magphase<float> : nullptr, measure<float>, init_energy<float>,
-                           ME_PREPARE_MATRIX_F32, kHasUserReject, ME_PER_CHAIN == 2, cycle<float>, D >= kTiledStateDof};
+                           ME_PREPARE_MATRIX_F32, kHasUserReject, ME_PER_CHAIN == 2, cycle<float>, state_layout<float, NR, NC>()};
 #endif
 #if ME_ONLY_DTYPE != 32
 const KernelSet kSetF64 = {ME_SET_NAME, ME_F64, NR, NC, ME_PER_CHAIN != 0, (ME_PER_CHAIN != 0 || ME_TRACK_COV != 0), has_energy, energy_terms, step<double>,
                            (NC > 0 && ME_PER_CHAIN == 1) ? magphase<double> : nullptr, measure<double>, init_energy<double>,
-                           ME_PREPARE_MATRIX_F64, kHasUserReject, ME_PER_CHAIN == 2, cycle<double>, D >= kTiledStateDof};
+                           ME_PREPARE_MATRIX_F64, kHasUserReject, ME_PER_CHAIN == 2, cycle<double>, state_layout<double, NR, NC>()};
 #endif
 
 struct Registrar {
diff --git a/metropolisengine_amd/csrc/me_pool_gram.h b/metropolisengine_amd/csrc/me_pool_gram.h
--- a/metropolisengine_amd/csrc/me_pool_gram.h
+++ b/metropolisengine_amd/csrc/me_pool_gram.h
@@ -329,7 +329,7 @@
     const long long cc = live ? c : 0;
 #pragma unroll
     for (int d = 0; d < D; ++d) {
-      const double v = x[state_index<double, D>(cc, d, n)];
+      const double v = x[state_index<double, D, state_layout<double, NR, NC>()>(cc, d, n)];
       next[d] = live ? v : 0.0;
     }
   };
diff --git a/metropolisengine_amd/csrc/me_population.hip b/metropolisengine_amd/csrc/me_population.hip
--- a/metropolisengine_amd/csrc/me_population.hip
+++ b/metropolisengine_amd/csrc/me_population.hip
@@ -280,16 +280,35 @@
 template <typename R>
 __global__ void __launch_bounds__(kPopThreads) k_pop_gather(const R *x, const R *energy, const long long *fam, R *x_out,
                                                            R *energy_out, long long *fam_out, long long n, int d, int n_terms,
-                                                           int tiled, const unsigned int *ancestors, const PopParams *params) {
+                                                           int layout, const unsigned int *ancestors, const PopParams *params) {
   const long long j = (long long)blockIdx.x * kPopThreads + threadIdx.x;
   if (j >= n) return;
   const long long hi = params->hi;
   const long long a = (long long)ancestors[j < hi ? j : hi - 1];
   const unsigned int a_off = (unsigned int)a * (unsigned int)sizeof(R), j_off = (unsigned int)j * (unsigned int)sizeof(R);
-  if (tiled) copy_rows(TiledField<R>(x, n, d), TiledField<R>(x_out, n, d), tiled_offset<R>(a, d), tiled_offset<R>(j, d), d);
+  if (layout == STATE_CHAIN) copy_rows(ChainField<R>(x, n, d), ChainField<R>(x_out, n, d), (unsigned int)a * (unsigned int)(d * sizeof(R)), (unsigned int)j * (unsigned int)(d * sizeof(R)), d);
+  else if (layout == STATE_TILED) copy_rows(TiledField<R>(x, n, d), TiledField<R>(x_out, n, d), tiled_offset<R>(a, d), tiled_offset<R>(j, d), d);
   else copy_rows(Field<R>(x, n, d), Field<R>(x_out, n, d), a_off, j_off, d);
   copy_rows(Field<R>(energy, n, n_terms), Field<R>(energy_out, n, n_terms), a_off, j_off, n_terms);
   fam_out[j] = fam[a];
+}
+
+template <typename R>
+__global__ void __launch_bounds__(kPopThreads) k_pop_gather_lines(const R *x, const R *energy, const long long *fam, R *x_out,
+                                                                 R *energy_out, long long *fam_out, long long n, int n_terms,
+                                                                 const unsigned int *ancestors, const PopParams *params) {
+  const long long t = (long long)blockIdx.x * kPopThreads + threadIdx.x;
+  const long long j = t >> 3;
+  const int part = (int)(t & 7);
+  if (j >= n) return;
+  const long long hi = params->hi;
+  const long long a = (long long)ancestors[j < hi ? j : hi - 1];
+  reinterpret_cast<uint4 *>(x_out)[j * 8 + part] = reinterpret_cast<const uint4 *>(x)[a * 8 + part];
+  if (part == 0) {
+    const unsigned int a_off = (unsigned int)a * (unsigned int)sizeof(R), j_off = (unsigned int)j * (unsigned int)sizeof(R);
+    copy_rows(Field<R>(energy, n, n_terms), Field<R>(energy_out, n, n_terms), a_off, j_off, n_terms);
+    fam_out[j] = fam[a];
+  }
 }
 
 __global__ void __launch_bounds__(kPopThreads) k_pop_init_families(long long *fam, long long n, unsigned long long chain_offset) {
@@ -314,9 +333,15 @@
   hipLaunchKernelGGL(k_pop_scan_ancestors<R>, dim3(n_blocks), dim3(kPopThreads), 0, stream, e->energy.get<const R>(), n,
                      e->n_terms, neg_dbeta, (const double *)partials, (const double *)factors, (const double *)offsets,
                      (const PopParams *)params, pop.anc.get<unsigned int>());
-  hipLaunchKernelGGL(k_pop_gather<R>, dim3(slot_blocks), dim3(kPopThreads), 0, stream, e->x.get<const R>(), e->energy.get<const R>(),
-                     pop.fam.get<const long long>(), pop.x.get<R>(), pop.energy.get<R>(), pop.fam_out.get<long long>(), n, e->d,
-                     e->n_terms, e->x_tiled ? 1 : 0, pop.anc.get<const unsigned int>(), (const PopParams *)params);
+  if (e->x_layout == STATE_CHAIN && (size_t)e->d * sizeof(R) == 128)
+    hipLaunchKernelGGL(k_pop_gather_lines<R>, dim3((unsigned)((8 * n + kPopThreads - 1) / kPopThreads)), dim3(kPopThreads), 0, stream,
+                       e->x.get<const R>(), e->energy.get<const R>(), pop.fam.get<const long long>(), pop.x.get<R>(),
+                       pop.energy.get<R>(), pop.fam_out.get<long long>(), n, e->n_terms, pop.anc.get<const unsigned int>(),
+                       (const PopParams *)params);
+  else
+    hipLaunchKernelGGL(k_pop_gather<R>, dim3(slot_blocks), dim3(kPopThreads), 0, stream, e->x.get<const R>(), e->energy.get<const R>(),
+                       pop.fam.get<const long long>(), pop.x.get<R>(), pop.energy.get<R>(), pop.fam_out.get<long long>(), n, e->d,
+                       e->n_terms, e->x_layout, pop.anc.get<const unsigned int>(), (const PopParams *)params);
   return hipGetLastError();
 }
 
diff --git a/metropolisengine_amd/csrc/me_replica.hip b/metropolisengine_amd/csrc/me_replica.hip
--- a/metropolisengine_amd/csrc/me_replica.hip
+++ b/metropolisengine_amd/csrc/me_replica.hip
@@ -20,7 +20,7 @@
   long long n, rung_chains;
   unsigned long long chain_offset, round;
   uint32_t seed_lo, seed_hi;
-  int d, n_terms, first_rung, tiled;
+  int d, n_terms, first_rung, layout;
 };
 
 template <class F>
@@ -59,7 +59,8 @@
   const R delta = dbeta * (ea - eb);
   const bool accept = N_::finite(ea) && N_::finite(eb) && (delta >= R(0) || N_::uphill(u, eb - ea, dbeta, dbeta_log2e));
   if (accept) {
-    if (s.tiled) swap_rows(TiledField<R>(s.x, s.n, s.d), tiled_offset<R>(a, s.d), tiled_offset<R>(b, s.d), s.d);
+    if (s.layout == STATE_CHAIN) swap_rows(ChainField<R>(s.x, s.n, s.d), (unsigned int)a * (unsigned int)(s.d * sizeof(R)), (unsigned int)b * (unsigned int)(s.d * sizeof(R)), s.d);
+    else if (s.layout == STATE_TILED) swap_rows(TiledField<R>(s.x, s.n, s.d), tiled_offset<R>(a, s.d), tiled_offset<R>(b, s.d), s.d);
     else swap_rows(Field<R>(s.x, s.n, s.d), ea_off, eb_off, s.d);
     swap_rows(fe, ea_off, eb_off, s.n_terms);
   }
@@ -92,7 +93,7 @@
 }
 
 template <typename R>
-hipError_t launch(void *x, void *energy, long long n, int d, int n_terms, bool tiled_state, const void *ladder, int n_rungs,
+hipError_t launch(void *x, void *energy, long long n, int d, int n_terms, int state_layout, const void *ladder, int n_rungs,
                   unsigned long long round, unsigned long long chain_offset, unsigned long long seed,
                   unsigned long long *pair_counts, hipStream_t stream) {
   SwapArgs<R> s;
@@ -110,7 +111,7 @@
   s.seed_hi = (uint32_t)(seed >> 32);
   s.d = d;
   s.n_terms = n_terms;
-  s.tiled = tiled_state ? 1 : 0;
+  s.layout = state_layout;
   if (n_pairs == 0) return hipSuccess;
   const long long per_pair = std::min<long long>((s.rung_chains + kSwapThreads - 1) / kSwapThreads, std::max(kSwapBlocks / n_pairs, 1));
   hipLaunchKernelGGL(k_replica_swap<R>, dim3((unsigned)per_pair, (unsigned)n_pairs), dim3(kSwapThreads), 0, stream, s);
@@ -183,7 +184,7 @@
   ME_HIP(e, hipSetDevice(e->device));
   const auto swap = e->dtype == ME_F32 ? launch<float> : launch<double>;
   for (int i = 0; i < n_rounds; ++i) {
-    ME_HIP(e, swap(e->x.get(), e->energy.get(), e->n, e->d, e->n_terms, e->x_tiled, e->ladder.table.get(), e->ladder.n_rungs, e->ladder.round,
+    ME_HIP(e, swap(e->x.get(), e->energy.get(), e->n, e->d, e->n_terms, e->x_layout, e->ladder.table.get(), e->ladder.n_rungs, e->ladder.round,
                    e->chain_offset, e->seed, e->ladder.pair_counts.get<unsigned long long>(), e->stream));
     e->ladder.round += 1;
   }
```

Result: slower. 18.55 billion (-2.3%).
